# thangvubk/SoftGroup

Measured on AMD Instinct MI355X. Metric: scans/sec ScanNet-v2-like inference (softgroup_scannet.yaml, full forward_test), higher is better.
Workload: dtype f32

## Files before the change

### include/softgroup_hip.h

```cpp
#ifndef SOFTGROUP_HIP_H
#define SOFTGROUP_HIP_H

#include <stddef.h>
#include <stdint.h>

#ifdef __cplusplus
extern "C" {
#endif

typedef void *sg_stream_t;

#define SG_OK 0
#define SG_ERR_ARG (-1)
#define SG_ERR_WORKSPACE (-2)
#define SG_ERR_LAUNCH (-3)
#define SG_ERR_UNSUPPORTED (-4)

#define SG_BALLQUERY_MAX_NEIGHBORS 1000
#define SG_OCTREE_NUM_NODES 585
#define SG_OCTREE_NUM_LEAVES 512
#define SG_LISTS_SORTED 1
#define SG_LISTS_RADIUS 2

int sg_version(void);
const char *sg_last_error(void);
int sg_device_info(char *name_host, int name_cap, int *num_cu_host, int *clock_khz_host);

int sg_stream_release(sg_stream_t stream);
int sg_stream_create(sg_stream_t *stream_out);
int sg_stream_destroy(sg_stream_t stream);
int sg_stream_create_priority(sg_stream_t *stream_out, int level);

int sg_voxelize_idx_host(const int64_t *coords_host, int n, int ncol, int mode,
                         int32_t *input_map_host, int32_t *num_voxels_host,
                         int32_t *max_active_host);
int sg_voxelize_idx_fill_host(const int64_t *coords_host, int n, int ncol, int mode,
                              const int32_t *input_map_host, int num_voxels, int max_active,
                              int64_t *out_coords_host, int32_t *out_map_host);
size_t sg_voxelize_idx_workspace_bytes(int n);
int sg_voxelize_idx_build(const int64_t *coords, int n, int ncol, int mode, int32_t *input_map,
                          int32_t *meta, void *ws, size_t ws_bytes, sg_stream_t stream);
int sg_voxelize_idx_fill(const int64_t *coords, int n, int ncol, int mode,
                         const int32_t *input_map, int num_voxels, int max_active,
                         int64_t *out_coords, int32_t *out_map, void *ws, size_t ws_bytes,
                         sg_stream_t stream);

int sg_voxelize_fp(const float *feats, const int32_t *rules, int num_voxels, int max_active,
                   int channels, int average, float *out, sg_stream_t stream);
int sg_voxelize_bp(const float *d_out, const int32_t *rules, int num_voxels, int max_active,
                   int channels, int average, float *d_feats, sg_stream_t stream);

size_t sg_ballquery_workspace_bytes(int n);
int sg_ballquery_build_grid(const float *xyz, const int32_t *batch_idxs, int n, float radius,
                            void *ws, size_t ws_bytes, sg_stream_t stream);
int sg_ballquery_count(const float *xyz, const int32_t *batch_idxs, int n, float radius,
                       int32_t *start_len, int32_t *meta, void *ws, size_t ws_bytes,
                       sg_stream_t stream);
int sg_ballquery_fill(const float *xyz, const int32_t *batch_idxs, int n, float radius,
                      const int32_t *start_len, int32_t *idx, void *ws, size_t ws_bytes,
                      sg_stream_t stream);
size_t sg_scan_workspace_bytes(int n);
int sg_exclusive_scan_startlen(int32_t *start_len, int n, int32_t *meta, void *ws,
                               size_t ws_bytes, sg_stream_t stream);

int sg_octree_build_host(const float *points_host, const float *xyzwhl_host, int num_points,
                         int num_levels, float *boxes_host, int32_t *pt_inds_host,
                         int32_t *pt_start_len_host);
size_t sg_octree_build_workspace_bytes(int n);
int sg_octree_build(const float *points, int n, float *boxes, int32_t *pt_inds, int32_t *pt_start_len,
                    void *ws, size_t ws_bytes, sg_stream_t stream);
size_t sg_pyramid_inverse_map_workspace_bytes(int n_points, int n_voxels, int n_prop);
int sg_pyramid_inverse_map(const int32_t *proposals_idx, int64_t num_pairs, int n_prop,
                           const int32_t *l2p_map, int n_points, int n_voxels, int32_t *out_idx,
                           int32_t *out_offsets, int32_t *n_out_dev, void *ws, size_t ws_bytes,
                           sg_stream_t stream);
int sg_octree_ballquery_count(const float *points, const float *boxes, const int32_t *pt_inds,
                              const int32_t *pt_start_len, int n, float radius,
                              int32_t *start_len, sg_stream_t stream);
int sg_octree_ballquery_fill(const float *points, const float *boxes, const int32_t *pt_inds,
                             const int32_t *pt_start_len, int n, float radius,
                             const int32_t *start_len, int32_t *idx, sg_stream_t stream);

size_t sg_bfs_workspace_bytes(int n, int64_t n_edges);
int sg_bfs_cluster_label(const int32_t *bq_idxs, const int32_t *start_len, int n,
                         int64_t n_edges, int list_flags, const int32_t *seg_of_point,
                         const float *seg_thr, int n_seg, int32_t *n_cluster_host,
                         int32_t *sum_npoint_host, void *ws, size_t ws_bytes, sg_stream_t stream);
int sg_bfs_cluster_emit(const int32_t *bq_idxs, const int32_t *start_len, int n, int64_t n_edges,
                        const int32_t *seg_of_point, const float *seg_thr, int n_cluster,
                        int sum_npoint, int32_t *cluster_idxs, int32_t *cluster_offsets, void *ws,
                        size_t ws_bytes, sg_stream_t stream);

int sg_sec_mean(const float *inp, const int32_t *offsets, int n_seg, int channels, float *out,
                sg_stream_t stream);
int sg_sec_min(const float *inp, const int32_t *offsets, int n_seg, int channels, float *out,
               sg_stream_t stream);
int sg_sec_max(const float *inp, const int32_t *offsets, int n_seg, int channels, float *out,
               sg_stream_t stream);
int sg_global_avg_pool_fp(const float *feats, const int32_t *offsets, int n_seg, int channels,
                          float *out, sg_stream_t stream);
int sg_global_avg_pool_bp(float *d_feats, const int32_t *offsets, const float *d_out, int n_seg,
                          int channels, sg_stream_t stream);

int sg_get_mask_iou_on_cluster(const int32_t *proposals_idx, const int32_t *proposals_offset,
                               const int64_t *instance_labels, const int32_t *instance_pointnum,
                               int n_instance, int n_proposal, float *proposals_iou,
                               sg_stream_t stream);
int sg_get_mask_iou_on_pred(const int32_t *proposals_idx, const int32_t *proposals_offset,
                            const int64_t *instance_labels, const int32_t *instance_pointnum,
                            const float *mask_scores_sigmoid, int n_instance, int n_proposal,
                            float *proposals_iou, sg_stream_t stream);
int sg_get_mask_label(const int32_t *proposals_idx, const int32_t *proposals_offset,
                      const int64_t *instance_labels, const int64_t *instance_cls,
                      const float *proposals_iou, int n_instance, int n_proposal, float iou_thr,
                      float *mask_label, sg_stream_t stream);

size_t sg_spconv_hash_workspace_bytes(int num_rows);
int sg_spconv_subm_rulebook(const int32_t *indices, int num_rows, const int32_t *spatial_shape_host,
                            int32_t *nbr, void *ws, size_t ws_bytes, sg_stream_t stream);
int sg_spconv_down_build(const int32_t *indices, int num_rows, const int32_t *spatial_shape_host,
                         int32_t *in2out, int32_t *meta, void *ws, size_t ws_bytes,
                         sg_stream_t stream);
int sg_spconv_down_fill(const int32_t *indices, int num_rows, const int32_t *in2out,
                        int num_out_rows, int32_t *out_indices, int32_t *child, void *ws,
                        size_t ws_bytes, sg_stream_t stream);
int sg_spconv_inverse_rulebook(const int32_t *indices_fine, const int32_t *in2out, int num_rows,
                               int32_t *inv_nbr, sg_stream_t stream);

#define SG_PLAN_HIST_WORDS 40
size_t sg_spconv_plan_workspace_bytes(int num_out_rows);
int sg_spconv_plan(const int32_t *nbr, int num_out_rows, int kvol, int32_t *order,
                   uint32_t *tile_mask, int32_t *nbr_tiles, void *ws, size_t ws_bytes,
                   sg_stream_t stream);

#define SG_PYRAMID_MAX_LEVELS 10
typedef struct sg_plan_ptrs {
  int32_t *order;
  uint32_t *tile_mask;
  int32_t *nbr_tiles;
} sg_plan_ptrs;
typedef struct sg_pyramid_level {
  int rows;
  int32_t *indices;
  int32_t *nbr;
  sg_plan_ptrs subm;
  int32_t *in2out;
  int32_t *child;
  sg_plan_ptrs down;
  int32_t *inv;
  sg_plan_ptrs up;
} sg_pyramid_level;
size_t sg_spconv_pyramid_workspace_bytes(int num_rows, int n_levels);
int sg_spconv_pyramid_rows(const int32_t *indices, int num_rows, const int32_t *spatial_shape_host,
                           int n_levels, int32_t *rows_dev, void *ws, size_t ws_bytes,
                           sg_stream_t stream);
size_t sg_spconv_pyramid_build_workspace_bytes(const sg_pyramid_level *levels_host, int n_levels);
int sg_spconv_pyramid_build(const int32_t *indices, int num_rows, const int32_t *spatial_shape_host,
                            int n_levels, const sg_pyramid_level *levels_host, void *ws,
                            size_t ws_bytes, void *ws2, size_t ws2_bytes, sg_stream_t stream);

size_t sg_spconv_packed_weight_elems(int kvol, int cin, int cout);
int sg_spconv_pack_weight(const float *w, int cout, int kvol, int cin, int src_is_kio, float *w_k8,
                          sg_stream_t stream);

size_t sg_spconv_conv_workspace_bytes(int num_out_rows, int cout);
int sg_spconv_gather_conv_f32(const float *in, int num_in_rows, const int32_t *nbr,
                              int num_out_rows, int kvol, int cin, int cout, const float *w_k8,
                              const float *post_scale, const float *post_shift,
                              const float *residual, const float *act_scale,
                              const float *act_shift, float *out_act, const int32_t *order,
                              const uint32_t *tile_mask, const int32_t *nbr_tiles, float *out,
                              void *ws, size_t ws_bytes, sg_stream_t stream);

int sg_spconv_set_arithmetic(int mode);

int sg_spconv_set_combine(int mode);

int sg_grouping_set_lanes(int lanes);

int sg_spconv_set_chain(int mode);
int sg_spconv_chain_stats(int64_t *launches, int64_t *steps);

int sg_spconv_profile(int enable);
int sg_spconv_profile_read(double *total_ms, int *launches);
int sg_spconv_profile_detail(float *ms, int32_t *dims, int cap, int *calls);

typedef struct sg_mlp2 {
  const float *w1, *b1, *bn_scale, *bn_shift, *w2, *b2;
  int out;
} sg_mlp2;
int sg_pointwise_heads(const float *voxel_feats, const void *v2p_map, int v2p_is_int64, int n_points,
                       int channels, const sg_mlp2 *semantic, const sg_mlp2 *offset, float *output_feats,
                       float *semantic_scores, float *pt_offsets, int64_t *semantic_preds,
                       sg_stream_t stream);

size_t sg_spconv_packed_weight_elems_bf16(int kvol, int cin, int cout);
int sg_spconv_pack_weight_bf16(const float *w, int cout, int kvol, int cin, int src_is_kio,
                               uint16_t *w_k8_bf16, sg_stream_t stream);
size_t sg_spconv_conv_bf16_workspace_bytes(int num_out_rows, int cout);
int sg_spconv_gather_conv_bf16(const uint16_t *in, int num_in_rows, const int32_t *nbr, int num_out_rows,
                               int kvol, int cin, int cout, const uint16_t *w_k8_bf16,
                               const int32_t *order, const uint32_t *tile_mask, const int32_t *nbr_tiles,
                               uint16_t *out, void *ws, size_t ws_bytes, sg_stream_t stream);

int sg_spconv_transpose_table(const int32_t *nbr, int num_out_rows, int kvol, int32_t *nbr_t,
                              sg_stream_t stream);
size_t sg_spconv_wgrad_workspace_bytes(int num_out_rows, int kvol, int cin, int cout);
int sg_spconv_wgrad(const void *in, int in_is_bf16, const void *g_out, int g_is_bf16, const int32_t *nbr_t,
                    int num_out_rows, int kvol, int cin, int cout, float *dw_kio, void *ws,
                    size_t ws_bytes, sg_stream_t stream);

typedef struct sg_unet_block {
  int cin, cout;
  const float *bn1_scale, *bn1_shift;
  const float *w1;
  const float *bn2_scale, *bn2_shift;
  const float *w2;
  const float *w_i;
} sg_unet_block;
typedef struct sg_unet_level {
  int planes, n_blocks;
  const sg_unet_block *blocks;
  const sg_unet_block *tail;
  const float *down_bn_scale, *down_bn_shift, *down_w;
  const float *up_bn_scale, *up_bn_shift, *up_w;
} sg_unet_level;
typedef struct sg_unet_desc {
  int n_levels;
  const sg_unet_level *levels;
  int input_cin;
  const float *input_w;
  const float *out_bn_scale, *out_bn_shift;
  int input_cin_packed;
  int arithmetic;
} sg_unet_desc;
size_t sg_unet_arena_bytes(const sg_unet_desc *desc, int num_rows);
int sg_unet_forward(const sg_unet_desc *desc, const float *feats, const int32_t *indices,
                    int num_rows, const int32_t *spatial_shape_host, float *out, void *arena,
                    size_t arena_bytes, sg_stream_t stream);

typedef struct sg_train_bn {
  const float *weight, *bias;
  float *running_mean, *running_var;
  float momentum, eps;
  float *g_weight, *g_bias;
} sg_train_bn;
typedef struct sg_train_conv {
  const float *w;
  float *g_w;
} sg_train_conv;
typedef struct sg_unet_train_block {
  int cin, cout;
  sg_train_bn bn1, bn2;
  sg_train_conv c1, c2, ci;
} sg_unet_train_block;
typedef struct sg_unet_train_level {
  int planes, n_blocks;
  const sg_unet_train_block *blocks, *tail;
  sg_train_bn down_bn, up_bn;
  sg_train_conv down, up;
} sg_unet_train_level;
typedef struct sg_unet_train_desc {
  int n_levels;
  const sg_unet_train_level *levels;
  int input_cin;
  sg_train_conv input;
  sg_train_bn out_bn;
  int arithmetic;
} sg_unet_train_desc;
size_t sg_unet_train_arena_hint(const sg_unet_train_desc *desc, int num_rows);
int sg_unet_train_forward(const sg_unet_train_desc *desc, const float *feats, const int32_t *indices,
                          int num_rows, const int32_t *spatial_shape_host, float *out, void *arena,
                          size_t arena_bytes, size_t *arena_needed, void **tape, sg_stream_t stream);
int sg_unet_train_backward(void *tape, const float *g_out, float *g_feats, sg_stream_t stream);
void sg_unet_train_release(void *tape);

int sg_bn_relu_f32(const float *x, const float *scale, const float *shift, int64_t num_rows,
                   int channels, int relu, float *out, sg_stream_t stream);

int sg_gather_rows_f32(const float *in, const int32_t *index, int64_t num_out_rows, int channels,
                       float *out, sg_stream_t stream);
int sg_gather_rows_i64idx_f32(const float *in, const int64_t *index, int64_t num_out_rows,
                              int channels, float *out, sg_stream_t stream);

int sg_instance_npoint(const int32_t *proposals_idx, const float *mask_scores, int64_t num_pairs,
                       int stride, int n_classes, float mask_thr, int n_prop, int32_t *npoint,
                       sg_stream_t stream);
size_t sg_instance_runs_workspace_bytes(int n_kept, int n_points);
int sg_instance_runs(const int32_t *proposals_idx, const float *mask_scores, int64_t num_pairs,
                     int stride, int n_classes, float mask_thr, const int32_t *inst_of, int n_prop,
                     int n_kept, int n_points, int32_t *starts, int32_t *ends, int64_t *bounds,
                     int64_t runs_capacity, void *ws, size_t ws_bytes, sg_stream_t stream);

int64_t sg_rle_format_bound(int64_t total_runs, int digits);
int sg_rle_format_host(const int64_t *starts_host, const int64_t *lens_host,
                       const int64_t *bounds_host, int n_groups, char *out_host,
                       int64_t out_capacity, int64_t *out_offsets_host);
size_t sg_rle_format_device_workspace_bytes(int64_t run_capacity);
int64_t sg_rle_format_device_text_bytes(int64_t run_capacity, int64_t length);
int sg_rle_format_device(const int32_t *starts, const int32_t *ends, const int64_t *bounds, int n_inst,
                         int64_t run_capacity, int64_t length, uint8_t *text, int64_t text_capacity,
                         int64_t *text_off, void *ws, size_t ws_bytes, sg_stream_t stream);
int sg_rle_format_runs_host(const int32_t *starts_host, const int32_t *ends_host,
                            const int64_t *bounds_host, int n_groups, char *out_host,
                            int64_t out_capacity, int64_t *out_offsets_host);

size_t sg_panoptic_fusion_workspace_bytes(int n_inst, int n_points);
int sg_panoptic_fusion(const uint32_t *bits, int n_inst, int n_points, const int32_t *order,
                       const int32_t *label_id, const int64_t *semantic_preds, int cls_offset,
                       double skip_iou, int semantic_classes, int thing_class_min, uint32_t *out,
                       void *ws, size_t ws_bytes, sg_stream_t stream);

#define SG_NMS_IOU 0
#define SG_NMS_MIN 1
size_t sg_mask_nms_workspace_bytes(int n_inst, int64_t n_points);
int sg_mask_nms(const uint32_t *bits, int n_inst, int64_t n_points, const float *scores, const int32_t *labels,
                double thr, int measure, int class_agnostic, uint8_t *keep, int32_t *n_keep, int32_t *inter_out,
                void *ws, size_t ws_bytes, sg_stream_t stream);
int sg_mask_bits_from_runs(const int32_t *starts, const int32_t *ends, const int64_t *bounds, int64_t n_runs,
                           int n_inst, int64_t n_points, uint32_t *bits, sg_stream_t stream);

#define SG_SPLIT_ALL 0
#define SG_SPLIT_LARGEST 1
#define SG_SPLIT_FLAG_NOT_FINITE 1
#define SG_SPLIT_FLAG_CELL_RANGE 2
#define SG_SPLIT_FLAG_INTERNAL 4
#define SG_SPLIT_FLAG_TOO_MANY 8
size_t sg_mask_split_workspace_bytes(int n_inst, int64_t n_points, int64_t n_pairs);
int sg_mask_split_count(const float *xyz, const uint32_t *bits, int n_inst, int64_t n_points, double radius,
                        int min_npoint, int mode, int32_t *meta, void *ws, size_t ws_bytes, sg_stream_t stream);
int sg_mask_split_fill(int n_inst, int64_t n_points, int64_t n_pairs, const void *ws, size_t ws_bytes,
                       int64_t capacity, uint32_t *out_bits, int32_t *source, int32_t *npoint, sg_stream_t stream);

#define SG_SNAP_SNAP 0
#define SG_SNAP_GROW 1
#define SG_SNAP_TRIM 2
#define SG_SUPERPOINT_FLAG_ID 1
#define SG_SUPERPOINT_WALK 2048
size_t sg_superpoint_index_workspace_bytes(int64_t n_points);
int sg_superpoint_index(const int32_t *sp, int64_t n_points, int32_t *order, int32_t *seg_of, int32_t *seg_start,
                        int32_t *meta, void *ws, size_t ws_bytes, sg_stream_t stream);
size_t sg_mask_snap_workspace_bytes(int n_inst, int64_t n_points, int64_t n_seg);
int sg_mask_snap(const uint32_t *bits, int n_inst, int64_t n_points, const int32_t *order, const int32_t *seg_of,
                 const int32_t *seg_start, int64_t n_seg, int64_t n_valid, double thr, int mode, uint32_t *out_bits,
                 int32_t *npoint, void *ws, size_t ws_bytes, sg_stream_t stream);
size_t sg_superpoint_vote_workspace_bytes(int64_t n_points, int64_t n_seg, int n_classes);
int sg_superpoint_vote(const int32_t *labels, int64_t n_points, const int32_t *order, const int32_t *seg_of,
                       const int32_t *seg_start, int64_t n_seg, int n_classes, int ignore_label, int32_t *out_labels,
                       int32_t *seg_label, void *ws, size_t ws_bytes, sg_stream_t stream);

typedef struct sg_grouping_cfg {
  int n_points;
  int n_sem_classes;
  int n_seg;
  const int32_t *seg_class;
  const float *seg_thr;
  float score_thr;
  int min_npoint;
  float radius;
  int batch_size;
  float voxel_scale;
  int voxel_shape;
  int feat_channels;
} sg_grouping_cfg;
typedef struct sg_grouping_result {
  int n_selected, n_neighbours, n_proposals, sum_npoint, n_voxels, max_active;
  size_t proposals_idx;
  size_t proposals_offset;
  size_t voxel_coords;
  size_t voxel_offsets;
  size_t voxel_feats;
  size_t point_to_voxel;
  size_t arena_used, arena_needed;
  int deferred_classes;
  int reserved_;
} sg_grouping_result;
int sg_scan_grouping(const sg_grouping_cfg *cfg, const float *scores, const float *pt_offsets,
                     const float *coords_float, const int32_t *batch_idxs, const float *point_feats,
                     void *arena, size_t arena_bytes, sg_grouping_result *result_host,
                     sg_stream_t stream);

typedef struct sg_grouping_pp_cfg {
  sg_grouping_cfg base;
  int with_pyramid, with_octree, lvl_fusion;
  double radius;
  double base_size;
} sg_grouping_pp_cfg;
int sg_scan_grouping_pp(const sg_grouping_pp_cfg *cfg, const float *scores, const float *pt_offsets,
                        const float *coords_float, const int32_t *batch_idxs, const float *point_feats,
                        void *arena, size_t arena_bytes, sg_grouping_result *result_host,
                        sg_stream_t stream);

int sg_host_copy_2d(void *dst, int64_t dst_pitch_bytes, const void *src, int64_t src_pitch_bytes, int64_t rows,
                    int64_t row_bytes);
int sg_host_cast_f64_f32(float *dst, const double *src, int64_t n);
int sg_host_fill_i64_strided(int64_t *dst, int64_t pitch_elems, int64_t rows, int64_t value);
int sg_host_colmax_i64(const int64_t *src, int64_t rows, int64_t cols, int64_t *out_max);

typedef struct sg_instances_cfg {
  int n_proposals, n_classes;
  int score_stride;
  int64_t sum_npoint;
  int n_points;
  float cls_score_thr, mask_score_thr;
  int min_npoint;
} sg_instances_cfg;
typedef struct sg_instances_result {
  int n_kept;
  size_t off_class, off_score, off_text, text_bytes;
  size_t host_needed, arena_used, arena_needed;
  size_t bits;
  size_t label_id;
} sg_instances_result;
int sg_scan_instances(const sg_instances_cfg *cfg, const int32_t *proposals_idx, const float *mask_scores,
                      const float *cls_prob, const float *iou_scores, void *arena, size_t arena_bytes,
                      void *host_out, size_t host_bytes, sg_instances_result *result_host,
                      sg_stream_t stream);

typedef struct sg_linear {
  const float *w, *b;
  int out, in;
} sg_linear;
int sg_softmax_rows(const float *x, int64_t rows, int cols, float *out, sg_stream_t stream);
int sg_mlp_rows(const float *feats, const int32_t *idx, int64_t rows, int channels, const sg_mlp2 *mlp,
                float *out, sg_stream_t stream);
int sg_linear_rows(const float *x, int64_t rows, const sg_linear *lin, float *out, sg_stream_t stream);

#define SG_SCAN_DENSE_MAX 16
typedef struct sg_scan_dense_item {
  int kind;
  const void *ptr;
  size_t bytes;
} sg_scan_dense_item;
typedef struct sg_scan_desc {
  const sg_unet_desc *backbone;
  const sg_unet_desc *tiny;
  sg_mlp2 semantic, offset, mask;
  sg_linear cls, iou;
  int channels;
  int with_coords;
  int semantic_classes, instance_classes;
  sg_grouping_cfg grouping;
  float cls_score_thr, mask_score_thr;
  int min_npoint;
  int want_instances;
  int with_pyramid, with_octree;
  double pp_radius, pp_base_size;
} sg_scan_desc;
typedef struct sg_scan_input {
  int n_points, n_voxels, max_active;
  int batch_size;
  int spatial_shape[3];
  const float *feats;
  int feat_dim;
  const float *coords_float;
  const int32_t *p2v_map;
  const void *v2p_map;
  int v2p_is_int64;
  const void *voxel_coords;
  int voxel_coords_is_int64;
  const int32_t *batch_idxs;
  const int64_t *semantic_labels, *instance_labels;
  int n_dense;
  sg_scan_dense_item dense[SG_SCAN_DENSE_MAX];
} sg_scan_input;
typedef struct sg_scan_result {
  sg_grouping_result grouping;
  sg_instances_result instances;
  size_t grouping_base, instances_base;
  size_t dense_offset[SG_SCAN_DENSE_MAX];
  size_t dense_bytes;
  size_t voxel_feats_in, backbone_out, output_feats, semantic_scores, semantic_prob, pt_offsets,
      semantic_preds, tiny_out, mask_scores, cls_scores, cls_prob, iou_scores;
  size_t arena_used, arena_needed, host_dense_needed, host_inst_needed;
  int stage;
} sg_scan_result;
size_t sg_scan_arena_bytes(const sg_scan_desc *desc, int n_points, int n_voxels);
int sg_scan_forward(const sg_scan_desc *desc, const sg_scan_input *in, void *arena, size_t arena_bytes,
                    void *host_dense, size_t host_dense_bytes, void *host_inst, size_t host_inst_bytes,
                    sg_scan_result *result_host, sg_stream_t stream);

int sg_eval_intersections(const int32_t *run_start, const int64_t *run_off, const int32_t *run_pred,
                          int n_runs, int64_t total_points, const int32_t *gt_slot, int n_pred,
                          int n_slots, int32_t *counts, sg_stream_t stream);

#define SG_EVAL_I32 0
#define SG_EVAL_I64 1
#define SG_EVAL_U32 2
#define SG_EVAL_MAX_CLASSES 1024
#define SG_EVAL_BAD_GT 1
#define SG_EVAL_BAD_PRED 2
#define SG_EVAL_BAD_INST 4

size_t sg_eval_tally_workspace_bytes(int64_t n_points);
int sg_eval_class_tally(const void *pred, int pred_kind, const void *gt, int gt_kind, int64_t n_points,
                        int64_t ignore_label, int panoptic, int n_classes, uint64_t *tallies,
                        const void *inst, int inst_kind, const float *offset_pred, const float *offset_gt,
                        double *offset_sum, uint64_t *offset_count, int32_t *flags, void *ws, size_t ws_bytes,
                        sg_stream_t stream);

size_t sg_eval_panoptic_workspace_bytes(int64_t n_points);
int sg_eval_panoptic_segments(const void *pred, int pred_kind, const void *sem, int sem_kind,
                              const void *inst, int inst_kind, const int64_t *scan_off, int n_scans,
                              int64_t n_points, int64_t ignore_label, int n_classes, int64_t min_points,
                              uint64_t *fp_fn, int64_t *tp_rows, uint64_t *tp_count, int32_t *flags,
                              void *ws, size_t ws_bytes, sg_stream_t stream);

#define SG_INST_BAD_TEXT 1
#define SG_INST_ODD_TOKENS 2
#define SG_INST_RUN_RANGE 4
#define SG_INST_BAD_GT 8
#define SG_INST_OVERFLOW_GT 16
#define SG_INST_OVERFLOW_EX 32
#define SG_INST_NO_EXAMPLES 64
#define SG_INST_MAX_THRESHOLDS 16
#define SG_INST_SECTIONS 16

int64_t sg_inst_rle_run_slots(int64_t text_bytes, int n_masks);
int sg_inst_rle_parse(const uint8_t *text, const int64_t *text_off, const int32_t *mask_pred, int n_masks,
                      int64_t text_bytes, int64_t length, int32_t *run_start, int32_t *run_len, int32_t *run_pred,
                      int64_t run_slots, int32_t *vert_count, int32_t *flags, sg_stream_t stream);

size_t sg_inst_scan_workspace_bytes(int64_t n_points, int n_pred, int64_t run_slots, int n_classes, int gt_cap,
                                    int n_thr, int n_labels, int64_t *section_off);
int sg_inst_scan_update(const int64_t *gts, int64_t n_points, const int32_t *run_start, const int32_t *run_len,
                        const int32_t *run_pred, int64_t run_slots, const int32_t *pred_label,
                        const int32_t *pred_vert, const double *pred_conf, int n_pred, int n_labels, int n_classes,
                        int64_t min_region, const double *thresholds, int n_thr, int gt_cap, uint64_t *ex_key,
                        uint32_t *ex_meta, int64_t ex_cap, int32_t *seg_stats, int64_t *totals, int32_t *flags,
                        void *ws, size_t ws_bytes, sg_stream_t stream);

int sg_inst_scan_coverage(int64_t n_points, int n_pred, int64_t run_slots, int n_classes, int gt_cap, int n_thr,
                          int n_labels, const int32_t *pred_label, const int32_t *pred_vert,
                          const double *pred_conf, int64_t min_region, double iou_thr, double score_thr,
                          double *cov_sums, int64_t *tallies, const int32_t *flags, void *ws, size_t ws_bytes,
                          sg_stream_t stream);

size_t sg_inst_curves_workspace_bytes(int64_t n_examples, int n_seg);
int sg_inst_curves(const uint64_t *ex_key, const uint32_t *ex_meta, int64_t n_examples, const int32_t *seg_stats,
                   int n_seg, double *ap, double *rc, int32_t *flags, void *ws, size_t ws_bytes,
                   sg_stream_t stream);

#define SG_DET_BAD_COORD 1
#define SG_DET_MAX_THRESHOLDS 16

int sg_det_boxes_runs(const void *coords, int coords_f64, const int64_t *run_start, const int64_t *run_off,
                      const int32_t *run_owner, int64_t n_runs, int64_t total_points, int64_t n_owner,
                      double *boxes, int32_t *flags, sg_stream_t stream);

int sg_det_boxes_labels(const void *coords, int coords_f64, const int64_t *labels, const int64_t *scan_off,
                        const int64_t *owner_off, int n_scans, int64_t n_points, int64_t n_owner, double *boxes,
                        int64_t *count, int64_t *first, int32_t *flags, sg_stream_t stream);

size_t sg_det_match_workspace_bytes(int64_t n_gt, int n_thresholds);
int sg_det_match(const double *det_box, const int32_t *det_group, const int32_t *det_rank, int64_t n_det,
                 const double *gt_box, const int64_t *group_off, int64_t n_gt, const double *thresholds,
                 int n_thresholds, double *ovmax, int64_t *jmax, uint8_t *tp, void *ws, size_t ws_bytes,
                 sg_stream_t stream);

int sg_train_augment(const float *xyz, int64_t n, int has_scale, float scale_factor, const double *m_host,
                     double work_scale, double down, double *xyz_middle, double *work, uint64_t *stats,
                     sg_stream_t stream);
int sg_train_blur(float *grids, float *tmp, int b0, int b1, int b2, int n_grids, sg_stream_t stream);
int sg_train_elastic(double *work, int64_t n, const float *grids, int b0, int b1, int b2, double gran, double mag,
                     uint64_t *stats, sg_stream_t stream);
int sg_train_crop_count(const double *work, int64_t n, double down, const double *min_host,
                        const double *cand_host, int k, uint64_t *counts, sg_stream_t stream);
size_t sg_train_compact_workspace_bytes(int64_t n);
int sg_train_compact(const double *work, const double *xyz_middle, const float *feat, int c, const float *noise,
                     const int64_t *sem, const int64_t *inst, int64_t n, double down, const double *min_host,
                     const double *crop_host, int64_t out_cap, int64_t *coord, double *xyz_middle_out,
                     float *feat_out, int64_t *sem_out, int64_t *inst_out, int32_t *kept, void *ws,
                     size_t ws_bytes, sg_stream_t stream);
int sg_train_gather(const int64_t *idx, int64_t m, const float *xyz, const float *feat, int c, const int64_t *sem,
                    const int64_t *inst, float *xyz_out, float *feat_out, int64_t *sem_out, int64_t *inst_out,
                    sg_stream_t stream);
size_t sg_train_id_set_workspace_bytes(void);
int sg_train_id_set(const int64_t *labels, int64_t n, int64_t ignore, int64_t *out, int cap, void *ws,
                    size_t ws_bytes, sg_stream_t stream);
int sg_train_remap(int64_t *labels, int64_t n, const int64_t *sorted_ids, const int64_t *mapped, int k,
                   sg_stream_t stream);
size_t sg_train_instance_workspace_bytes(int64_t n, int k);
int sg_train_instance_info(const double *xyz_middle, const int64_t *inst, const int64_t *sem, int64_t n, int k,
                           int64_t cls_shift, int32_t *pointnum, int64_t *cls, double *pt_offset, void *ws,
                           size_t ws_bytes, sg_stream_t stream);

int sg_test_x4_minima(const float *xyz, int64_t n, const double *m_host, double scale, uint64_t *stats,
                      sg_stream_t stream);
int sg_test_x4_split(const float *xyz, const float *feat, int c, const int64_t *sem, const int64_t *inst, int64_t n,
                     const double *m_host, double scale, const double *min_host, int64_t *coord,
                     double *xyz_middle, float *feat_out, int64_t *sem_out, int64_t *inst_out, sg_stream_t stream);
int sg_kitti_decode_labels(const int32_t *words, int64_t n, const int32_t *lut, int64_t *sem, int64_t *inst,
                           uint64_t *missing, sg_stream_t stream);

int sg_mask_text_runs(const int32_t *starts, const int32_t *ends, const int64_t *bounds, int64_t n_runs, int n_inst,
                      int64_t length, int first, int count, uint8_t *text, int64_t text_capacity, sg_stream_t stream);
int sg_mask_text_bits(const uint32_t *bits, int n_inst, int64_t length, int first, int count, uint8_t *text,
                      int64_t text_capacity, sg_stream_t stream);
size_t sg_decimal_lines_workspace_bytes(int64_t n);
int sg_decimal_lines(const int64_t *values, int64_t n, const int32_t *nyu_table, int nyu_len, uint8_t *text,
                     int64_t text_capacity, int64_t *meta, void *ws, size_t ws_bytes, sg_stream_t stream);
int sg_panoptic_kitti_words(const uint32_t *words, int64_t n, const int32_t *lut, int lut_len, uint32_t *out,
                            uint64_t *missing, uint64_t *missing_host, sg_stream_t stream);
size_t sg_parse_decimal_lines_workspace_bytes(int64_t nbytes);
int sg_parse_decimal_lines(const uint8_t *text, int64_t nbytes, int64_t *values, int64_t capacity, int64_t *meta,
                           void *ws, size_t ws_bytes, sg_stream_t stream);
int sg_parse_mask_text(const uint8_t *text, int64_t nbytes, uint8_t *flags, uint32_t *bits, int64_t *meta,
                       sg_stream_t stream);

int sg_viz_paint_bits(const uint32_t *bits, int n_inst, int64_t n, const int32_t *priority, const uint8_t *skip,
                      int32_t *label, int32_t *pointnum, sg_stream_t stream);
size_t sg_viz_paint_runs_workspace_bytes(int n_inst, int64_t n);
int sg_viz_paint_runs(const int32_t *starts, const int32_t *ends, const int64_t *bounds, int64_t n_runs, int n_inst,
                      int64_t n, const int32_t *priority, const uint8_t *skip, int32_t *label, int32_t *pointnum,
                      void *ws, size_t ws_bytes, sg_stream_t stream);
int sg_viz_gt_labels(const int64_t *ids, int64_t n, int32_t *label, int32_t *pointnum, sg_stream_t stream);
size_t sg_viz_instance_rank_workspace_bytes(int n_inst);
int sg_viz_instance_rank(const int32_t *pointnum, int n_inst, int32_t *rank, void *ws, size_t ws_bytes,
                         sg_stream_t stream);
#define SG_VIZ_INPUT 0
#define SG_VIZ_CLASS 1
#define SG_VIZ_CLASS_WRAP 2
#define SG_VIZ_INSTANCE 3
int sg_viz_colors(int mode, const float *colors, const int64_t *cls, const int32_t *inst, const int32_t *rank,
                  int n_rank, const uint8_t *table, int k, int64_t n, uint8_t *rgb, int64_t *meta,
                  sg_stream_t stream);
size_t sg_viz_ply_vertices_workspace_bytes(int64_t n);
int sg_viz_ply_vertices(const float *xyz, const float *offset, const uint8_t *rgb, const uint8_t *keep, int64_t n,
                        uint8_t *text, int64_t text_capacity, int64_t *meta, void *ws, size_t ws_bytes,
                        sg_stream_t stream);

size_t sg_loss_reduce_workspace_bytes(void);
int sg_pointwise_loss_fwd(const float *semantic_scores, const int64_t *semantic_labels, const float *weight,
                          int64_t ignore_label, const float *pt_offsets, const float *pt_offset_labels,
                          const int64_t *instance_labels, int64_t n, int c, float *out, void *ws, size_t ws_bytes,
                          sg_stream_t stream);
int sg_pointwise_loss_bwd(const float *semantic_scores, const int64_t *semantic_labels, const float *weight,
                          int64_t ignore_label, const float *pt_offsets, const float *pt_offset_labels,
                          const int64_t *instance_labels, int64_t n, int c, const float *sums,
                          const float *g_semantic, const float *g_offset, float *d_scores, float *d_offsets,
                          sg_stream_t stream);
size_t sg_assign_proposals_workspace_bytes(int n_proposal);
int sg_assign_proposals(const float *ious_on_cluster, const int64_t *instance_cls, int64_t ignore_label,
                        float pos_iou_thr, int match_low_quality, float min_pos_thr, int64_t background_label,
                        int n_proposal, int n_gt, int64_t *labels, void *ws, size_t ws_bytes, sg_stream_t stream);
int sg_proposal_loss_fwd(const float *cls_scores, const float *iou_scores, const int64_t *labels,
                         const float *ious_on_pred, const int64_t *instance_cls, int64_t ignore_label,
                         int n_proposal, int n_gt, int k1, float *gt_iou, float *out, void *ws, size_t ws_bytes,
                         sg_stream_t stream);
int sg_proposal_loss_bwd(const float *cls_scores, const float *iou_scores, const int64_t *labels,
                         const float *gt_iou, const float *sums, const float *g_cls, const float *g_iou,
                         int n_proposal, int k1, float *d_cls_scores, float *d_iou_scores, sg_stream_t stream);
int sg_mask_loss_fwd(const float *mask_scores, const int32_t *instance_batch_idxs, const int64_t *labels,
                     const float *mask_label, int64_t m, int n_proposal, int k1, float *mask_sig, float *out,
                     void *ws, size_t ws_bytes, sg_stream_t stream);
int sg_mask_loss_bwd(const float *mask_scores, const int32_t *instance_batch_idxs, const int64_t *labels,
                     const float *mask_label, const float *sums, const float *g_mask, int64_t m, int n_proposal,
                     int k1, float *d_mask_scores, sg_stream_t stream);

#define SG_OPTIM_ROW_PARAM 0
#define SG_OPTIM_ROW_GRAD 1
#define SG_OPTIM_ROW_STATE0 2
#define SG_OPTIM_ROW_STATE1 3
#define SG_OPTIM_ROW_STEP 4
#define SG_OPTIM_ROW_COUNT 5
#define SG_OPTIM_TABLE_ROWS 6
int sg_optim_chunk_elems(void);
int64_t sg_optim_plan(const int64_t *counts, int n_tensors, int64_t *chunks, int64_t chunk_capacity);
size_t sg_optim_workspace_bytes(void);
int sg_optim_grad_norm(const int64_t *table, int n_tensors, const int64_t *chunks, int64_t n_chunks,
                       const float *grad_scale, float max_norm, float *out, void *ws, size_t ws_bytes,
                       sg_stream_t stream);
int sg_optim_adam_step(const int64_t *table, int n_tensors, const int64_t *chunks, int64_t n_chunks, double lr,
                       double beta1, double beta2, double eps, double weight_decay, int adamw,
                       const float *grad_scale, const float *found_inf, const float *clip_coef, int zero_grad,
                       int32_t *arrive, sg_stream_t stream);
int sg_optim_sgd_step(const int64_t *table, int n_tensors, const int64_t *chunks, int64_t n_chunks, double lr,
                      double momentum, double dampening, double weight_decay, int nesterov, const float *grad_scale,
                      const float *found_inf, const float *clip_coef, int zero_grad, int32_t *arrive,
                      sg_stream_t stream);
int sg_optim_scale_grads(const int64_t *table, int n_tensors, const int64_t *chunks, int64_t n_chunks,
                         const float *coef, sg_stream_t stream);

#define SG_PICK_FIRST 0
#define SG_PICK_CENTER 1
size_t sg_grid_downsample_workspace_bytes(int n);
int sg_grid_downsample(const float *xyz, int n, double voxel, int pick, int32_t *sample_ids, int32_t *inverse,
                       int32_t *meta, void *ws, size_t ws_bytes, sg_stream_t stream);
double sg_nearest_default_cell(const double *lo, const double *hi, int64_t n_src);
size_t sg_nearest_grid_bytes(int n_src);
int sg_nearest_build(const float *src, int n_src, double cell, void *grid, size_t grid_bytes, int32_t *meta,
                     sg_stream_t stream);
size_t sg_nearest_query_workspace_bytes(int n_query);
int sg_nearest_query(const float *src, int n_src, double cell, const void *grid, size_t grid_bytes, const float *query,
                     int n_query, double max_dist, int32_t *index, double *dist2, int32_t *meta, void *ws,
                     size_t ws_bytes, sg_stream_t stream);
int sg_mask_bits_gather(const uint32_t *bits, int n_inst, int64_t n_src, const int32_t *index, int64_t n_out,
                        uint32_t *out, int32_t *meta, sg_stream_t stream);
size_t sg_mask_runs_workspace_bytes(int n_inst, int64_t n_points);
int sg_mask_runs_count(const uint32_t *bits, int n_inst, int64_t n_points, int64_t *bounds, void *ws, size_t ws_bytes,
                       sg_stream_t stream);
int sg_mask_runs_fill(const uint32_t *bits, int n_inst, int64_t n_points, const void *ws, size_t ws_bytes,
                      int32_t *starts, int32_t *ends, int64_t capacity, sg_stream_t stream);

size_t sg_tile_assign_workspace_bytes(int n);
size_t sg_tile_assign_fill_workspace_bytes(int64_t total);
int sg_tile_assign_count(const float *xyz, int n, double size, double margin, double ox, double oy, int32_t *meta,
                         void *ws, size_t ws_bytes, sg_stream_t stream);
int sg_tile_assign_fill(const float *xyz, int n, double size, double margin, double ox, double oy, int n_tiles,
                        int64_t total, int32_t *tile_cells, int64_t *tile_off, int32_t *tile_points,
                        int32_t *core_tile, int32_t *core_pos, const void *ws, size_t ws_bytes, void *ws2,
                        size_t ws2_bytes, sg_stream_t stream);
size_t sg_tile_shared_workspace_bytes(int n_a);
int sg_tile_shared(const int32_t *a, int n_a, const int32_t *b, int n_b, int32_t *pos_a, int32_t *pos_b,
                   int32_t *count, void *ws, size_t ws_bytes, sg_stream_t stream);
int sg_mask_cross_links(const uint32_t *bits_a, int n_a, const uint32_t *bits_b, int n_b, int64_t n_bits,
                        const int32_t *labels_a, const int32_t *labels_b, int base_a, int base_b, int n_total,
                        double thr, int measure, int min_shared, uint32_t *adj, int32_t *inter_out,
                        int32_t *cnt_a_out, int32_t *cnt_b_out, sg_stream_t stream);
int sg_stitch_components(const uint32_t *adj, int n_total, int32_t *comp, sg_stream_t stream);
int sg_mask_bits_ids_count(const uint32_t *bits, int n_inst, int64_t n_bits, const uint8_t *core, int32_t *cnt,
                           int32_t *core_cnt, sg_stream_t stream);
int sg_mask_bits_ids_fill(const uint32_t *bits, int n_inst, int64_t n_bits, const int32_t *map, int64_t n_points,
                          const int64_t *row_off, const int32_t *row_key, int32_t *ids, uint32_t *keys,
                          int64_t capacity, int32_t *meta, sg_stream_t stream);
size_t sg_stitch_union_workspace_bytes(int64_t total, int n_obj, int64_t n_points);
int sg_stitch_union_count(const int32_t *ids, const uint32_t *keys, int64_t total, int n_obj, int64_t n_points,
                          int64_t *bounds, void *ws, size_t ws_bytes, sg_stream_t stream);
int sg_stitch_union_fill(int64_t total, int n_obj, int64_t n_points, const void *ws, size_t ws_bytes, int32_t *starts,
                         int32_t *ends, int64_t capacity, sg_stream_t stream);

#define SG_KNN_MAX_K 32
#define SG_KNN_MAX_SHELL 3
#define SG_KNN_FLAG_NOT_FINITE 1
#define SG_KNN_FLAG_CELL_RANGE 4
double sg_knn_default_cell(const double *lo, const double *hi, int64_t n, int k);
size_t sg_knn_workspace_bytes(int64_t n, int k);
int sg_knn(const float *xyz, int64_t n, int k, double cell, double max_dist, int32_t *idx, double *d2, int32_t *meta,
           void *ws, size_t ws_bytes, sg_stream_t stream);
#define SG_GEOMETRY_FLAG_INDEX 1
#define SG_GEOMETRY_FLAG_INTERNAL 2
int sg_point_normals(const float *xyz, int64_t n, const int32_t *nbr, int k, int min_neighbours, float *normals,
                     float *curvature, int32_t *meta, sg_stream_t stream);
size_t sg_grow_segments_workspace_bytes(int64_t n);
int sg_grow_segments(const int32_t *nbr, const double *nbr_d2, int64_t n, int k, const float *normals,
                     const float *curvature, double cos_thr, float max_curvature, double max_dist, int min_size,
                     int absorb, int32_t *sp, int32_t *meta, void *ws, size_t ws_bytes, sg_stream_t stream);

#ifdef __cplusplus
}
#endif
#endif
```

### softgroup_amd/_lib.py

```python
import ctypes as C
import os

_HERE = os.path.dirname(os.path.abspath(__file__))
LIB_PATH = os.path.join(_HERE, 'lib', os.environ.get('SG_LIB_NAME', 'libsoftgroup_hip.so'))

_lib = None

_vp, _i, _f, _i64, _sz, _d = C.c_void_p, C.c_int, C.c_float, C.c_int64, C.c_size_t, C.c_double
_pi32 = C.POINTER(C.c_int32)

SIGNATURES = {
    'sg_version': (_i, []),
    'sg_last_error': (C.c_char_p, []),
    'sg_device_info': (_i, [C.c_char_p, _i, C.POINTER(_i), C.POINTER(_i)]),
    'sg_stream_release': (_i, [_vp]),
    'sg_host_copy_2d': (_i, [_vp, _i64, _vp, _i64, _i64, _i64]),
    'sg_host_cast_f64_f32': (_i, [_vp, _vp, _i64]),
    'sg_host_fill_i64_strided': (_i, [_vp, _i64, _i64, _i64]),
    'sg_host_colmax_i64': (_i, [_vp, _i64, _i64, _vp]),
    'sg_stream_create': (_i, [_vp]),
    'sg_stream_create_priority': (_i, [_vp, _i]),
    'sg_stream_destroy': (_i, [_vp]),
    'sg_voxelize_idx_host': (_i, [_vp, _i, _i, _i, _vp, _pi32, _pi32]),
    'sg_voxelize_idx_fill_host': (_i, [_vp, _i, _i, _i, _vp, _i, _i, _vp, _vp]),
    'sg_voxelize_idx_workspace_bytes': (_sz, [_i]),
    'sg_voxelize_idx_build': (_i, [_vp, _i, _i, _i, _vp, _vp, _vp, _sz, _vp]),
    'sg_voxelize_idx_fill': (_i, [_vp, _i, _i, _i, _vp, _i, _i, _vp, _vp, _vp, _sz, _vp]),
    'sg_voxelize_fp': (_i, [_vp, _vp, _i, _i, _i, _i, _vp, _vp]),
    'sg_voxelize_bp': (_i, [_vp, _vp, _i, _i, _i, _i, _vp, _vp]),
    'sg_ballquery_workspace_bytes': (_sz, [_i]),
    'sg_ballquery_build_grid': (_i, [_vp, _vp, _i, _f, _vp, _sz, _vp]),
    'sg_ballquery_count': (_i, [_vp, _vp, _i, _f, _vp, _vp, _vp, _sz, _vp]),
    'sg_ballquery_fill': (_i, [_vp, _vp, _i, _f, _vp, _vp, _vp, _sz, _vp]),
    'sg_scan_workspace_bytes': (_sz, [_i]),
    'sg_exclusive_scan_startlen': (_i, [_vp, _i, _vp, _vp, _sz, _vp]),
    'sg_octree_build_host': (_i, [_vp, _vp, _i, _i, _vp, _vp, _vp]),
    'sg_octree_build_workspace_bytes': (_sz, [_i]),
    'sg_octree_build': (_i, [_vp, _i, _vp, _vp, _vp, _vp, _sz, _vp]),
    'sg_pyramid_inverse_map_workspace_bytes': (_sz, [_i, _i, _i]),
    'sg_pyramid_inverse_map': (_i, [_vp, _i64, _i, _vp, _i, _i, _vp, _vp, _vp, _vp, _sz, _vp]),
    'sg_octree_ballquery_count': (_i, [_vp, _vp, _vp, _vp, _i, _f, _vp, _vp]),
    'sg_octree_ballquery_fill': (_i, [_vp, _vp, _vp, _vp, _i, _f, _vp, _vp, _vp]),
    'sg_bfs_workspace_bytes': (_sz, [_i, _i64]),
    'sg_bfs_cluster_label': (_i, [_vp, _vp, _i, _i64, _i, _vp, _vp, _i, _pi32, _pi32, _vp, _sz, _vp]),
    'sg_bfs_cluster_emit': (_i, [_vp, _vp, _i, _i64, _vp, _vp, _i, _i, _vp, _vp, _vp, _sz, _vp]),
    'sg_sec_mean': (_i, [_vp, _vp, _i, _i, _vp, _vp]),
    'sg_sec_min': (_i, [_vp, _vp, _i, _i, _vp, _vp]),
    'sg_sec_max': (_i, [_vp, _vp, _i, _i, _vp, _vp]),
    'sg_global_avg_pool_fp': (_i, [_vp, _vp, _i, _i, _vp, _vp]),
    'sg_global_avg_pool_bp': (_i, [_vp, _vp, _vp, _i, _i, _vp]),
    'sg_get_mask_iou_on_cluster': (_i, [_vp, _vp, _vp, _vp, _i, _i, _vp, _vp]),
    'sg_get_mask_iou_on_pred': (_i, [_vp, _vp, _vp, _vp, _vp, _i, _i, _vp, _vp]),
    'sg_get_mask_label': (_i, [_vp, _vp, _vp, _vp, _vp, _i, _i, _f, _vp, _vp]),
    'sg_spconv_hash_workspace_bytes': (_sz, [_i]),
    'sg_spconv_subm_rulebook': (_i, [_vp, _i, _pi32, _vp, _vp, _sz, _vp]),
    'sg_spconv_pyramid_workspace_bytes': (_sz, [_i, _i]),
    'sg_spconv_pyramid_rows': (_i, [_vp, _i, _pi32, _i, _vp, _vp, _sz, _vp]),
    'sg_spconv_pyramid_build_workspace_bytes': (_sz, [_vp, _i]),
    'sg_spconv_pyramid_build': (_i, [_vp, _i, _pi32, _i, _vp, _vp, _sz, _vp, _sz, _vp]),
    'sg_spconv_down_build': (_i, [_vp, _i, _pi32, _vp, _vp, _vp, _sz, _vp]),
    'sg_spconv_down_fill': (_i, [_vp, _i, _vp, _i, _vp, _vp, _vp, _sz, _vp]),
    'sg_spconv_inverse_rulebook': (_i, [_vp, _vp, _i, _vp, _vp]),
    'sg_spconv_plan_workspace_bytes': (_sz, [_i]),
    'sg_spconv_plan': (_i, [_vp, _i, _i, _vp, _vp, _vp, _vp, _sz, _vp]),
    'sg_spconv_set_arithmetic': (_i, [_i]),
    'sg_spconv_set_combine': (_i, [_i]),
    'sg_spconv_set_chain': (_i, [_i]),
    'sg_grouping_set_lanes': (_i, [_i]),
    'sg_spconv_chain_stats': (_i, [_vp, _vp]),
    'sg_spconv_profile': (_i, [_i]),
    'sg_spconv_profile_read': (_i, [_vp, _vp]),
    'sg_spconv_profile_detail': (_i, [_vp, _vp, _i, _vp]),
    'sg_unet_arena_bytes': (_sz, [_vp, _i]),
    'sg_unet_forward': (_i, [_vp, _vp, _vp, _i, _vp, _vp, _vp, _sz, _vp]),
    'sg_unet_train_arena_hint': (_sz, [_vp, _i]),
    'sg_unet_train_forward': (_i, [_vp, _vp, _vp, _i, _vp, _vp, _vp, _sz, _vp, _vp, _vp]),
    'sg_unet_train_backward': (_i, [_vp, _vp, _vp, _vp]),
    'sg_unet_train_release': (None, [_vp]),
    'sg_pointwise_heads': (_i, [_vp, _vp, _i, _i, _i, _vp, _vp, _vp, _vp, _vp, _vp, _vp]),
    'sg_spconv_packed_weight_elems': (_sz, [_i, _i, _i]),
    'sg_spconv_pack_weight': (_i, [_vp, _i, _i, _i, _i, _vp, _vp]),
    'sg_spconv_conv_workspace_bytes': (_sz, [_i, _i]),
    'sg_spconv_gather_conv_f32': (_i, [_vp, _i, _vp, _i, _i, _i, _i, _vp, _vp, _vp, _vp, _vp, _vp,
                                       _vp, _vp, _vp, _vp, _vp, _vp, _sz, _vp]),
    'sg_spconv_packed_weight_elems_bf16': (_sz, [_i, _i, _i]),
    'sg_spconv_pack_weight_bf16': (_i, [_vp, _i, _i, _i, _i, _vp, _vp]),
    'sg_spconv_conv_bf16_workspace_bytes': (_sz, [_i, _i]),
    'sg_spconv_gather_conv_bf16': (_i, [_vp, _i, _vp, _i, _i, _i, _i, _vp, _vp, _vp, _vp, _vp, _vp, _sz,
                                        _vp]),
    'sg_spconv_transpose_table': (_i, [_vp, _i, _i, _vp, _vp]),
    'sg_spconv_wgrad_workspace_bytes': (_sz, [_i, _i, _i, _i]),
    'sg_spconv_wgrad': (_i, [_vp, _i, _vp, _i, _vp, _i, _i, _i, _i, _vp, _vp, _sz, _vp]),
    'sg_instance_npoint': (_i, [_vp, _vp, _i64, _i, _i, _f, _i, _vp, _vp]),
    'sg_instance_runs_workspace_bytes': (_sz, [_i, _i]),
    'sg_instance_runs': (_i, [_vp, _vp, _i64, _i, _i, _f, _vp, _i, _i, _i, _vp, _vp, _vp, _i64, _vp, _sz, _vp]),
    'sg_rle_format_bound': (_i64, [_i64, _i]),
    'sg_rle_format_host': (_i, [_vp, _vp, _vp, _i, _vp, _i64, _vp]),
    'sg_rle_format_device_workspace_bytes': (_sz, [_i64]),
    'sg_rle_format_device_text_bytes': (_i64, [_i64, _i64]),
    'sg_rle_format_device': (_i, [_vp, _vp, _vp, _i, _i64, _i64, _vp, _i64, _vp, _vp, _sz, _vp]),
    'sg_rle_format_runs_host': (_i, [_vp, _vp, _vp, _i, _vp, _i64, _vp]),
    'sg_panoptic_fusion_workspace_bytes': (_sz, [_i, _i]),
    'sg_panoptic_fusion': (_i, [_vp, _i, _i, _vp, _vp, _vp, _i, C.c_double, _i, _i, _vp, _vp, _sz, _vp]),
    'sg_mask_nms_workspace_bytes': (_sz, [_i, _i64]),
    'sg_mask_nms': (_i, [_vp, _i, _i64, _vp, _vp, _d, _i, _i, _vp, _vp, _vp, _vp, _sz, _vp]),
    'sg_mask_bits_from_runs': (_i, [_vp, _vp, _vp, _i64, _i, _i64, _vp, _vp]),
    'sg_mask_split_workspace_bytes': (_sz, [_i, _i64, _i64]),
    'sg_mask_split_count': (_i, [_vp, _vp, _i, _i64, _d, _i, _i, _vp, _vp, _sz, _vp]),
    'sg_mask_split_fill': (_i, [_i, _i64, _i64, _vp, _sz, _i64, _vp, _vp, _vp, _vp]),
    'sg_superpoint_index_workspace_bytes': (_sz, [_i64]),
    'sg_superpoint_index': (_i, [_vp, _i64, _vp, _vp, _vp, _vp, _vp, _sz, _vp]),
    'sg_mask_snap_workspace_bytes': (_sz, [_i, _i64, _i64]),
    'sg_mask_snap': (_i, [_vp, _i, _i64, _vp, _vp, _vp, _i64, _i64, _d, _i, _vp, _vp, _vp, _sz, _vp]),
    'sg_superpoint_vote_workspace_bytes': (_sz, [_i64, _i64, _i]),
    'sg_superpoint_vote': (_i, [_vp, _i64, _vp, _vp, _vp, _i64, _i, _i, _vp, _vp, _vp, _sz, _vp]),
    'sg_scan_grouping': (_i, [_vp, _vp, _vp, _vp, _vp, _vp, _vp, _sz, _vp, _vp]),
    'sg_scan_grouping_pp': (_i, [_vp, _vp, _vp, _vp, _vp, _vp, _vp, _sz, _vp, _vp]),
    'sg_scan_instances': (_i, [_vp, _vp, _vp, _vp, _vp, _vp, _sz, _vp, _sz, _vp, _vp]),
    'sg_softmax_rows': (_i, [_vp, _i64, _i, _vp, _vp]),
    'sg_mlp_rows': (_i, [_vp, _vp, _i64, _i, _vp, _vp, _vp]),
    'sg_linear_rows': (_i, [_vp, _i64, _vp, _vp, _vp]),
    'sg_scan_arena_bytes': (_sz, [_vp, _i, _i]),
    'sg_scan_forward': (_i, [_vp, _vp, _vp, _sz, _vp, _sz, _vp, _sz, _vp, _vp]),
    'sg_eval_intersections': (_i, [_vp, _vp, _vp, _i, _i64, _vp, _i, _i, _vp, _vp]),
    'sg_eval_tally_workspace_bytes': (_sz, [_i64]),
    'sg_eval_class_tally': (_i, [_vp, _i, _vp, _i, _i64, _i64, _i, _i, _vp, _vp, _i, _vp, _vp, _vp, _vp, _vp,
                                 _vp, _sz, _vp]),
    'sg_eval_panoptic_workspace_bytes': (_sz, [_i64]),
    'sg_eval_panoptic_segments': (_i, [_vp, _i, _vp, _i, _vp, _i, _vp, _i, _i64, _i64, _i, _i64, _vp, _vp, _vp,
                                       _vp, _vp, _sz, _vp]),
    'sg_inst_rle_run_slots': (_i64, [_i64, _i]),
    'sg_inst_rle_parse': (_i, [_vp, _vp, _vp, _i, _i64, _i64, _vp, _vp, _vp, _i64, _vp, _vp, _vp]),
    'sg_inst_scan_workspace_bytes': (_sz, [_i64, _i, _i64, _i, _i, _i, _i, _vp]),
    'sg_inst_scan_update': (_i, [_vp, _i64, _vp, _vp, _vp, _i64, _vp, _vp, _vp, _i, _i, _i, _i64, _vp, _i, _i,
                                 _vp, _vp, _i64, _vp, _vp, _vp, _vp, _sz, _vp]),
    'sg_inst_scan_coverage': (_i, [_i64, _i, _i64, _i, _i, _i, _i, _vp, _vp, _vp, _i64, _d, _d, _vp, _vp, _vp, _vp,
                                   _sz, _vp]),
    'sg_inst_curves_workspace_bytes': (_sz, [_i64, _i]),
    'sg_inst_curves': (_i, [_vp, _vp, _i64, _vp, _i, _vp, _vp, _vp, _vp, _sz, _vp]),
    'sg_det_boxes_runs': (_i, [_vp, _i, _vp, _vp, _vp, _i64, _i64, _i64, _vp, _vp, _vp]),
    'sg_det_boxes_labels': (_i, [_vp, _i, _vp, _vp, _vp, _i, _i64, _i64, _vp, _vp, _vp, _vp, _vp]),
    'sg_det_match_workspace_bytes': (_sz, [_i64, _i]),
    'sg_det_match': (_i, [_vp, _vp, _vp, _i64, _vp, _vp, _i64, _vp, _i, _vp, _vp, _vp, _vp, _sz, _vp]),
    'sg_bn_relu_f32': (_i, [_vp, _vp, _vp, _i64, _i, _i, _vp, _vp]),
    'sg_gather_rows_f32': (_i, [_vp, _vp, _i64, _i, _vp, _vp]),
    'sg_gather_rows_i64idx_f32': (_i, [_vp, _vp, _i64, _i, _vp, _vp]),
    'sg_train_augment': (_i, [_vp, _i64, _i, _f, _vp, C.c_double, C.c_double, _vp, _vp, _vp, _vp]),
    'sg_train_blur': (_i, [_vp, _vp, _i, _i, _i, _i, _vp]),
    'sg_train_elastic': (_i, [_vp, _i64, _vp, _i, _i, _i, C.c_double, C.c_double, _vp, _vp]),
    'sg_train_crop_count': (_i, [_vp, _i64, C.c_double, _vp, _vp, _i, _vp, _vp]),
    'sg_train_compact_workspace_bytes': (_sz, [_i64]),
    'sg_train_compact': (_i, [_vp, _vp, _vp, _i, _vp, _vp, _vp, _i64, C.c_double, _vp, _vp, _i64, _vp, _vp, _vp, _vp,
                              _vp, _vp, _vp, _sz, _vp]),
    'sg_train_gather': (_i, [_vp, _i64, _vp, _vp, _i, _vp, _vp, _vp, _vp, _vp, _vp, _vp]),
    'sg_train_id_set_workspace_bytes': (_sz, []),
    'sg_train_id_set': (_i, [_vp, _i64, _i64, _vp, _i, _vp, _sz, _vp]),
    'sg_train_remap': (_i, [_vp, _i64, _vp, _vp, _i, _vp]),
    'sg_train_instance_workspace_bytes': (_sz, [_i64, _i]),
    'sg_train_instance_info': (_i, [_vp, _vp, _vp, _i64, _i, _i64, _vp, _vp, _vp, _vp, _sz, _vp]),
    'sg_test_x4_minima': (_i, [_vp, _i64, _vp, C.c_double, _vp, _vp]),
    'sg_test_x4_split': (_i, [_vp, _vp, _i, _vp, _vp, _i64, _vp, C.c_double, _vp, _vp, _vp, _vp, _vp, _vp, _vp]),
    'sg_kitti_decode_labels': (_i, [_vp, _i64, _vp, _vp, _vp, _vp, _vp]),
    'sg_mask_text_runs': (_i, [_vp, _vp, _vp, _i64, _i, _i64, _i, _i, _vp, _i64, _vp]),
    'sg_mask_text_bits': (_i, [_vp, _i, _i64, _i, _i, _vp, _i64, _vp]),
    'sg_decimal_lines_workspace_bytes': (_sz, [_i64]),
    'sg_decimal_lines': (_i, [_vp, _i64, _vp, _i, _vp, _i64, _vp, _vp, _sz, _vp]),
    'sg_panoptic_kitti_words': (_i, [_vp, _i64, _vp, _i, _vp, _vp, _vp, _vp]),
    'sg_parse_decimal_lines_workspace_bytes': (_sz, [_i64]),
    'sg_parse_decimal_lines': (_i, [_vp, _i64, _vp, _i64, _vp, _vp, _sz, _vp]),
    'sg_parse_mask_text': (_i, [_vp, _i64, _vp, _vp, _vp, _vp]),
    'sg_viz_paint_bits': (_i, [_vp, _i, _i64, _vp, _vp, _vp, _vp, _vp]),
    'sg_viz_paint_runs_workspace_bytes': (_sz, [_i, _i64]),
    'sg_viz_paint_runs': (_i, [_vp, _vp, _vp, _i64, _i, _i64, _vp, _vp, _vp, _vp, _vp, _sz, _vp]),
    'sg_viz_gt_labels': (_i, [_vp, _i64, _vp, _vp, _vp]),
    'sg_viz_instance_rank_workspace_bytes': (_sz, [_i]),
    'sg_viz_instance_rank': (_i, [_vp, _i, _vp, _vp, _sz, _vp]),
    'sg_viz_colors': (_i, [_i, _vp, _vp, _vp, _vp, _i, _vp, _i, _i64, _vp, _vp, _vp]),
    'sg_viz_ply_vertices_workspace_bytes': (_sz, [_i64]),
    'sg_viz_ply_vertices': (_i, [_vp, _vp, _vp, _vp, _i64, _vp, _i64, _vp, _vp, _sz, _vp]),
    'sg_loss_reduce_workspace_bytes': (_sz, []),
    'sg_pointwise_loss_fwd': (_i, [_vp, _vp, _vp, _i64, _vp, _vp, _vp, _i64, _i, _vp, _vp, _sz, _vp]),
    'sg_pointwise_loss_bwd': (_i, [_vp, _vp, _vp, _i64, _vp, _vp, _vp, _i64, _i, _vp, _vp, _vp, _vp, _vp, _vp]),
    'sg_assign_proposals_workspace_bytes': (_sz, [_i]),
    'sg_assign_proposals': (_i, [_vp, _vp, _i64, _f, _i, _f, _i64, _i, _i, _vp, _vp, _sz, _vp]),
    'sg_proposal_loss_fwd': (_i, [_vp, _vp, _vp, _vp, _vp, _i64, _i, _i, _i, _vp, _vp, _vp, _sz, _vp]),
    'sg_proposal_loss_bwd': (_i, [_vp, _vp, _vp, _vp, _vp, _vp, _vp, _i, _i, _vp, _vp, _vp]),
    'sg_mask_loss_fwd': (_i, [_vp, _vp, _vp, _vp, _i64, _i, _i, _vp, _vp, _vp, _sz, _vp]),
    'sg_mask_loss_bwd': (_i, [_vp, _vp, _vp, _vp, _vp, _vp, _i64, _i, _i, _vp, _vp]),
    'sg_optim_chunk_elems': (_i, []),
    'sg_optim_plan': (_i64, [_vp, _i, _vp, _i64]),
    'sg_optim_workspace_bytes': (_sz, []),
    'sg_optim_grad_norm': (_i, [_vp, _i, _vp, _i64, _vp, _f, _vp, _vp, _sz, _vp]),
    'sg_optim_adam_step': (_i, [_vp, _i, _vp, _i64, _d, _d, _d, _d, _d, _i, _vp, _vp, _vp, _i, _vp, _vp]),
    'sg_optim_sgd_step': (_i, [_vp, _i, _vp, _i64, _d, _d, _d, _d, _i, _vp, _vp, _vp, _i, _vp, _vp]),
    'sg_optim_scale_grads': (_i, [_vp, _i, _vp, _i64, _vp, _vp]),
    'sg_grid_downsample_workspace_bytes': (_sz, [_i]),
    'sg_grid_downsample': (_i, [_vp, _i, _d, _i, _vp, _vp, _vp, _vp, _sz, _vp]),
    'sg_nearest_default_cell': (_d, [_vp, _vp, _i64]),
    'sg_nearest_grid_bytes': (_sz, [_i]),
    'sg_nearest_build': (_i, [_vp, _i, _d, _vp, _sz, _vp, _vp]),
    'sg_nearest_query_workspace_bytes': (_sz, [_i]),
    'sg_nearest_query': (_i, [_vp, _i, _d, _vp, _sz, _vp, _i, _d, _vp, _vp, _vp, _vp, _sz, _vp]),
    'sg_mask_bits_gather': (_i, [_vp, _i, _i64, _vp, _i64, _vp, _vp, _vp]),
    'sg_mask_runs_workspace_bytes': (_sz, [_i, _i64]),
    'sg_mask_runs_count': (_i, [_vp, _i, _i64, _vp, _vp, _sz, _vp]),
    'sg_mask_runs_fill': (_i, [_vp, _i, _i64, _vp, _sz, _vp, _vp, _i64, _vp]),
    'sg_tile_assign_workspace_bytes': (_sz, [_i]),
    'sg_tile_assign_fill_workspace_bytes': (_sz, [_i64]),
    'sg_tile_assign_count': (_i, [_vp, _i, _d, _d, _d, _d, _vp, _vp, _sz, _vp]),
    'sg_tile_assign_fill': (_i, [_vp, _i, _d, _d, _d, _d, _i, _i64, _vp, _vp, _vp, _vp, _vp, _vp, _sz, _vp, _sz, _vp]),
    'sg_tile_shared_workspace_bytes': (_sz, [_i]),
    'sg_tile_shared': (_i, [_vp, _i, _vp, _i, _vp, _vp, _vp, _vp, _sz, _vp]),
    'sg_mask_cross_links': (_i, [_vp, _i, _vp, _i, _i64, _vp, _vp, _i, _i, _i, _d, _i, _i, _vp, _vp, _vp, _vp, _vp]),
    'sg_stitch_components': (_i, [_vp, _i, _vp, _vp]),
    'sg_mask_bits_ids_count': (_i, [_vp, _i, _i64, _vp, _vp, _vp, _vp]),
    'sg_mask_bits_ids_fill': (_i, [_vp, _i, _i64, _vp, _i64, _vp, _vp, _vp, _vp, _i64, _vp, _vp]),
    'sg_stitch_union_workspace_bytes': (_sz, [_i64, _i, _i64]),
    'sg_stitch_union_count': (_i, [_vp, _vp, _i64, _i, _i64, _vp, _vp, _sz, _vp]),
    'sg_stitch_union_fill': (_i, [_i64, _i, _i64, _vp, _sz, _vp, _vp, _i64, _vp]),
    'sg_knn_default_cell': (_d, [_vp, _vp, _i64, _i]),
    'sg_knn_workspace_bytes': (_sz, [_i64, _i]),
    'sg_knn': (_i, [_vp, _i64, _i, _d, _d, _vp, _vp, _vp, _vp, _sz, _vp]),
    'sg_point_normals': (_i, [_vp, _i64, _vp, _i, _i, _vp, _vp, _vp, _vp]),
    'sg_grow_segments_workspace_bytes': (_sz, [_i64]),
    'sg_grow_segments': (_i, [_vp, _vp, _i64, _i, _vp, _vp, _d, _f, _d, _i, _i, _vp, _vp, _vp, _sz, _vp]),
}


class SoftGroupHipError(RuntimeError):
    pass


def lib():
    global _lib
    if _lib is None:
        import torch
        if not os.path.exists(LIB_PATH):
            raise SoftGroupHipError(
                f'{LIB_PATH} not found: the HIP extension is required (no CPU fallback). '
                'Build it with `python -c "import __graft_entry__ as g; g.build()"`.')
        L = C.CDLL(LIB_PATH)
        for name, (res, args) in SIGNATURES.items():
            fn = getattr(L, name)
            fn.restype = res
            fn.argtypes = args
        _lib = L
    return _lib


def check(rc, what=''):
    if rc != 0:
        msg = lib().sg_last_error()
        raise SoftGroupHipError(f'{what} failed ({rc}): {msg.decode() if msg else ""}')


def ptr(t):
    return None if t is None else t.data_ptr()


_raw_stream = None


def stream():
    global _raw_stream
    import torch
    if _raw_stream is None:
        _raw_stream = getattr(torch._C, '_cuda_getCurrentRawStream', None) or (
            lambda dev: torch.cuda.current_stream(dev).cuda_stream)
    return _raw_stream(torch.cuda.current_device())


def workspace(nbytes, device):
    import torch
    return torch.empty(max(int(nbytes), 256), dtype=torch.uint8, device=device)
```

### softgroup_amd/csrc/heads.h

```cpp
#pragma once
#include "common.h"

namespace sg {

struct Mlp2 {
  const float *w1, *b1, *scale, *shift, *w2, *b2;
  int out;
};

template <int C, int OUT_MAX>
__device__ __forceinline__ void mlp2(const float (&x)[C], const Mlp2 &m, float (&y)[OUT_MAX]) {
  float h[C];
#pragma unroll
  for (int o = 0; o < C; ++o) {
    float a = m.b1[o];
#pragma unroll
    for (int c = 0; c < C; ++c) a = fmaf(x[c], m.w1[o * C + c], a);
    h[o] = fmaxf(fmaf(a, m.scale[o], m.shift[o]), 0.f);
  }
#pragma unroll
  for (int o = 0; o < OUT_MAX; ++o) {
    if (o < m.out) {
      float a = m.b2[o];
#pragma unroll
      for (int c = 0; c < C; ++c) a = fmaf(h[c], m.w2[o * C + c], a);
      y[o] = a;
    }
  }
}

}
```

### softgroup_amd/csrc/heads.hip

```cpp
#include "common.h"
#include "heads.h"

namespace sg {

template <int C, int SEM_MAX, typename IdxT>
__global__ void __launch_bounds__(256) pointwise_heads_kernel(const float *__restrict__ vox, const IdxT *__restrict__ v2p,
                                                             int n, Mlp2 sem, Mlp2 off, float *__restrict__ out_feats,
                                                             float *__restrict__ sem_scores, float *__restrict__ pt_offsets,
                                                             int64_t *__restrict__ sem_preds) {
  const int p = blockIdx.x * 256 + threadIdx.x;
  if (p >= n) return;
  const int64_t row = v2p ? static_cast<int64_t>(v2p[p]) : p;
  float x[C];
  const float4 *src = reinterpret_cast<const float4 *>(vox + row * C);
#pragma unroll
  for (int q = 0; q < C / 4; ++q) {
    const float4 v = src[q];
    x[4 * q] = v.x; x[4 * q + 1] = v.y; x[4 * q + 2] = v.z; x[4 * q + 3] = v.w;
  }
  if (out_feats) {
    float4 *dst = reinterpret_cast<float4 *>(out_feats + static_cast<int64_t>(p) * C);
#pragma unroll
    for (int q = 0; q < C / 4; ++q) dst[q] = make_float4(x[4 * q], x[4 * q + 1], x[4 * q + 2], x[4 * q + 3]);
  }
  {
    float y[SEM_MAX];
    mlp2<C, SEM_MAX>(x, sem, y);
    float best = y[0];
    int arg = 0;
#pragma unroll
    for (int o = 0; o < SEM_MAX; ++o) {
      if (o < sem.out) {
        sem_scores[static_cast<int64_t>(p) * sem.out + o] = y[o];
        if (o > 0 && (y[o] > best || (y[o] != y[o] && best == best))) {
          best = y[o];
          arg = o;
        }
      }
    }
    if (sem_preds) sem_preds[p] = arg;
  }
  {
    float y[4];
    mlp2<C, 4>(x, off, y);
#pragma unroll
    for (int o = 0; o < 4; ++o)
      if (o < off.out) pt_offsets[static_cast<int64_t>(p) * off.out + o] = y[o];
  }
}

template <int C, typename IdxT>
static void launch_heads(const float *vox, const void *v2p, int n, const Mlp2 &s, const Mlp2 &o, float *out_feats,
                         float *sem_scores, float *pt_offsets, int64_t *sem_preds, hipStream_t st) {
  pointwise_heads_kernel<C, 32, IdxT><<<(n + 255) / 256, 256, 0, st>>>(vox, static_cast<const IdxT *>(v2p), n, s, o,
                                                                       out_feats, sem_scores, pt_offsets, sem_preds);
}

}

using namespace sg;

extern "C" int sg_pointwise_heads(const float *voxel_feats, const void *v2p_map, int v2p_is_int64, int n_points,
                                  int channels, const sg_mlp2 *semantic, const sg_mlp2 *offset, float *output_feats,
                                  float *semantic_scores, float *pt_offsets, int64_t *semantic_preds,
                                  sg_stream_t stream) {
  SG_REQUIRE(n_points >= 0 && semantic && offset && semantic_scores && pt_offsets, "sg_pointwise_heads: bad arguments");
  SG_REQUIRE(channels == 16 || channels == 32, "sg_pointwise_heads: channels must be 16 or 32 (got %d)", channels);
  SG_REQUIRE(semantic->out >= 1 && semantic->out <= 32 && offset->out >= 1 && offset->out <= 4,
             "sg_pointwise_heads: head widths out of range (semantic %d, offset %d)", semantic->out, offset->out);
  if (n_points == 0) return SG_OK;
  const Mlp2 s{semantic->w1, semantic->b1, semantic->bn_scale, semantic->bn_shift, semantic->w2, semantic->b2, semantic->out};
  const Mlp2 o{offset->w1, offset->b1, offset->bn_scale, offset->bn_shift, offset->w2, offset->b2, offset->out};
  hipStream_t st = as_stream(stream);
  if (channels == 32) {
    if (v2p_is_int64) launch_heads<32, int64_t>(voxel_feats, v2p_map, n_points, s, o, output_feats, semantic_scores, pt_offsets, semantic_preds, st);
    else launch_heads<32, int32_t>(voxel_feats, v2p_map, n_points, s, o, output_feats, semantic_scores, pt_offsets, semantic_preds, st);
  } else {
    if (v2p_is_int64) launch_heads<16, int64_t>(voxel_feats, v2p_map, n_points, s, o, output_feats, semantic_scores, pt_offsets, semantic_preds, st);
    else launch_heads<16, int32_t>(voxel_feats, v2p_map, n_points, s, o, output_feats, semantic_scores, pt_offsets, semantic_preds, st);
  }
  return check_launch("sg_pointwise_heads");
}
```

### softgroup_amd/csrc/scan_exec.hip

```cpp
#include <stdlib.h>
#include <string.h>

#include "common.h"
#include "scan.h"

namespace sg {

constexpr int kSelBlock = 256;
constexpr int kMaxSeg = 32;

__global__ void __launch_bounds__(kSelBlock) select_count_kernel(const float *__restrict__ scores, int n,
                                                                int n_cls, const int32_t *__restrict__ seg_class,
                                                                int n_seg, float thr, int n_blocks,
                                                                int32_t *__restrict__ blk_cnt) {
  __shared__ int part[4][kMaxSeg];
  const int i = blockIdx.x * kSelBlock + threadIdx.x;
  const int wave = threadIdx.x >> 6, lane = threadIdx.x & 63;
  for (int s = 0; s < n_seg; ++s) {
    const bool on = i < n && scores[static_cast<int64_t>(i) * n_cls + seg_class[s]] > thr;
    const int c = __popcll(__ballot(on));
    if (lane == 0) part[wave][s] = c;
  }
  __syncthreads();
  if (threadIdx.x < n_seg)
    blk_cnt[threadIdx.x * n_blocks + blockIdx.x] =
        part[0][threadIdx.x] + part[1][threadIdx.x] + part[2][threadIdx.x] + part[3][threadIdx.x];
}

__global__ void __launch_bounds__(1024) select_scan_kernel(const int32_t *__restrict__ blk_cnt, int n_seg,
                                                          int n_blocks, int min_npoint,
                                                          int32_t *__restrict__ blk_off,
                                                          int32_t *__restrict__ meta) {
  constexpr int kG = 8;
  __shared__ int seg_tot[kMaxSeg], seg_base[kMaxSeg + 1], carry_s[kMaxSeg];
  __shared__ int wtot[kG][16];
  const int wave = threadIdx.x >> 6, lane = threadIdx.x & 63;
  for (int s0 = 0; s0 < n_seg; s0 += kG) {
    int sum[kG];
#pragma unroll
    for (int j = 0; j < kG; ++j) sum[j] = 0;
    for (int b0 = 0; b0 < n_blocks; b0 += 1024) {
      const int b = b0 + threadIdx.x;
      int v[kG];
#pragma unroll
      for (int j = 0; j < kG; ++j) v[j] = (s0 + j < n_seg && b < n_blocks) ? blk_cnt[(s0 + j) * n_blocks + b] : 0;
#pragma unroll
      for (int j = 0; j < kG; ++j) sum[j] += v[j];
    }
#pragma unroll
    for (int j = 0; j < kG; ++j) {
      const int t = wave_sum(sum[j]);
      if (lane == 0) wtot[j][wave] = t;
    }
    __syncthreads();
    if (threadIdx.x < kG && s0 + threadIdx.x < n_seg) {
      int t = 0;
      for (int w = 0; w < 16; ++w) t += wtot[threadIdx.x][w];
      seg_tot[s0 + threadIdx.x] = t >= min_npoint ? t : 0;
    }
    __syncthreads();
  }
  if (threadIdx.x == 0) {
    int acc = 0;
    for (int s = 0; s < n_seg; ++s) {
      seg_base[s] = acc;
      carry_s[s] = acc;
      acc += seg_tot[s];
      meta[1 + s] = seg_tot[s];
    }
    seg_base[n_seg] = acc;
    meta[0] = acc;
  }
  __syncthreads();
  for (int s0 = 0; s0 < n_seg; s0 += kG) {
    for (int b0 = 0; b0 < n_blocks; b0 += 1024) {
      const int b = b0 + threadIdx.x;
      int v[kG], incl[kG];
#pragma unroll
      for (int j = 0; j < kG; ++j)
        v[j] = (s0 + j < n_seg && b < n_blocks && seg_tot[s0 + j] > 0) ? blk_cnt[(s0 + j) * n_blocks + b] : 0;
#pragma unroll
      for (int j = 0; j < kG; ++j) {
        incl[j] = wave_incl_scan(v[j]);
        if (lane == 63) wtot[j][wave] = incl[j];
      }
      __syncthreads();
#pragma unroll
      for (int j = 0; j < kG; ++j) {
        if (s0 + j < n_seg) {
          int before = 0, all = 0;
          for (int w = 0; w < 16; ++w) {
            const int x = wtot[j][w];
            before += w < wave ? x : 0;
            all += x;
          }
          if (b < n_blocks)
            blk_off[(s0 + j) * n_blocks + b] = seg_tot[s0 + j] > 0 ? carry_s[s0 + j] + before + incl[j] - v[j] : -1;
        }
      }
      __syncthreads();
      if (threadIdx.x < kG && s0 + threadIdx.x < n_seg) {
        int all = 0;
        for (int w = 0; w < 16; ++w) all += wtot[threadIdx.x][w];
        carry_s[s0 + threadIdx.x] += all;
      }
      __syncthreads();
    }
  }
}

__global__ void __launch_bounds__(kSelBlock) select_emit_kernel(
    const float *__restrict__ scores, int n, int n_cls, const int32_t *__restrict__ seg_class, int n_seg,
    float thr, int n_blocks, const int32_t *__restrict__ blk_off, const float *__restrict__ coords,
    const float *__restrict__ offsets, const int32_t *__restrict__ batch_idxs, int batch_size,
    int32_t *__restrict__ obj, int32_t *__restrict__ seg_of, float *__restrict__ pts, int32_t *__restrict__ key) {
  __shared__ int wcnt[4];
  const int i = blockIdx.x * kSelBlock + threadIdx.x;
  const int wave = threadIdx.x >> 6;
  float c[3] = {0.f, 0.f, 0.f};
  int bi = 0;
  if (i < n) {
#pragma unroll
    for (int a = 0; a < 3; ++a) c[a] = __fadd_rn(coords[3LL * i + a], offsets[3LL * i + a]);
    bi = batch_idxs[i];
  }
  for (int s = 0; s < n_seg; ++s) {
    const int base = blk_off[s * n_blocks + blockIdx.x];
    if (base < 0) continue;
    const bool on = i < n && scores[static_cast<int64_t>(i) * n_cls + seg_class[s]] > thr;
    const uint64_t m = __ballot(on);
    if ((threadIdx.x & 63) == 0) wcnt[wave] = __popcll(m);
    __syncthreads();
    int before = 0;
    for (int w = 0; w < wave; ++w) before += wcnt[w];
    if (on) {
      const int pos = base + before + mask_prefix(m);
      obj[pos] = i;
      seg_of[pos] = s;
      pts[3LL * pos] = c[0];
      pts[3LL * pos + 1] = c[1];
      pts[3LL * pos + 2] = c[2];
      key[pos] = s * batch_size + bi;
    }
    __syncthreads();
  }
}

__global__ void __launch_bounds__(256) proposal_map_kernel(int32_t *__restrict__ pairs, int64_t S,
                                                          const int32_t *__restrict__ obj) {
  for (int64_t e = blockIdx.x * 256LL + threadIdx.x; e < S; e += gridDim.x * 256LL)
    pairs[2 * e + 1] = obj[pairs[2 * e + 1]];
}

__global__ void __launch_bounds__(256) proposal_box_kernel(const int32_t *__restrict__ pairs,
                                                          const int32_t *__restrict__ offsets, int n_prop,
                                                          const float *__restrict__ coords, float inv_ss,
                                                          float scale_max, float *__restrict__ cscale,
                                                          float *__restrict__ lo_s) {
  __shared__ float rmin[3][256], rmax[3][256];
  for (int p = blockIdx.x; p < n_prop; p += gridDim.x) {
    const int s = offsets[p], e = offsets[p + 1];
    float mn[3] = {INFINITY, INFINITY, INFINITY}, mx[3] = {-INFINITY, -INFINITY, -INFINITY};
#pragma unroll 4
    for (int i = s + threadIdx.x; i < e; i += 256) {
      const int pt = pairs[2LL * i + 1];
#pragma unroll
      for (int a = 0; a < 3; ++a) {
        const float x = coords[3LL * pt + a];
        if (x < mn[a]) mn[a] = x;
        if (x > mx[a]) mx[a] = x;
      }
    }
#pragma unroll
    for (int a = 0; a < 3; ++a) {
      rmin[a][threadIdx.x] = mn[a];
      rmax[a][threadIdx.x] = mx[a];
    }
    __syncthreads();
    for (int w = 128; w > 0; w >>= 1) {
      if (threadIdx.x < w) {
#pragma unroll
        for (int a = 0; a < 3; ++a) {
          const float x = rmin[a][threadIdx.x + w], y = rmax[a][threadIdx.x + w];
          if (x < rmin[a][threadIdx.x]) rmin[a][threadIdx.x] = x;
          if (y > rmax[a][threadIdx.x]) rmax[a][threadIdx.x] = y;
        }
      }
      __syncthreads();
    }
    if (threadIdx.x == 0) {
      float ext = -INFINITY;
      bool nan = false;
#pragma unroll
      for (int a = 0; a < 3; ++a) {
        const float d = __fmul_rn(__fsub_rn(rmax[a][0], rmin[a][0]), inv_ss);
        nan |= d != d;
        if (d > ext) ext = d;
      }
      if (nan) ext = NAN;
      float cs = __fadd_rn(__fmul_rn(__fdiv_rn(1.0f, ext), 1.0f), -0.01f);
      cs = (cs != cs) ? cs : fminf(cs, scale_max);
      cscale[p] = cs;
#pragma unroll
      for (int a = 0; a < 3; ++a) lo_s[3 * p + a] = __fmul_rn(rmin[a][0], cs);
    }
    __syncthreads();
  }
}

__global__ void __launch_bounds__(256) proposal_voxel_coords_kernel(
    const int32_t *__restrict__ pairs, int64_t S, const float *__restrict__ coords,
    const float *__restrict__ cscale, const float *__restrict__ lo_s, int ss, int64_t *__restrict__ vox,
    int32_t *__restrict__ bad) {
  for (int64_t e = blockIdx.x * 256LL + threadIdx.x; e < S; e += gridDim.x * 256LL) {
    const int p = pairs[2 * e], pt = pairs[2 * e + 1];
    const float cs = cscale[p];
    int64_t *o = vox + 4 * e;
    o[0] = p;
    bool ok = true;
#pragma unroll
    for (int a = 0; a < 3; ++a) {
      const float v = __fsub_rn(__fmul_rn(coords[3LL * pt + a], cs), lo_s[3 * p + a]);
      ok &= v >= 0.f && v < static_cast<float>(ss);
      o[1 + a] = static_cast<int64_t>(v);
    }
    if (!ok) atomicOr(bad, 1);
  }
}

__global__ void __launch_bounds__(256) proposal_voxel_feats_kernel(const float *__restrict__ feats,
                                                                  const int32_t *__restrict__ pairs,
                                                                  const int32_t *__restrict__ rules, int M,
                                                                  int max_active, int C,
                                                                  float *__restrict__ out) {
  const int64_t total = static_cast<int64_t>(M) * C;
  for (int64_t t = blockIdx.x * 256LL + threadIdx.x; t < total; t += gridDim.x * 256LL) {
    const int row = static_cast<int>(t / C), c = static_cast<int>(t - static_cast<int64_t>(row) * C);
    const int32_t *r = rules + static_cast<int64_t>(row) * (max_active + 1);
    const int cnt = r[0];
    const float m = cnt > 0 ? __fdiv_rn(1.0f, static_cast<float>(cnt)) : 1.0f;
    float acc = 0.0f;
    int i = 1;
    for (; i + 15 <= cnt; i += 16) {
      int a[16], q[16];
      float f[16];
#pragma unroll
      for (int j = 0; j < 16; ++j) a[j] = r[i + j];
#pragma unroll
      for (int j = 0; j < 16; ++j) q[j] = pairs[2LL * a[j] + 1];
#pragma unroll
      for (int j = 0; j < 16; ++j) f[j] = feats[static_cast<int64_t>(q[j]) * C + c];
#pragma unroll
      for (int j = 0; j < 16; ++j) acc = __fadd_rn(acc, __fmul_rn(m, f[j]));
    }
    for (; i + 3 <= cnt; i += 4) {
      const int a0 = r[i], a1 = r[i + 1], a2 = r[i + 2], a3 = r[i + 3];
      const int p0 = pairs[2LL * a0 + 1], p1 = pairs[2LL * a1 + 1], p2 = pairs[2LL * a2 + 1],
                p3 = pairs[2LL * a3 + 1];
      const float f0 = feats[static_cast<int64_t>(p0) * C + c], f1 = feats[static_cast<int64_t>(p1) * C + c],
                  f2 = feats[static_cast<int64_t>(p2) * C + c], f3 = feats[static_cast<int64_t>(p3) * C + c];
      acc = __fadd_rn(acc, __fmul_rn(m, f0));
      acc = __fadd_rn(acc, __fmul_rn(m, f1));
      acc = __fadd_rn(acc, __fmul_rn(m, f2));
      acc = __fadd_rn(acc, __fmul_rn(m, f3));
    }
    for (; i <= cnt; ++i)
      acc = __fadd_rn(acc, __fmul_rn(m, feats[static_cast<int64_t>(pairs[2LL * r[i] + 1]) * C + c]));
    out[t] = acc;
  }
}

__global__ void __launch_bounds__(256) proposal_voxel_pack_kernel(const int64_t *__restrict__ vc, int M,
                                                                 int n_prop, int32_t *__restrict__ out,
                                                                 int32_t *__restrict__ vox_off) {
  for (int m = blockIdx.x * 256 + threadIdx.x; m < M; m += gridDim.x * 256) {
    const int p = static_cast<int>(vc[4LL * m]);
#pragma unroll
    for (int a = 0; a < 4; ++a) out[4LL * m + a] = static_cast<int32_t>(vc[4LL * m + a]);
    if (m == 0 || static_cast<int>(vc[4LL * (m - 1)]) != p) vox_off[p] = m;
    if (m == M - 1) vox_off[n_prop] = M;
  }
}

__global__ void __launch_bounds__(1024) instance_keep_kernel(const float *__restrict__ cls_prob,
                                                           const float *__restrict__ iou, int stride,
                                                           const int32_t *__restrict__ npoint, int n_prop,
                                                           int nc, float cls_thr, int min_npoint,
                                                           int32_t *__restrict__ inst_of,
                                                           int32_t *__restrict__ kept_cls,
                                                           float *__restrict__ kept_score,
                                                           int32_t *__restrict__ head) {
  __shared__ int wsum[16];
  __shared__ int cap_s;
  if (threadIdx.x == 0) cap_s = 0;
  __syncthreads();
  const int total = nc * n_prop;
  const int wave = threadIdx.x >> 6, lane = threadIdx.x & 63;
  int carry = 0, cap = 0;
  for (int base = 0; base < total; base += 1024) {
    const int t = base + threadIdx.x;
    int keep = 0, np = 0, i = 0, p = 0;
    if (t < total) {
      i = t / n_prop;
      p = t - i * n_prop;
      np = npoint[p * nc + i];
      keep = (cls_prob[p * stride + i] > cls_thr && np >= min_npoint) ? 1 : 0;
    }
    int incl = wave_incl_scan(keep);
    if (lane == 63) wsum[wave] = incl;
    __syncthreads();
    int tot = 0;
#pragma unroll
    for (int w = 0; w < 16; ++w) {
      const int x = wsum[w];
      incl += w < wave ? x : 0;
      tot += x;
    }
    __syncthreads();
    if (t < total) {
      const int k = carry + incl - keep;
      inst_of[t] = keep ? k : -1;
      if (keep) {
        kept_cls[k] = i + 1;
        const float q = iou[p * stride + i];
        const float qc = (q != q) ? q : fminf(fmaxf(q, 0.f), 1.f);
        kept_score[k] = __fmul_rn(cls_prob[p * stride + i], qc);
        cap += np;
      }
    }
    carry += tot;
  }
  cap = wave_sum(cap);
  if ((threadIdx.x & 63) == 0) atomicAdd(&cap_s, cap);
  __syncthreads();
  if (threadIdx.x == 0) {
    head[0] = carry;
    head[1] = cap_s;
  }
}

__global__ void __launch_bounds__(256) pp_level_inputs_kernel(const int32_t *__restrict__ obj, int n,
                                                             const float *__restrict__ coords,
                                                             const float *__restrict__ offsets,
                                                             const int32_t *__restrict__ batch_idxs, float inv,
                                                             int64_t *__restrict__ vox, float *__restrict__ c3,
                                                             float *__restrict__ o3) {
  const int i = blockIdx.x * 256 + threadIdx.x;
  if (i >= n) return;
  const int p = obj[i];
  vox[4LL * i] = batch_idxs[p];
#pragma unroll
  for (int a = 0; a < 3; ++a) {
    const float c = coords[3LL * p + a];
    c3[3LL * i + a] = c;
    o3[3LL * i + a] = offsets[3LL * p + a];
    vox[4LL * i + 1 + a] = static_cast<int64_t>(__fmul_rn(c, inv));
  }
}
__global__ void __launch_bounds__(256) pp_level_points_kernel(const float *__restrict__ cl, const float *__restrict__ ol,
                                                             const int64_t *__restrict__ vc, int m,
                                                             float *__restrict__ q, int32_t *__restrict__ qb) {
  const int i = blockIdx.x * 256 + threadIdx.x;
  if (i >= m) return;
#pragma unroll
  for (int a = 0; a < 3; ++a) q[3LL * i + a] = __fadd_rn(cl[3LL * i + a], ol[3LL * i + a]);
  qb[i] = static_cast<int32_t>(vc[4LL * i]);
}
__global__ void __launch_bounds__(256) pp_append_kernel(const int32_t *__restrict__ pairs, int rows,
                                                       const int32_t *__restrict__ offs, int n_prop,
                                                       const int32_t *__restrict__ obj, int prop_base, int row_base,
                                                       int32_t *__restrict__ out_pairs, int32_t *__restrict__ out_offs) {
  const int i = blockIdx.x * 256 + threadIdx.x;
  if (i < rows) {
    out_pairs[2LL * (row_base + i)] = pairs[2LL * i] + prop_base;
    out_pairs[2LL * (row_base + i) + 1] = obj[pairs[2LL * i + 1]];
  }
  if (i < n_prop) out_offs[prop_base + 1 + i] = offs[i + 1] + row_base;
  if (i == 0 && prop_base == 0) out_offs[0] = 0;
}

struct ScanArena {
  char *base;
  size_t cap, off;
  bool ok = true;
  ScanArena(void *p, size_t n) : base(static_cast<char *>(p)), cap(n), off(0) {}
  template <typename T>
  T *take(size_t count) {
    const size_t bytes = align_up((count ? count : 1) * sizeof(T));
    const size_t at = off;
    off += bytes;
    if (off > cap) {
      ok = false;
      return nullptr;
    }
    return reinterpret_cast<T *>(base + at);
  }
  size_t at(const void *p) const { return static_cast<size_t>(static_cast<const char *>(p) - base); }
};

__global__ void __launch_bounds__(64) read_back_kernel(const int32_t *__restrict__ dev, int words, int32_t *host) {
  if (static_cast<int>(threadIdx.x) < words)
    __hip_atomic_store(host + threadIdx.x, dev[threadIdx.x], __ATOMIC_RELAXED, __HIP_MEMORY_SCOPE_SYSTEM);
}
static int read_back(int32_t *host, const int32_t *dev, int words, hipStream_t stream, const char *what) {
  static const bool by_kernel = getenv("SG_READBACK_KERNEL") && atoi(getenv("SG_READBACK_KERNEL")) != 0;
  if (by_kernel && words <= 64) {
    read_back_kernel<<<1, 64, 0, stream>>>(dev, words, host);
    if (hipStreamSynchronize(stream) != hipSuccess) {
      set_error("%s: device -> host read-back failed", what);
      return SG_ERR_LAUNCH;
    }
    return SG_OK;
  }
  if (hipMemcpyAsync(host, dev, sizeof(int32_t) * words, hipMemcpyDeviceToHost, stream) != hipSuccess ||
      hipStreamSynchronize(stream) != hipSuccess) {
    set_error("%s: device -> host read-back failed", what);
    return SG_ERR_LAUNCH;
  }
  return SG_OK;
}

#define SG_TRY(expr)              \
  do {                            \
    const int rc_ = (expr);       \
    if (rc_ != SG_OK) return rc_; \
  } while (0)
#define SG_TAKE(var, T, count)                                                                    \
  T *var = ar.take<T>(count);                                                                     \
  if (var == nullptr) {                                                                           \
    res->arena_needed = ar.off + ar.off / 2 + (8 << 20);                                          \
    set_error("%s: arena too small (%zu bytes, need about %zu)", kWhat, ar.cap, res->arena_needed); \
    return SG_ERR_WORKSPACE;                                                                      \
  }

thread_local void (*t_scan_emit_hook)(void *) = nullptr;
thread_local void *t_scan_emit_ctx = nullptr;

}

using namespace sg;

static int voxelise_proposals(const sg_grouping_cfg *cfg, const int32_t *pairs, const int32_t *poff, int n_prop, int S,
                              const float *coords_float, const float *point_feats, ScanArena &ar, int32_t *meta,
                              int32_t *host, sg_grouping_result *res, sg_stream_t stream_, const char *kWhat) {
  hipStream_t stream = as_stream(stream_);
  const int C = cfg->feat_channels;
  SG_TAKE(cscale, float, n_prop);
  SG_TAKE(lo_s, float, 3 * static_cast<size_t>(n_prop));
  SG_TAKE(vox, int64_t, 4 * static_cast<size_t>(S));
  SG_TAKE(bad, int32_t, 64);
  hipMemsetAsync(bad, 0, sizeof(int32_t), stream);
  const float inv_ss = 1.0f / static_cast<float>(cfg->voxel_shape);
  proposal_box_kernel<<<n_prop < 1024 ? n_prop : 1024, 256, 0, stream>>>(pairs, poff, n_prop, coords_float, inv_ss,
                                                                        cfg->voxel_scale, cscale, lo_s);
  proposal_voxel_coords_kernel<<<grid_for(S, 256), 256, 0, stream>>>(pairs, S, coords_float, cscale, lo_s,
                                                                    cfg->voxel_shape, vox, bad);
  const size_t vx_bytes = sg_voxelize_idx_workspace_bytes(S);
  SG_TAKE(vx_ws, char, vx_bytes);
  SG_TAKE(inp_map, int32_t, S);
  SG_TRY(sg_voxelize_idx_build(vox, S, 4, 4, inp_map, meta + 40, vx_ws, vx_bytes, stream_));
  hipMemcpyAsync(meta + 42, bad, sizeof(int32_t), hipMemcpyDeviceToDevice, stream);
  SG_TRY(read_back(host, meta + 40, 3, stream, kWhat));
  const int M = host[0], mA = host[1];
  SG_REQUIRE(host[2] == 0, "%s: a proposal voxel coordinate fell outside [0, %d) "
             "(the reference asserts here, softgroup.py:698)", kWhat, cfg->voxel_shape);
  res->n_voxels = M;
  res->max_active = mA;
  SG_TAKE(vc64, int64_t, 4 * static_cast<size_t>(M));
  SG_TAKE(rules, int32_t, static_cast<size_t>(M) * (mA + 1));
  SG_TRY(sg_voxelize_idx_fill(vox, S, 4, 4, inp_map, M, mA, vc64, rules, vx_ws, vx_bytes, stream_));
  SG_TAKE(vc32, int32_t, 4 * static_cast<size_t>(M));
  SG_TAKE(vox_off, int32_t, static_cast<size_t>(n_prop) + 1);
  SG_TAKE(vfeat, float, static_cast<size_t>(M) * C);
  proposal_voxel_pack_kernel<<<grid_for(M, 256), 256, 0, stream>>>(vc64, M, n_prop, vc32, vox_off);
  proposal_voxel_feats_kernel<<<grid_for(static_cast<int64_t>(M) * C, 256), 256, 0, stream>>>(
      point_feats, pairs, rules, M, mA, C, vfeat);
  res->voxel_coords = ar.at(vc32);
  res->voxel_offsets = ar.at(vox_off);
  res->voxel_feats = ar.at(vfeat);
  res->point_to_voxel = ar.at(inp_map);
  res->arena_used = ar.off;
  return check_launch(kWhat);
}

extern "C" {

int sg_scan_grouping(const sg_grouping_cfg *cfg, const float *scores, const float *pt_offsets,
                     const float *coords_float, const int32_t *batch_idxs, const float *point_feats,
                     void *arena, size_t arena_bytes, sg_grouping_result *res, sg_stream_t stream_) {
  static const char *kWhat = "sg_scan_grouping";
  SG_REQUIRE(cfg != nullptr && res != nullptr, "sg_scan_grouping: null descriptor");
  SG_REQUIRE(cfg->n_points >= 0 && cfg->n_sem_classes >= 1 && cfg->n_seg >= 0 && cfg->n_seg <= kMaxSeg &&
                 cfg->batch_size >= 1 && cfg->feat_channels >= 1 && cfg->voxel_shape >= 0,
             "sg_scan_grouping: bad configuration (n_seg must be <= %d)", kMaxSeg);
  memset(res, 0, sizeof(*res));
  hipStream_t stream = as_stream(stream_);
  int32_t *host = pinned_words();
  SG_REQUIRE(host != nullptr, "sg_scan_grouping: no pinned host words");
  ScanArena ar(arena, arena_bytes);
  const int n = cfg->n_points, n_seg = cfg->n_seg;
  if (n == 0 || n_seg == 0) return SG_OK;

  const int n_blocks = (n + kSelBlock - 1) / kSelBlock;
  SG_TAKE(meta, int32_t, 64);
  SG_TAKE(blk_cnt, int32_t, static_cast<size_t>(n_seg) * n_blocks);
  SG_TAKE(blk_off, int32_t, static_cast<size_t>(n_seg) * n_blocks);
  select_count_kernel<<<n_blocks, kSelBlock, 0, stream>>>(scores, n, cfg->n_sem_classes, cfg->seg_class, n_seg,
                                                         cfg->score_thr, n_blocks, blk_cnt);
  select_scan_kernel<<<1, 1024, 0, stream>>>(blk_cnt, n_seg, n_blocks, cfg->min_npoint, blk_off, meta);
  SG_TRY(check_launch(kWhat));
  SG_TRY(read_back(host, meta, 1, stream, kWhat));
  const int n_sel = host[0];
  res->n_selected = n_sel;
  if (n_sel == 0) return SG_OK;
  SG_TAKE(obj, int32_t, n_sel);
  SG_TAKE(seg_of, int32_t, n_sel);
  SG_TAKE(pts, float, 3 * static_cast<size_t>(n_sel));
  SG_TAKE(key, int32_t, n_sel);
  select_emit_kernel<<<n_blocks, kSelBlock, 0, stream>>>(scores, n, cfg->n_sem_classes, cfg->seg_class, n_seg,
                                                        cfg->score_thr, n_blocks, blk_off, coords_float,
                                                        pt_offsets, batch_idxs, cfg->batch_size, obj, seg_of,
                                                        pts, key);

  const size_t bq_bytes = sg_ballquery_workspace_bytes(n_sel);
  SG_TAKE(bq_ws, char, bq_bytes);
  SG_TAKE(start_len, int32_t, 2 * static_cast<size_t>(n_sel));
  const size_t sc_bytes = sg_scan_workspace_bytes(n_sel);
  SG_TAKE(sc_ws, char, sc_bytes);
  hipMemsetAsync(start_len, 0, sizeof(int32_t) * 2 * n_sel, stream);
  SG_TRY(sg_ballquery_build_grid(pts, key, n_sel, cfg->radius, bq_ws, bq_bytes, stream_));
  SG_TRY(sg_ballquery_count(pts, key, n_sel, cfg->radius, start_len, nullptr, bq_ws, bq_bytes, stream_));
  SG_TRY(sg_exclusive_scan_startlen(start_len, n_sel, meta + 32, sc_ws, sc_bytes, stream_));
  SG_TRY(read_back(host, meta + 32, 1, stream, kWhat));
  const int n_active = host[0];
  res->n_neighbours = n_active;
  SG_TAKE(bq_idx, int32_t, n_active);
  SG_TRY(sg_ballquery_fill(pts, key, n_sel, cfg->radius, start_len, bq_idx, bq_ws, bq_bytes, stream_));

  const size_t bfs_bytes = sg_bfs_workspace_bytes(n_sel, n_active);
  SG_TAKE(bfs_ws, char, bfs_bytes);
  int32_t n_prop = 0, S = 0;
  SG_TRY(sg_bfs_cluster_label(bq_idx, start_len, n_sel, n_active, SG_LISTS_SORTED | SG_LISTS_RADIUS, seg_of,
                              cfg->seg_thr, n_seg, &n_prop, &S, bfs_ws, bfs_bytes, stream_));
  res->n_proposals = n_prop;
  res->sum_npoint = S;
  if (S == 0) return SG_OK;
  SG_TAKE(pairs, int32_t, 2 * static_cast<size_t>(S));
  SG_TAKE(poff, int32_t, static_cast<size_t>(n_prop) + 1);
  hipMemsetAsync(poff, 0, sizeof(int32_t) * (n_prop + 1), stream);
  if (t_scan_emit_hook != nullptr) t_scan_emit_hook(t_scan_emit_ctx);
  SG_TRY(sg_bfs_cluster_emit(bq_idx, start_len, n_sel, n_active, seg_of, cfg->seg_thr, n_prop, S, pairs, poff,
                             bfs_ws, bfs_bytes, stream_));
  proposal_map_kernel<<<grid_for(S, 256), 256, 0, stream>>>(pairs, S, obj);
  res->proposals_idx = ar.at(pairs);
  res->proposals_offset = ar.at(poff);
  if (cfg->voxel_shape == 0) {
    res->arena_used = ar.off;
    return check_launch(kWhat);
  }

  return voxelise_proposals(cfg, pairs, poff, n_prop, S, coords_float, point_feats, ar, meta, host, res, stream_, kWhat);
}

int sg_scan_grouping_pp(const sg_grouping_pp_cfg *pcfg, const float *scores, const float *pt_offsets,
                        const float *coords_float, const int32_t *batch_idxs, const float *point_feats,
                        void *arena, size_t arena_bytes, sg_grouping_result *res, sg_stream_t stream_) {
  static const char *kWhat = "sg_scan_grouping_pp";
  SG_REQUIRE(pcfg != nullptr && res != nullptr, "sg_scan_grouping_pp: null descriptor");
  const sg_grouping_cfg *cfg = &pcfg->base;
  SG_REQUIRE(cfg->n_points >= 0 && cfg->n_sem_classes >= 1 && cfg->n_seg >= 0 && cfg->n_seg <= kMaxSeg &&
                 cfg->batch_size >= 1 && cfg->feat_channels >= 1 && cfg->voxel_shape >= 0,
             "sg_scan_grouping_pp: bad configuration (n_seg must be <= %d)", kMaxSeg);
  SG_REQUIRE(pcfg->radius > 0 && (!pcfg->with_pyramid || pcfg->base_size > 0),
             "sg_scan_grouping_pp: radius and pyramid_base_size must be positive");
  memset(res, 0, sizeof(*res));
  hipStream_t stream = as_stream(stream_);
  int32_t *host = pinned_words();
  SG_REQUIRE(host != nullptr, "sg_scan_grouping_pp: no pinned host words");
  ScanArena ar(arena, arena_bytes);
  const int n = cfg->n_points, n_seg = cfg->n_seg;
  if (n == 0 || n_seg == 0) return SG_OK;

  const int n_blocks = (n + kSelBlock - 1) / kSelBlock;
  SG_TAKE(meta, int32_t, 128);
  SG_TAKE(blk_cnt, int32_t, static_cast<size_t>(n_seg) * n_blocks);
  SG_TAKE(blk_off, int32_t, static_cast<size_t>(n_seg) * n_blocks);
  select_count_kernel<<<n_blocks, kSelBlock, 0, stream>>>(scores, n, cfg->n_sem_classes, cfg->seg_class, n_seg,
                                                         cfg->score_thr, n_blocks, blk_cnt);
  select_scan_kernel<<<1, 1024, 0, stream>>>(blk_cnt, n_seg, n_blocks, cfg->min_npoint, blk_off, meta);
  SG_TRY(check_launch(kWhat));
  SG_TRY(read_back(host, meta, 1 + n_seg, stream, kWhat));
  const int n_sel = host[0];
  int count[kMaxSeg];
  for (int s = 0; s < n_seg; ++s) count[s] = host[1 + s];
  res->n_selected = n_sel;
  if (n_sel == 0) return SG_OK;
  SG_TAKE(obj, int32_t, n_sel);
  SG_TAKE(seg_of, int32_t, n_sel);
  SG_TAKE(pts, float, 3 * static_cast<size_t>(n_sel));
  SG_TAKE(key, int32_t, n_sel);
  select_emit_kernel<<<n_blocks, kSelBlock, 0, stream>>>(scores, n, cfg->n_sem_classes, cfg->seg_class, n_seg,
                                                        cfg->score_thr, n_blocks, blk_off, coords_float,
                                                        pt_offsets, batch_idxs, cfg->batch_size, obj, seg_of,
                                                        pts, key);
  SG_TAKE(pairs, int32_t, 2 * static_cast<size_t>(n_sel));
  SG_TAKE(poff, int32_t, static_cast<size_t>(n_sel) + 2);
  int n_prop = 0, S = 0;
  int64_t n_nbr = 0;
  const size_t loop_mark0 = ar.off;
  size_t loop_mark = loop_mark0;
  bool hook_pending = t_scan_emit_hook != nullptr;
  const bool defer_on = !(getenv("SG_PP_DEFER") && atoi(getenv("SG_PP_DEFER")) == 0);
  BfsDefer def;
  int def_rows = -1;
  bool def_mapped = false;
  struct DeferGuard {
    BfsDefer &d;
    ~DeferGuard() {
      if (d.deferred && d.side != nullptr) hipStreamSynchronize(d.side);
    }
  } defer_guard{def};
  int s0 = 0;
  for (int s = 0; s < n_seg; s0 += count[s], ++s) {
    const int nc_pts = count[s];
    if (nc_pts == 0) continue;
    ar.off = loop_mark;
    int level = 1;
    if (pcfg->with_pyramid) level = nc_pts > 1000000 ? 3 : nc_pts > 100000 ? 2 : 1;
    const float radius = static_cast<float>(pcfg->with_pyramid ? pcfg->radius * level : pcfg->radius);
    const bool mapped = pcfg->with_pyramid && (level > 1 || !pcfg->lvl_fusion);
    const float *q = pts + 3 * static_cast<size_t>(s0);
    const int32_t *qb = key + s0;
    int n_q = nc_pts, n_lvl = 0;
    const int32_t *l2p = nullptr;
    if (mapped) {
      const float inv = 1.0f / static_cast<float>(pcfg->base_size * level);
      SG_TAKE(vox, int64_t, 4 * static_cast<size_t>(nc_pts));
      SG_TAKE(c3, float, 3 * static_cast<size_t>(nc_pts));
      SG_TAKE(o3, float, 3 * static_cast<size_t>(nc_pts));
      pp_level_inputs_kernel<<<grid_for(nc_pts, 256, 1 << 22), 256, 0, stream>>>(obj + s0, nc_pts, coords_float, pt_offsets,
                                                                            batch_idxs, inv, vox, c3, o3);
      const size_t vx_bytes = sg_voxelize_idx_workspace_bytes(nc_pts);
      SG_TAKE(vx_ws, char, vx_bytes);
      SG_TAKE(l2p_, int32_t, nc_pts);
      SG_TRY(sg_voxelize_idx_build(vox, nc_pts, 4, 4, l2p_, meta + 40, vx_ws, vx_bytes, stream_));
      SG_TRY(read_back(host, meta + 40, 2, stream, kWhat));
      const int M = host[0], mA = host[1];
      SG_TAKE(vc64, int64_t, 4 * static_cast<size_t>(M));
      SG_TAKE(rules, int32_t, static_cast<size_t>(M) * (mA + 1));
      SG_TRY(sg_voxelize_idx_fill(vox, nc_pts, 4, 4, l2p_, M, mA, vc64, rules, vx_ws, vx_bytes, stream_));
      SG_TAKE(cl, float, 3 * static_cast<size_t>(M));
      SG_TAKE(ol, float, 3 * static_cast<size_t>(M));
      SG_TAKE(ql, float, 3 * static_cast<size_t>(M));
      SG_TAKE(qbl, int32_t, M);
      SG_TRY(sg_voxelize_fp(c3, rules, M, mA, 3, 1, cl, stream_));
      SG_TRY(sg_voxelize_fp(o3, rules, M, mA, 3, 1, ol, stream_));
      pp_level_points_kernel<<<grid_for(M, 256, 1 << 22), 256, 0, stream>>>(cl, ol, vc64, M, ql, qbl);
      q = ql;
      qb = qbl;
      n_q = n_lvl = M;
      l2p = l2p_;
    }
    SG_TAKE(start_len, int32_t, 2 * static_cast<size_t>(n_q));
    const size_t sc_bytes = sg_scan_workspace_bytes(n_q);
    SG_TAKE(sc_ws, char, sc_bytes);
    hipMemsetAsync(start_len, 0, sizeof(int32_t) * 2 * n_q, stream);
    int32_t *bq_idx = nullptr;
    int n_active = 0, flags = 0;
    if (pcfg->with_octree) {
      SG_TAKE(boxes, float, (1 + 8 + 64 + 512) * 6);
      SG_TAKE(pt_inds, int32_t, n_q);
      SG_TAKE(pt_sl, int32_t, 512 * 2);
      const size_t ob = sg_octree_build_workspace_bytes(n_q);
      SG_TAKE(o_ws, char, ob);
      SG_TAKE(stash, int32_t, octree_stash_bytes(n_q) / sizeof(int32_t));
      SG_TRY(sg_octree_build(q, n_q, boxes, pt_inds, pt_sl, o_ws, ob, stream_));
      SG_TRY(octree_ballquery_count_stash(q, boxes, pt_inds, pt_sl, n_q, radius, start_len, stash, stream));
      SG_TRY(sg_exclusive_scan_startlen(start_len, n_q, meta + 56, sc_ws, sc_bytes, stream_));
      SG_TRY(read_back(host, meta + 56, 1, stream, kWhat));
      n_active = host[0];
      SG_TAKE(idx_, int32_t, n_active);
      SG_TRY(octree_ballquery_fill_stash(q, boxes, pt_inds, pt_sl, n_q, radius, start_len, stash, idx_, stream));
      bq_idx = idx_;
      flags = SG_LISTS_RADIUS;
    } else {
      const size_t bq_bytes = sg_ballquery_workspace_bytes(n_q);
      SG_TAKE(bq_ws, char, bq_bytes);
      SG_TRY(sg_ballquery_build_grid(q, qb, n_q, radius, bq_ws, bq_bytes, stream_));
      SG_TRY(sg_ballquery_count(q, qb, n_q, radius, start_len, nullptr, bq_ws, bq_bytes, stream_));
      SG_TRY(sg_exclusive_scan_startlen(start_len, n_q, meta + 56, sc_ws, sc_bytes, stream_));
      SG_TRY(read_back(host, meta + 56, 1, stream, kWhat));
      n_active = host[0];
      SG_TAKE(idx_, int32_t, n_active);
      SG_TRY(sg_ballquery_fill(q, qb, n_q, radius, start_len, idx_, bq_ws, bq_bytes, stream_));
      bq_idx = idx_;
      flags = SG_LISTS_SORTED | SG_LISTS_RADIUS;
    }
    n_nbr += n_active;
    const size_t bfs_bytes = sg_bfs_workspace_bytes(n_q, n_active);
    SG_TAKE(bfs_ws, char, bfs_bytes);
    int32_t nc = 0, sp = 0;
    SG_TRY(sg_bfs_cluster_label(bq_idx, start_len, n_q, n_active, flags, nullptr, cfg->seg_thr + s, 1, &nc, &sp, bfs_ws,
                                bfs_bytes, stream_));
    if (sp == 0) continue;
    bool later = false;
    for (int t = s + 1; t < n_seg; ++t) later = later || count[t] > 0;
    const bool want_defer = defer_on && def_rows < 0 && later && bfs_label_max_kept(bfs_ws) > kBfsGiantMin;
    int rows = sp;
    if (want_defer && mapped) {
      SG_TRY(bfs_count_kept_members(bfs_ws, bfs_bytes, n_q, n_active, l2p, nc_pts, cfg->seg_thr + s, meta + 72, stream));
      SG_TRY(read_back(host, meta + 72, 1, stream, kWhat));
      rows = host[0];
    }
    SG_TAKE(cidx, int32_t, 2 * static_cast<size_t>(sp));
    SG_TAKE(coff, int32_t, static_cast<size_t>(nc) + 1);
    hipMemsetAsync(coff, 0, sizeof(int32_t) * (nc + 1), stream);
    if (hook_pending) {
      t_scan_emit_hook(t_scan_emit_ctx);
      hook_pending = false;
    }
    if (want_defer) bfs_emit_defer(&def);
    SG_TRY(sg_bfs_cluster_emit(bq_idx, start_len, n_q, n_active, nullptr, cfg->seg_thr + s, nc, sp, cidx, coff, bfs_ws,
                               bfs_bytes, stream_));
    const bool deferred = want_defer && def.deferred;
    hipStream_t tail = deferred ? def.side : stream;
    const int32_t *src_idx = cidx, *src_off = coff;
    if (mapped) {
      SG_TAKE(oidx, int32_t, 2 * static_cast<size_t>(nc_pts));
      SG_TAKE(ooff, int32_t, static_cast<size_t>(nc) + 1);
      const size_t ib = sg_pyramid_inverse_map_workspace_bytes(nc_pts, n_lvl, nc);
      SG_TAKE(i_ws, char, ib);
      SG_TRY(sg_pyramid_inverse_map(cidx, sp, nc, l2p, nc_pts, n_lvl, oidx, ooff, deferred ? meta + 80 : meta + 48, i_ws,
                                    ib, reinterpret_cast<sg_stream_t>(tail)));
      if (!deferred) {
        SG_TRY(read_back(host, meta + 48, 1, stream, kWhat));
        rows = host[0];
      }
      src_idx = oidx;
      src_off = ooff;
    }
    if (deferred) {
      def_rows = rows;
      def_mapped = mapped;
      loop_mark = ar.off;
    }
    if (rows == 0) continue;
    SG_REQUIRE(S + rows <= n_sel, "sg_scan_grouping_pp: more proposal rows than selected points");
    pp_append_kernel<<<grid_for(rows > nc ? rows : nc, 256, 1 << 22), 256, 0, tail>>>(src_idx, rows, src_off, nc, obj + s0,
                                                                                  n_prop, S, pairs, poff);
    n_prop += nc;
    S += rows;
  }
  res->deferred_classes = def_rows >= 0 ? 1 : 0;
  if (def.deferred) {
    SG_TRY(bfs_emit_join(def, stream));
    def.deferred = false;
    if (def_mapped) {
      SG_TRY(read_back(host, meta + 80, 1, stream, kWhat));
      SG_REQUIRE(host[0] == def_rows, "sg_scan_grouping_pp: the deferred class's rows were predicted as %d, the inverse map made %d",
                 def_rows, host[0]);
    }
  }
  ar.off = loop_mark0;
  res->n_neighbours = static_cast<int>(n_nbr < 0x7fffffff ? n_nbr : 0x7fffffff);
  res->n_proposals = n_prop;
  res->sum_npoint = S;
  if (S == 0) return check_launch(kWhat);
  res->proposals_idx = ar.at(pairs);
  res->proposals_offset = ar.at(poff);
  if (cfg->voxel_shape == 0) {
    res->arena_used = ar.off;
    return check_launch(kWhat);
  }
  return voxelise_proposals(cfg, pairs, poff, n_prop, S, coords_float, point_feats, ar, meta, host, res, stream_, kWhat);
}

int sg_scan_instances(const sg_instances_cfg *cfg, const int32_t *proposals_idx, const float *mask_scores,
                      const float *cls_prob, const float *iou_scores, void *arena, size_t arena_bytes,
                      void *host_out, size_t host_bytes, sg_instances_result *res, sg_stream_t stream_) {
  static const char *kWhat = "sg_scan_instances";
  SG_REQUIRE(cfg != nullptr && res != nullptr, "sg_scan_instances: null descriptor");
  SG_REQUIRE(cfg->n_classes >= 1 && cfg->score_stride >= cfg->n_classes && cfg->n_proposals >= 0 &&
                 cfg->sum_npoint >= 0 && cfg->n_points >= 0,
             "sg_scan_instances: bad configuration");
  memset(res, 0, sizeof(*res));
  hipStream_t stream = as_stream(stream_);
  int32_t *host = pinned_words();
  SG_REQUIRE(host != nullptr, "sg_scan_instances: no pinned host words");
  ScanArena ar(arena, arena_bytes);
  const int nP = cfg->n_proposals, nc = cfg->n_classes, stride = cfg->score_stride;
  const int64_t S = cfg->sum_npoint;
  if (nP == 0 || S == 0) return SG_OK;
  SG_TAKE(npoint, int32_t, static_cast<size_t>(nP) * nc);
  SG_TAKE(inst_of, int32_t, static_cast<size_t>(nP) * nc);
  SG_TAKE(kept_cls, int32_t, static_cast<size_t>(nP) * nc);
  SG_TAKE(kept_score, float, static_cast<size_t>(nP) * nc);
  SG_TAKE(head, int32_t, 64);
  SG_TRY(sg_instance_npoint(proposals_idx, mask_scores, S, stride, nc, cfg->mask_score_thr, nP, npoint, stream_));
  instance_keep_kernel<<<1, 1024, 0, stream>>>(cls_prob, iou_scores, stride, npoint, nP, nc, cfg->cls_score_thr,
                                             cfg->min_npoint, inst_of, kept_cls, kept_score, head);
  SG_TRY(check_launch(kWhat));
  SG_TRY(read_back(host, head, 2, stream, kWhat));
  const int n_kept = host[0];
  const int64_t cap = host[1] > 0 ? host[1] : 1;
  res->n_kept = n_kept;
  if (n_kept == 0) return SG_OK;
  SG_TAKE(starts, int32_t, cap);
  SG_TAKE(ends, int32_t, cap);
  SG_TAKE(bounds, int64_t, static_cast<size_t>(n_kept) + 1);
  const size_t rws_bytes = sg_instance_runs_workspace_bytes(n_kept, cfg->n_points);
  SG_TAKE(rws, char, rws_bytes);
  SG_TRY(sg_instance_runs(proposals_idx, mask_scores, S, stride, nc, cfg->mask_score_thr, inst_of, nP, n_kept,
                          cfg->n_points, starts, ends, bounds, cap, rws, rws_bytes, stream_));
  const int64_t tcap = sg_rle_format_device_text_bytes(cap, cfg->n_points);
  SG_TAKE(text, uint8_t, static_cast<size_t>(tcap));
  SG_TAKE(text_off, int64_t, static_cast<size_t>(n_kept) + 1);
  const size_t fws_bytes = sg_rle_format_device_workspace_bytes(cap);
  SG_TAKE(fws, char, fws_bytes);
  SG_TRY(sg_rle_format_device(starts, ends, bounds, n_kept, cap, cfg->n_points, text, tcap, text_off, fws,
                              fws_bytes, stream_));
  const size_t off_cls = sizeof(int64_t) * (static_cast<size_t>(n_kept) + 1);
  const size_t off_score = off_cls + sizeof(int32_t) * static_cast<size_t>(n_kept);
  const size_t off_text = align_up(off_score + sizeof(float) * static_cast<size_t>(n_kept), 8);
  res->host_needed = off_text + static_cast<size_t>(tcap);
  if (host_out == nullptr || host_bytes < off_text + 16) {
    set_error("sg_scan_instances: host buffer too small (%zu bytes, need up to %zu)", host_bytes, res->host_needed);
    return SG_ERR_WORKSPACE;
  }
  char *h = static_cast<char *>(host_out);
  if (hipMemcpyAsync(h, text_off, off_cls, hipMemcpyDeviceToHost, stream) != hipSuccess ||
      hipMemcpyAsync(h + off_cls, kept_cls, sizeof(int32_t) * n_kept, hipMemcpyDeviceToHost, stream) != hipSuccess ||
      hipMemcpyAsync(h + off_score, kept_score, sizeof(float) * n_kept, hipMemcpyDeviceToHost, stream) != hipSuccess ||
      hipStreamSynchronize(stream) != hipSuccess) {
    set_error("sg_scan_instances: result copy failed");
    return SG_ERR_LAUNCH;
  }
  const int64_t text_bytes = reinterpret_cast<const int64_t *>(h)[n_kept];
  res->host_needed = off_text + static_cast<size_t>(text_bytes);
  if (host_bytes < res->host_needed) {
    set_error("sg_scan_instances: host buffer too small (%zu bytes, need %zu)", host_bytes, res->host_needed);
    return SG_ERR_WORKSPACE;
  }
  if (text_bytes > 0 &&
      (hipMemcpyAsync(h + off_text, text, static_cast<size_t>(text_bytes), hipMemcpyDeviceToHost, stream) != hipSuccess ||
       hipStreamSynchronize(stream) != hipSuccess)) {
    set_error("sg_scan_instances: text copy failed");
    return SG_ERR_LAUNCH;
  }
  res->bits = ar.at(rws);
  res->label_id = ar.at(kept_cls);
  res->off_class = off_cls;
  res->off_score = off_score;
  res->off_text = off_text;
  res->text_bytes = static_cast<size_t>(text_bytes);
  res->arena_used = ar.off;
  return SG_OK;
}

}
```

### softgroup_amd/csrc/scan_forward.hip

```cpp
#include <stdlib.h>
#include <string.h>
#include <condition_variable>

#include <map>
#include <mutex>
#include <utility>

#include "common.h"
#include "heads.h"

#define SG_TRY_(expr)             \
  do {                            \
    const int rc_ = (expr);       \
    if (rc_ != SG_OK) return rc_; \
  } while (0)

namespace sg {

extern thread_local void (*t_scan_emit_hook)(void *);
extern thread_local void (*t_unet_conv_hook)(void *);
extern thread_local void *t_unet_conv_ctx;
extern thread_local void *t_scan_emit_ctx;

__global__ void __launch_bounds__(256) voxelize_cat_kernel(const float *__restrict__ a, int ca,
                                                          const float *__restrict__ b, int cb,
                                                          const int32_t *__restrict__ rules, int M, int max_active,
                                                          float *__restrict__ out) {
  const int C = ca + cb;
  const int64_t total = static_cast<int64_t>(M) * C;
  for (int64_t t = blockIdx.x * 256LL + threadIdx.x; t < total; t += gridDim.x * 256LL) {
    const int row = static_cast<int>(t / C), p = static_cast<int>(t - static_cast<int64_t>(row) * C);
    const float *src = p < ca ? a + p : b + (p - ca);
    const int pitch = p < ca ? ca : cb;
    const int32_t *r = rules + static_cast<int64_t>(row) * (max_active + 1);
    const int cnt = r[0];
    const float m = cnt > 0 ? __fdiv_rn(1.0f, static_cast<float>(cnt)) : 1.0f;
    float acc = 0.0f;
    int i = 1;
    for (; i + 3 <= cnt; i += 4) {
      const int a0 = r[i], a1 = r[i + 1], a2 = r[i + 2], a3 = r[i + 3];
      const float f0 = src[static_cast<int64_t>(a0) * pitch], f1 = src[static_cast<int64_t>(a1) * pitch],
                  f2 = src[static_cast<int64_t>(a2) * pitch], f3 = src[static_cast<int64_t>(a3) * pitch];
      acc = __fadd_rn(acc, __fmul_rn(m, f0));
      acc = __fadd_rn(acc, __fmul_rn(m, f1));
      acc = __fadd_rn(acc, __fmul_rn(m, f2));
      acc = __fadd_rn(acc, __fmul_rn(m, f3));
    }
    for (; i <= cnt; ++i) acc = __fadd_rn(acc, __fmul_rn(m, src[static_cast<int64_t>(r[i]) * pitch]));
    out[t] = acc;
  }
}

__global__ void __launch_bounds__(256) narrow_i64_kernel(const int64_t *__restrict__ in, int64_t n,
                                                        int32_t *__restrict__ out) {
  for (int64_t i = blockIdx.x * 256LL + threadIdx.x; i < n; i += gridDim.x * 256LL) out[i] = static_cast<int32_t>(in[i]);
}

template <int COLS_MAX>
__global__ void __launch_bounds__(256) softmax_rows_kernel(const float *__restrict__ x, int64_t rows, int cols,
                                                          float *__restrict__ out) {
  const int64_t r = blockIdx.x * 256LL + threadIdx.x;
  if (r >= rows) return;
  float e[32];
  float mx = -INFINITY;
#pragma unroll
  for (int j = 0; j < COLS_MAX; ++j) {
    e[j] = j < cols ? x[r * cols + j] : -INFINITY;
    mx = fmaxf(mx, e[j]);
  }
#pragma unroll
  for (int j = 0; j < 32; ++j) e[j] = j < COLS_MAX ? expf(e[j] - mx) : 0.f;
  float s[32];
#pragma unroll
  for (int j = 0; j < 32; ++j) s[j] = e[j];
#pragma unroll
  for (int off = 16; off > 0; off >>= 1) {
    float t[32];
#pragma unroll
    for (int j = 0; j < 32; ++j) t[j] = __fadd_rn(s[j], s[j ^ off]);
#pragma unroll
    for (int j = 0; j < 32; ++j) s[j] = t[j];
  }
  const float sum = s[0];
#pragma unroll
  for (int j = 0; j < COLS_MAX; ++j)
    if (j < cols) out[r * cols + j] = __fdiv_rn(e[j], sum);
}

template <int C>
__global__ void __launch_bounds__(256) mlp_rows_kernel(const float *__restrict__ feats, const int32_t *__restrict__ idx,
                                                      int64_t rows, Mlp2 m, float *__restrict__ out) {
  const int64_t r = blockIdx.x * 256LL + threadIdx.x;
  if (r >= rows) return;
  const int64_t row = idx ? static_cast<int64_t>(idx[r]) : r;
  float x[C];
  const float4 *src = reinterpret_cast<const float4 *>(feats + row * C);
#pragma unroll
  for (int q = 0; q < C / 4; ++q) {
    const float4 v = src[q];
    x[4 * q] = v.x; x[4 * q + 1] = v.y; x[4 * q + 2] = v.z; x[4 * q + 3] = v.w;
  }
  float y[32];
  mlp2<C, 32>(x, m, y);
#pragma unroll
  for (int o = 0; o < 32; ++o)
    if (o < m.out) out[r * m.out + o] = y[o];
}

__global__ void __launch_bounds__(256) linear_rows_kernel(const float *__restrict__ x, int64_t rows,
                                                         const float *__restrict__ w, const float *__restrict__ b,
                                                         int n_out, int n_in, float *__restrict__ out) {
  const int64_t total = rows * n_out;
  for (int64_t t = blockIdx.x * 256LL + threadIdx.x; t < total; t += gridDim.x * 256LL) {
    const int64_t r = t / n_out;
    const int j = static_cast<int>(t - r * n_out);
    float a = b ? b[j] : 0.f;
    for (int c = 0; c < n_in; ++c) a = fmaf(x[r * n_in + c], w[static_cast<int64_t>(j) * n_in + c], a);
    out[t] = a;
  }
}

__global__ void __launch_bounds__(256) gt_instances_kernel(const int64_t *__restrict__ sem, const int64_t *__restrict__ inst,
                                                          int n, int64_t shift, int64_t *__restrict__ out) {
  for (int i = blockIdx.x * 256 + threadIdx.x; i < n; i += gridDim.x * 256) {
    int64_t s = sem[i] - shift + 1;
    if (s < 0) s = 0;
    const int64_t k = inst[i] + 1;
    out[i] = k < 0 ? 0 : s * 1000 + k;
  }
}

struct PackList {
  const char *src[SG_SCAN_DENSE_MAX];
  size_t dst[SG_SCAN_DENSE_MAX], bytes[SG_SCAN_DENSE_MAX];
  int n;
};
__global__ void __launch_bounds__(256) pack_segments_kernel(PackList p, char *__restrict__ out) {
  const int s = blockIdx.y;
  const char *src = p.src[s];
  char *dst = out + p.dst[s];
  const size_t nb = p.bytes[s];
  if ((reinterpret_cast<uintptr_t>(src) & 15) == 0) {
    const size_t q = nb / 16;
    const uint4 *s4 = reinterpret_cast<const uint4 *>(src);
    uint4 *d4 = reinterpret_cast<uint4 *>(dst);
    for (size_t i = blockIdx.x * 256ull + threadIdx.x; i < q; i += gridDim.x * 256ull) d4[i] = s4[i];
    if (blockIdx.x == 0)
      for (size_t i = q * 16 + threadIdx.x; i < nb; i += 256) dst[i] = src[i];
  } else {
    for (size_t i = blockIdx.x * 256ull + threadIdx.x; i < nb; i += gridDim.x * 256ull) dst[i] = src[i];
  }
}

typedef unsigned u32x4 __attribute__((ext_vector_type(4)));
__global__ void __launch_bounds__(256) d2h_copy_kernel(const u32x4 *__restrict__ src, u32x4 *__restrict__ dst, size_t n16) {
  for (size_t i = blockIdx.x * 256ull + threadIdx.x; i < n16; i += gridDim.x * 256ull)
    __builtin_nontemporal_store(src[i], dst + i);
}

struct ScanStream {
  hipStream_t copy = nullptr;
  hipEvent_t packed = nullptr, copied = nullptr, backbone_done = nullptr;
};
static std::mutex g_backbone_mu[16];
static hipEvent_t g_backbone_last[16];
struct BackboneSem {
  std::mutex m;
  std::condition_variable cv;
  int in_use = 0;
};
static BackboneSem g_backbone_sem[16];
static int backbone_permits() {
  static const int p = getenv("SG_SCAN_TOKEN_PERMITS") ? atoi(getenv("SG_SCAN_TOKEN_PERMITS")) : 2;
  return p < 1 ? 1 : p;
}
struct BackboneToken {
  int dev;
  hipStream_t stream;
  std::unique_lock<std::mutex> lock;
  bool taken = false;
  bool sem = false;
};
static void backbone_token_take(void *ctx) {
  BackboneToken *t = static_cast<BackboneToken *>(ctx);
  if (t->sem) {
    BackboneSem &s = g_backbone_sem[t->dev];
    std::unique_lock<std::mutex> g(s.m);
    s.cv.wait(g, [&] { return s.in_use < backbone_permits(); });
    ++s.in_use;
    t->taken = true;
    return;
  }
  t->lock = std::unique_lock<std::mutex>(g_backbone_mu[t->dev]);
  t->taken = true;
  if (g_backbone_last[t->dev] != nullptr) hipStreamWaitEvent(t->stream, g_backbone_last[t->dev], 0);
}
static void backbone_token_give(BackboneToken *t) {
  if (!t->taken) return;
  if (t->sem) {
    BackboneSem &s = g_backbone_sem[t->dev];
    {
      std::lock_guard<std::mutex> g(s.m);
      --s.in_use;
    }
    s.cv.notify_one();
  } else {
    t->lock.unlock();
  }
  t->taken = false;
}
static std::mutex g_scan_mu;
static std::map<std::pair<int, hipStream_t>, ScanStream> g_scan_streams;

static ScanStream *scan_stream(hipStream_t stream) {
  int dev = 0;
  if (hipGetDevice(&dev) != hipSuccess) return nullptr;
  std::lock_guard<std::mutex> g(g_scan_mu);
  ScanStream &s = g_scan_streams[{dev, stream}];
  if (s.copy == nullptr) {
    if (hipStreamCreateWithFlags(&s.copy, hipStreamNonBlocking) != hipSuccess ||
        hipEventCreateWithFlags(&s.packed, hipEventDisableTiming) != hipSuccess ||
        hipEventCreateWithFlags(&s.copied, hipEventDisableTiming) != hipSuccess ||
        hipEventCreateWithFlags(&s.backbone_done, hipEventDisableTiming) != hipSuccess) {
      s = ScanStream();
      return nullptr;
    }
  }
  return &s;
}

void scan_release_stream(int dev, hipStream_t stream) {
  std::lock_guard<std::mutex> g(g_scan_mu);
  auto it = g_scan_streams.find({dev, stream});
  if (it == g_scan_streams.end()) return;
  if (it->second.copy) {
    hipStreamSynchronize(it->second.copy);
    hipStreamDestroy(it->second.copy);
    hipEventDestroy(it->second.packed);
    hipEventDestroy(it->second.copied);
    if (dev >= 0 && dev < 16) {
      std::lock_guard<std::mutex> b(g_backbone_mu[dev]);
      if (g_backbone_last[dev] == it->second.backbone_done) g_backbone_last[dev] = nullptr;
    }
    hipEventDestroy(it->second.backbone_done);
  }
  g_scan_streams.erase(it);
}

struct DenseCopy {
  ScanStream *ss;
  hipStream_t main;
  const void *dev_block;
  void *host_block;
  size_t bytes;
  bool issued, failed;
};
static void start_dense_copy(void *ctx) {
  DenseCopy *d = static_cast<DenseCopy *>(ctx);
  if (d->issued || d->bytes == 0) return;
  d->issued = true;
  static const int d2h_wgs = getenv("SG_SCAN_D2H_WGS") ? atoi(getenv("SG_SCAN_D2H_WGS")) : 0;
  static const bool side = !(getenv("SG_SCAN_COPY_STREAM") && atoi(getenv("SG_SCAN_COPY_STREAM")) == 0);
  hipStream_t cs = side ? d->ss->copy : d->main;
  if (side && (hipEventRecord(d->ss->packed, d->main) != hipSuccess ||
               hipStreamWaitEvent(d->ss->copy, d->ss->packed, 0) != hipSuccess)) {
    d->failed = true;
    return;
  }
  if (d2h_wgs > 0 && d->bytes % 16 == 0) {
    d2h_copy_kernel<<<d2h_wgs, 256, 0, cs>>>(static_cast<const u32x4 *>(d->dev_block),
                                             static_cast<u32x4 *>(d->host_block), d->bytes / 16);
    if (hipGetLastError() != hipSuccess) d->failed = true;
  } else if (hipMemcpyAsync(d->host_block, d->dev_block, d->bytes, hipMemcpyDeviceToHost, cs) != hipSuccess) {
    d->failed = true;
  }
  if (hipEventRecord(d->ss->copied, cs) != hipSuccess) d->failed = true;
}

static Mlp2 as_mlp(const sg_mlp2 &m) { return Mlp2{m.w1, m.b1, m.bn_scale, m.bn_shift, m.w2, m.b2, m.out}; }

struct Carve {
  char *base;
  size_t cap, off;
  Carve(void *p, size_t n) : base(static_cast<char *>(p)), cap(n), off(0) {}
  template <typename T>
  T *take(size_t count) {
    const size_t bytes = align_up((count ? count : 1) * sizeof(T));
    const size_t at = off;
    off += bytes;
    return off > cap ? nullptr : reinterpret_cast<T *>(base + at);
  }
  size_t at(const void *p) const { return static_cast<size_t>(static_cast<const char *>(p) - base); }
};

}

using namespace sg;

extern "C" {

int sg_softmax_rows(const float *x, int64_t rows, int cols, float *out, sg_stream_t stream) {
  SG_REQUIRE(rows >= 0 && cols >= 1 && cols <= 32 && x && out, "sg_softmax_rows: rows of 1..32 columns (got %d)", cols);
  if (rows == 0) return SG_OK;
  const int grid = static_cast<int>((rows + 255) / 256);
  if (cols <= 4) softmax_rows_kernel<4><<<grid, 256, 0, as_stream(stream)>>>(x, rows, cols, out);
  else if (cols <= 8) softmax_rows_kernel<8><<<grid, 256, 0, as_stream(stream)>>>(x, rows, cols, out);
  else if (cols <= 16) softmax_rows_kernel<16><<<grid, 256, 0, as_stream(stream)>>>(x, rows, cols, out);
  else softmax_rows_kernel<32><<<grid, 256, 0, as_stream(stream)>>>(x, rows, cols, out);
  return check_launch("sg_softmax_rows");
}

int sg_mlp_rows(const float *feats, const int32_t *idx, int64_t rows, int channels, const sg_mlp2 *mlp, float *out,
                sg_stream_t stream) {
  SG_REQUIRE(rows >= 0 && mlp && feats && out, "sg_mlp_rows: bad arguments");
  SG_REQUIRE(channels == 16 || channels == 32, "sg_mlp_rows: channels must be 16 or 32 (got %d)", channels);
  SG_REQUIRE(mlp->out >= 1 && mlp->out <= 32, "sg_mlp_rows: head width %d out of range", mlp->out);
  if (rows == 0) return SG_OK;
  const int grid = static_cast<int>((rows + 255) / 256);
  if (channels == 32) mlp_rows_kernel<32><<<grid, 256, 0, as_stream(stream)>>>(feats, idx, rows, as_mlp(*mlp), out);
  else mlp_rows_kernel<16><<<grid, 256, 0, as_stream(stream)>>>(feats, idx, rows, as_mlp(*mlp), out);
  return check_launch("sg_mlp_rows");
}

int sg_linear_rows(const float *x, int64_t rows, const sg_linear *lin, float *out, sg_stream_t stream) {
  SG_REQUIRE(rows >= 0 && lin && lin->w && lin->out >= 1 && lin->in >= 1 && x && out, "sg_linear_rows: bad arguments");
  if (rows == 0) return SG_OK;
  linear_rows_kernel<<<grid_for(rows * lin->out, 256), 256, 0, as_stream(stream)>>>(x, rows, lin->w, lin->b, lin->out,
                                                                                  lin->in, out);
  return check_launch("sg_linear_rows");
}

size_t sg_scan_arena_bytes(const sg_scan_desc *d, int n_points, int n_voxels) {
  if (d == nullptr || d->backbone == nullptr) return 0;
  const size_t N = static_cast<size_t>(n_points > 0 ? n_points : 1), M = static_cast<size_t>(n_voxels > 0 ? n_voxels : 1);
  const size_t C = static_cast<size_t>(d->channels), ns = static_cast<size_t>(d->semantic_classes);
  size_t p = align_up(M * 16) + align_up(M * 8 * 4) + align_up(M * C * 4) + align_up(N * C * 4) + 2 * align_up(N * ns * 4) +
             align_up(N * 12) + 2 * align_up(N * 8) + align_up(N * 96) + (1 << 20);
  size_t bb = sg_unet_arena_bytes(d->backbone, n_voxels) / 4;
  if (bb < (64u << 20)) bb = 64u << 20;
  const size_t later = (160u << 20) + N * 256;
  return p + (bb > later ? bb : later) + (8 << 20);
}

int sg_scan_forward(const sg_scan_desc *d, const sg_scan_input *in, void *arena, size_t arena_bytes, void *host_dense,
                    size_t host_dense_bytes, void *host_inst, size_t host_inst_bytes, sg_scan_result *res,
                    sg_stream_t stream_) {
  static const char *kWhat = "sg_scan_forward";
  SG_REQUIRE(d && in && res && d->backbone, "sg_scan_forward: null descriptor");
  SG_REQUIRE(!d->want_instances || d->tiny, "sg_scan_forward: instances need the tiny U-Net's descriptor");
  SG_REQUIRE(d->channels == 16 || d->channels == 32, "sg_scan_forward: backbone channels must be 16 or 32");
  SG_REQUIRE(d->semantic.out == d->semantic_classes && d->semantic_classes >= 1 && d->semantic_classes <= 32,
             "sg_scan_forward: 1..32 semantic classes");
  SG_REQUIRE(in->n_points >= 0 && in->n_voxels >= 0 && in->max_active >= 0 && in->batch_size >= 1 && in->feat_dim >= 1,
             "sg_scan_forward: bad input sizes");
  SG_REQUIRE(in->n_dense >= 0 && in->n_dense <= SG_SCAN_DENSE_MAX, "sg_scan_forward: at most %d dense items",
             SG_SCAN_DENSE_MAX);
  memset(res, 0, sizeof(*res));
  hipStream_t stream = as_stream(stream_);
  const int N = in->n_points, M = in->n_voxels, C = d->channels, ns = d->semantic_classes;
  const int cin = in->feat_dim + (d->with_coords ? 3 : 0);
  SG_REQUIRE(d->backbone->input_w == nullptr ? cin == C : cin == d->backbone->input_cin,
             "sg_scan_forward: %d feature columns, the backbone takes %d", cin,
             d->backbone->input_w ? d->backbone->input_cin : C);
  if (N == 0 || M == 0) return SG_OK;
  ScanStream *ss = scan_stream(stream);
  SG_REQUIRE(ss != nullptr, "sg_scan_forward: side stream / event creation failed");
  Carve ar(arena, arena_bytes);
#define SG_CARVE(var, T, count)                                                                          \
  T *var = ar.take<T>(count);                                                                            \
  if (var == nullptr) {                                                                                  \
    res->arena_needed = ar.off + ar.off / 4 + (64u << 20);                                               \
    set_error("%s: arena too small (%zu bytes, need about %zu)", kWhat, ar.cap, res->arena_needed);      \
    return SG_ERR_WORKSPACE;                                                                             \
  }

  const int32_t *vc32 = static_cast<const int32_t *>(in->voxel_coords);
  if (in->voxel_coords_is_int64) {
    SG_CARVE(vc, int32_t, static_cast<size_t>(M) * 4);
    narrow_i64_kernel<<<grid_for(static_cast<int64_t>(M) * 4, 256), 256, 0, stream>>>(
        static_cast<const int64_t *>(in->voxel_coords), static_cast<int64_t>(M) * 4, vc);
    vc32 = vc;
  }
  SG_CARVE(vfeat, float, static_cast<size_t>(M) * cin);
  SG_CARVE(bb_out, float, static_cast<size_t>(M) * C);
  SG_CARVE(out_feats, float, static_cast<size_t>(N) * C);
  SG_CARVE(sem, float, static_cast<size_t>(N) * ns);
  SG_CARVE(prob, float, static_cast<size_t>(N) * ns);
  SG_CARVE(off, float, static_cast<size_t>(N) * 3);
  SG_CARVE(preds, int64_t, N);
  PackList pl;
  pl.n = 0;
  size_t dense_total = 0;
  bool want_gt = false;
  for (int i = 0; i < in->n_dense; ++i) {
    const sg_scan_dense_item &it = in->dense[i];
    size_t nb = 0;
    switch (it.kind) {
      case 0: nb = it.bytes; SG_REQUIRE(it.ptr != nullptr || nb == 0, "sg_scan_forward: dense item %d has no source", i); break;
      case 1: nb = static_cast<size_t>(N) * 8; break;
      case 2: nb = static_cast<size_t>(N) * 12; break;
      case 3:
        nb = static_cast<size_t>(N) * 8;
        want_gt = true;
        SG_REQUIRE(in->semantic_labels && in->instance_labels, "sg_scan_forward: gt_instances need the label arrays");
        break;
      case 4: nb = static_cast<size_t>(N) * ns * 4; break;
      default: SG_REQUIRE(false, "sg_scan_forward: dense item %d: unknown kind %d", i, it.kind);
    }
    res->dense_offset[i] = dense_total;
    pl.dst[i] = dense_total;
    pl.bytes[i] = nb;
    dense_total += align_up(nb);
  }
  pl.n = in->n_dense;
  res->dense_bytes = dense_total;
  res->host_dense_needed = dense_total;
  if (dense_total > 0 && (host_dense == nullptr || host_dense_bytes < dense_total)) {
    set_error("%s: host block for the dense results too small (%zu bytes, need %zu)", kWhat, host_dense_bytes, dense_total);
    return SG_ERR_WORKSPACE;
  }
  int64_t *gt = nullptr;
  if (want_gt) {
    SG_CARVE(gt_, int64_t, N);
    gt = gt_;
  }
  SG_CARVE(dense_dev, char, dense_total);
  for (int i = 0; i < in->n_dense; ++i) {
    switch (in->dense[i].kind) {
      case 0: pl.src[i] = static_cast<const char *>(in->dense[i].ptr); break;
      case 1: pl.src[i] = reinterpret_cast<const char *>(preds); break;
      case 2: pl.src[i] = reinterpret_cast<const char *>(off); break;
      case 3: pl.src[i] = reinterpret_cast<const char *>(gt); break;
      default: pl.src[i] = reinterpret_cast<const char *>(sem); break;
    }
  }
  res->voxel_feats_in = ar.at(vfeat);
  res->backbone_out = ar.at(bb_out);
  res->output_feats = ar.at(out_feats);
  res->semantic_scores = ar.at(sem);
  res->semantic_prob = ar.at(prob);
  res->pt_offsets = ar.at(off);
  res->semantic_preds = ar.at(preds);

  static const int token_env = getenv("SG_SCAN_TOKEN") ? atoi(getenv("SG_SCAN_TOKEN")) : 4;
  int token_mode = 0;
  int dev = 0;
  if (token_env != 0 && hipGetDevice(&dev) == hipSuccess && dev >= 0 && dev < 16) {
    std::lock_guard<std::mutex> g(g_scan_mu);
    int n = 0;
    for (const auto &kv : g_scan_streams) n += kv.first.first == dev;
    if (n > 1) token_mode = token_env;
  }
  const bool use_token = token_mode == 3;
  std::unique_lock<std::mutex> token;
  if (use_token) token = std::unique_lock<std::mutex>(g_backbone_mu[dev]);
  BackboneToken bt{dev, stream, {}, false, token_mode == 4};
  struct TokenHookScope {
    BackboneToken &t;
    ~TokenHookScope() {
      t_unet_conv_hook = nullptr;
      t_unet_conv_ctx = nullptr;
      if (t.sem) backbone_token_give(&t);
    }
  } token_hook_scope{bt};
  if (token_mode == 1 || token_mode == 2 || token_mode == 4) {
    t_unet_conv_hook = backbone_token_take;
    t_unet_conv_ctx = &bt;
  }
  voxelize_cat_kernel<<<grid_for(static_cast<int64_t>(M) * cin, 256), 256, 0, stream>>>(
      in->feats, in->feat_dim, d->with_coords ? in->coords_float : nullptr, d->with_coords ? 3 : 0, in->p2v_map, M,
      in->max_active, vfeat);
  SG_TRY_(check_launch(kWhat));
  {
    const size_t room = arena_bytes > ar.off ? arena_bytes - ar.off : 0;
    const int rc = sg_unet_forward(d->backbone, vfeat, vc32, M, in->spatial_shape, bb_out,
                                   static_cast<char *>(arena) + ar.off, room, stream_);
    if (rc == SG_ERR_WORKSPACE) res->arena_needed = ar.off + sg_unet_arena_bytes(d->backbone, M) + (64u << 20);
    SG_TRY_(rc);
  }
  SG_TRY_(sg_pointwise_heads(bb_out, in->v2p_map, in->v2p_is_int64, N, C, &d->semantic, &d->offset, out_feats, sem, off,
                             preds, stream_));
  if (want_gt)
    gt_instances_kernel<<<grid_for(N, 256, 1024), 256, 0, stream>>>(in->semantic_labels, in->instance_labels, N,
                                                                  static_cast<int64_t>(d->semantic_classes - d->instance_classes), gt);
  if (pl.n > 0) {
    size_t mx = 0;
    for (int i = 0; i < pl.n; ++i) mx = pl.bytes[i] > mx ? pl.bytes[i] : mx;
    pack_segments_kernel<<<dim3(grid_for(static_cast<int64_t>(mx / 16 + 1), 256, 512), pl.n), 256, 0, stream>>>(pl, dense_dev);
  }
  SG_TRY_(check_launch(kWhat));
  if (bt.taken) {
    if (hipEventRecord(ss->backbone_done, stream) == hipSuccess) {
      if (!bt.sem) g_backbone_last[dev] = ss->backbone_done;
      if (token_mode == 1 || token_mode == 4) hipEventSynchronize(ss->backbone_done);
    }
    backbone_token_give(&bt);
  }
  DenseCopy dc{ss, stream, dense_dev, host_dense, dense_total, false, false};
  struct DenseGuard {
    DenseCopy &d;
    ~DenseGuard() {
      if (d.issued && !d.failed && d.bytes > 0) hipEventSynchronize(d.ss->copied);
    }
  } dense_guard{dc};
  res->stage = 1;
  auto finish_dense = [&]() -> int {
    start_dense_copy(&dc);
    if (dc.failed || (dc.bytes > 0 && hipEventSynchronize(ss->copied) != hipSuccess)) {
      set_error("%s: copy of the dense results failed", kWhat);
      return SG_ERR_LAUNCH;
    }
    return SG_OK;
  };
  if (!d->want_instances) {
    res->arena_used = ar.off;
    SG_TRY_(finish_dense());
    if (hipStreamSynchronize(stream) != hipSuccess) return SG_ERR_LAUNCH;
    return SG_OK;
  }
  SG_TRY_(sg_softmax_rows(sem, N, ns, prob, stream_));
  if (use_token) {
    if (hipEventRecord(ss->backbone_done, stream) != hipSuccess || hipEventSynchronize(ss->backbone_done) != hipSuccess) {
      set_error("%s: waiting for the backbone failed", kWhat);
      return SG_ERR_LAUNCH;
    }
    token.unlock();
  }

  sg_grouping_cfg gc = d->grouping;
  gc.n_points = N;
  gc.n_sem_classes = ns;
  gc.batch_size = in->batch_size;
  gc.feat_channels = C;
  res->grouping_base = ar.off;
  {
    struct HookScope {
      HookScope(void (*f)(void *), void *c) { t_scan_emit_hook = f; t_scan_emit_ctx = c; }
      ~HookScope() { t_scan_emit_hook = nullptr; t_scan_emit_ctx = nullptr; }
    } hook(start_dense_copy, &dc);
    const size_t room = arena_bytes > ar.off ? arena_bytes - ar.off : 0;
    int rc;
    if (d->with_pyramid || d->with_octree) {
      sg_grouping_pp_cfg pc;
      memset(&pc, 0, sizeof(pc));
      pc.base = gc;
      pc.with_pyramid = d->with_pyramid;
      pc.with_octree = d->with_octree;
      pc.lvl_fusion = 0;
      pc.radius = d->pp_radius;
      pc.base_size = d->pp_base_size;
      rc = sg_scan_grouping_pp(&pc, prob, off, in->coords_float, in->batch_idxs, out_feats,
                               static_cast<char *>(arena) + ar.off, room, &res->grouping, stream_);
    } else {
      rc = sg_scan_grouping(&gc, prob, off, in->coords_float, in->batch_idxs, out_feats,
                            static_cast<char *>(arena) + ar.off, room, &res->grouping, stream_);
    }
    if (rc == SG_ERR_WORKSPACE) res->arena_needed = ar.off + res->grouping.arena_needed + (64u << 20);
    if (rc != SG_OK) return rc;
  }
  res->stage = 2;
  const sg_grouping_result &g = res->grouping;
  if (g.sum_npoint == 0) {
    res->arena_used = ar.off;
    SG_TRY_(finish_dense());
    if (hipStreamSynchronize(stream) != hipSuccess) return SG_ERR_LAUNCH;
    return SG_OK;
  }
  char *gbase = static_cast<char *>(arena) + res->grouping_base;
  ar.off += align_up(g.arena_used);
  const int nP = g.n_proposals, Mv = g.n_voxels;
  const int64_t S = g.sum_npoint;
  const int32_t *pairs = reinterpret_cast<const int32_t *>(gbase + g.proposals_idx);
  const int32_t *pvc = reinterpret_cast<const int32_t *>(gbase + g.voxel_coords);
  const int32_t *pvoff = reinterpret_cast<const int32_t *>(gbase + g.voxel_offsets);
  const float *pvfeat = reinterpret_cast<const float *>(gbase + g.voxel_feats);
  const int32_t *p2v = reinterpret_cast<const int32_t *>(gbase + g.point_to_voxel);

  const int ncol = d->instance_classes + 1;
  SG_REQUIRE(d->mask.out == ncol && d->cls.out == ncol && d->iou.out == ncol && d->cls.in == C && d->iou.in == C,
             "sg_scan_forward: refinement heads must have instance_classes + 1 = %d outputs", ncol);
  SG_CARVE(tiny_out, float, static_cast<size_t>(Mv) * C);
  SG_CARVE(mask_scores, float, static_cast<size_t>(S) * ncol);
  SG_CARVE(pooled, float, static_cast<size_t>(nP) * C);
  SG_CARVE(cls, float, static_cast<size_t>(nP) * ncol);
  SG_CARVE(cls_prob, float, static_cast<size_t>(nP) * ncol);
  SG_CARVE(iou, float, static_cast<size_t>(nP) * ncol);
  {
    const size_t room = arena_bytes > ar.off ? arena_bytes - ar.off : 0;
    const int32_t shape[3] = {d->grouping.voxel_shape, d->grouping.voxel_shape, d->grouping.voxel_shape};
    const int rc = sg_unet_forward(d->tiny, pvfeat, pvc, Mv, shape, tiny_out, static_cast<char *>(arena) + ar.off, room,
                                   stream_);
    if (rc == SG_ERR_WORKSPACE) res->arena_needed = ar.off + sg_unet_arena_bytes(d->tiny, Mv) + (64u << 20);
    if (rc != SG_OK) return rc;
  }
  int rc = sg_mlp_rows(tiny_out, p2v, S, C, &d->mask, mask_scores, stream_);
  if (rc == SG_OK) rc = sg_global_avg_pool_fp(tiny_out, pvoff, nP, C, pooled, stream_);
  if (rc == SG_OK) rc = sg_linear_rows(pooled, nP, &d->cls, cls, stream_);
  if (rc == SG_OK) rc = sg_linear_rows(pooled, nP, &d->iou, iou, stream_);
  if (rc == SG_OK) rc = sg_softmax_rows(cls, nP, ncol, cls_prob, stream_);
  if (rc != SG_OK) return rc;
  res->tiny_out = ar.at(tiny_out);
  res->mask_scores = ar.at(mask_scores);
  res->cls_scores = ar.at(cls);
  res->cls_prob = ar.at(cls_prob);
  res->iou_scores = ar.at(iou);
  res->stage = 3;

  sg_instances_cfg ic;
  ic.n_proposals = nP;
  ic.n_classes = d->instance_classes;
  ic.score_stride = ncol;
  ic.sum_npoint = S;
  ic.n_points = N;
  ic.cls_score_thr = d->cls_score_thr;
  ic.mask_score_thr = d->mask_score_thr;
  ic.min_npoint = d->min_npoint;
  res->instances_base = ar.off;
  {
    const size_t room = arena_bytes > ar.off ? arena_bytes - ar.off : 0;
    rc = sg_scan_instances(&ic, pairs, mask_scores, cls_prob, iou, static_cast<char *>(arena) + ar.off, room, host_inst,
                           host_inst_bytes, &res->instances, stream_);
    res->host_inst_needed = res->instances.host_needed;
    if (rc == SG_ERR_WORKSPACE && res->instances.arena_needed > room)
      res->arena_needed = ar.off + res->instances.arena_needed + (16u << 20);
    if (rc != SG_OK) return rc;
  }
  res->stage = 4;
  res->arena_used = ar.off + res->instances.arena_used;
  SG_TRY_(finish_dense());
  return SG_OK;
#undef SG_CARVE
}

}
```

Before: 430.2.

## Fuse pointwise heads, softmax and grouping selection into one front kernel

Adds a fused pointwise_front kernel that runs the semantic and offset MLP heads with LDS staging, computes softmax probabilities and argmax, and emits per-point selection bitmasks plus per-block counts for grouping. Outputs are written directly into the dense output block, which removes separate pack copies, the standalone softmax launch and the selection pass inside grouping. It is on by default via an env toggle and adds arena space plus a more complex kernel with higher LDS use.

New measurement: 435.5 (median of 6 runs). 1.01x the previous value.

```diff
diff --git a/include/softgroup_hip.h b/include/softgroup_hip.h
--- a/include/softgroup_hip.h
+++ b/include/softgroup_hip.h
@@ -193,6 +193,11 @@
                        int channels, const sg_mlp2 *semantic, const sg_mlp2 *offset, float *output_feats,
                        float *semantic_scores, float *pt_offsets, int64_t *semantic_preds,
                        sg_stream_t stream);
+int sg_pointwise_front(const float *voxel_feats, const void *v2p_map, int v2p_is_int64, int n_points,
+                       int channels, const sg_mlp2 *semantic, const sg_mlp2 *offset, const int32_t *seg_class,
+                       int n_seg, float score_thr, float *output_feats, float *semantic_scores,
+                       float *semantic_prob, float *pt_offsets, int64_t *semantic_preds, uint32_t *sel_words,
+                       int32_t *blk_cnt, sg_stream_t stream);
 
 size_t sg_spconv_packed_weight_elems_bf16(int kvol, int cin, int cout);
 int sg_spconv_pack_weight_bf16(const float *w, int cout, int kvol, int cin, int src_is_kio,
@@ -379,6 +384,9 @@
                      const float *coords_float, const int32_t *batch_idxs, const float *point_feats,
                      void *arena, size_t arena_bytes, sg_grouping_result *result_host,
                      sg_stream_t stream);
+int sg_scan_select(const sg_grouping_cfg *cfg, int source, const float *scores, const uint32_t *sel_words,
+                   const int32_t *blk_cnt, const float *pt_offsets, const float *coords_float,
+                   const int32_t *batch_idxs, void *arena, size_t arena_bytes, size_t *out, sg_stream_t stream);
 
 typedef struct sg_grouping_pp_cfg {
   sg_grouping_cfg base;
@@ -479,6 +487,7 @@
 int sg_scan_forward(const sg_scan_desc *desc, const sg_scan_input *in, void *arena, size_t arena_bytes,
                     void *host_dense, size_t host_dense_bytes, void *host_inst, size_t host_inst_bytes,
                     sg_scan_result *result_host, sg_stream_t stream);
+int sg_scan_set_pointwise_fused(int mode);
 
 int sg_eval_intersections(const int32_t *run_start, const int64_t *run_off, const int32_t *run_pred,
                           int n_runs, int64_t total_points, const int32_t *gt_slot, int n_pred,
diff --git a/softgroup_amd/_lib.py b/softgroup_amd/_lib.py
--- a/softgroup_amd/_lib.py
+++ b/softgroup_amd/_lib.py
@@ -78,6 +78,7 @@
     'sg_unet_train_backward': (_i, [_vp, _vp, _vp, _vp]),
     'sg_unet_train_release': (None, [_vp]),
     'sg_pointwise_heads': (_i, [_vp, _vp, _i, _i, _i, _vp, _vp, _vp, _vp, _vp, _vp, _vp]),
+    'sg_pointwise_front': (_i, [_vp, _vp, _i, _i, _i, _vp, _vp, _vp, _i, _f, _vp, _vp, _vp, _vp, _vp, _vp, _vp, _vp]),
     'sg_spconv_packed_weight_elems': (_sz, [_i, _i, _i]),
     'sg_spconv_pack_weight': (_i, [_vp, _i, _i, _i, _i, _vp, _vp]),
     'sg_spconv_conv_workspace_bytes': (_sz, [_i, _i]),
@@ -116,12 +117,14 @@
     'sg_superpoint_vote': (_i, [_vp, _i64, _vp, _vp, _vp, _i64, _i, _i, _vp, _vp, _vp, _sz, _vp]),
     'sg_scan_grouping': (_i, [_vp, _vp, _vp, _vp, _vp, _vp, _vp, _sz, _vp, _vp]),
     'sg_scan_grouping_pp': (_i, [_vp, _vp, _vp, _vp, _vp, _vp, _vp, _sz, _vp, _vp]),
+    'sg_scan_select': (_i, [_vp, _i, _vp, _vp, _vp, _vp, _vp, _vp, _vp, _sz, _vp, _vp]),
     'sg_scan_instances': (_i, [_vp, _vp, _vp, _vp, _vp, _vp, _sz, _vp, _sz, _vp, _vp]),
     'sg_softmax_rows': (_i, [_vp, _i64, _i, _vp, _vp]),
     'sg_mlp_rows': (_i, [_vp, _vp, _i64, _i, _vp, _vp, _vp]),
     'sg_linear_rows': (_i, [_vp, _i64, _vp, _vp, _vp]),
     'sg_scan_arena_bytes': (_sz, [_vp, _i, _i]),
     'sg_scan_forward': (_i, [_vp, _vp, _vp, _sz, _vp, _sz, _vp, _sz, _vp, _vp]),
+    'sg_scan_set_pointwise_fused': (_i, [_i]),
     'sg_eval_intersections': (_i, [_vp, _vp, _vp, _i, _i64, _vp, _i, _i, _vp, _vp]),
     'sg_eval_tally_workspace_bytes': (_sz, [_i64]),
     'sg_eval_class_tally': (_i, [_vp, _i, _vp, _i, _i64, _i64, _i, _i, _vp, _vp, _i, _vp, _vp, _vp, _vp, _vp,
diff --git a/softgroup_amd/csrc/heads.h b/softgroup_amd/csrc/heads.h
--- a/softgroup_amd/csrc/heads.h
+++ b/softgroup_amd/csrc/heads.h
@@ -8,25 +8,75 @@
   int out;
 };
 
+typedef const float __attribute__((address_space(4))) *cfloat_p;
+__device__ __forceinline__ cfloat_p as_const(const float *p) { return (cfloat_p)(uintptr_t)p; }
+
+template <int C, typename P>
+__device__ __forceinline__ float mlp2_hidden(const float (&x)[C], P w1, P b1, P scale, P shift, int o) {
+  float a = b1[o];
+#pragma unroll
+  for (int c = 0; c < C; ++c) a = fmaf(x[c], w1[o * C + c], a);
+  return fmaxf(fmaf(a, scale[o], shift[o]), 0.f);
+}
+template <int C, typename P>
+__device__ __forceinline__ float mlp2_out(const float (&h)[C], P w2, P b2, int o) {
+  float a = b2[o];
+#pragma unroll
+  for (int c = 0; c < C; ++c) a = fmaf(h[c], w2[o * C + c], a);
+  return a;
+}
+
 template <int C, int OUT_MAX>
 __device__ __forceinline__ void mlp2(const float (&x)[C], const Mlp2 &m, float (&y)[OUT_MAX]) {
   float h[C];
 #pragma unroll
-  for (int o = 0; o < C; ++o) {
-    float a = m.b1[o];
-#pragma unroll
-    for (int c = 0; c < C; ++c) a = fmaf(x[c], m.w1[o * C + c], a);
-    h[o] = fmaxf(fmaf(a, m.scale[o], m.shift[o]), 0.f);
-  }
+  for (int o = 0; o < C; ++o) h[o] = mlp2_hidden<C>(x, m.w1, m.b1, m.scale, m.shift, o);
 #pragma unroll
   for (int o = 0; o < OUT_MAX; ++o) {
-    if (o < m.out) {
-      float a = m.b2[o];
-#pragma unroll
-      for (int c = 0; c < C; ++c) a = fmaf(h[c], m.w2[o * C + c], a);
-      y[o] = a;
-    }
+    if (o < m.out) y[o] = mlp2_out<C>(h, m.w2, m.b2, o);
   }
 }
 
+template <int OUT_MAX>
+__device__ __forceinline__ int argmax_first(const float (&y)[OUT_MAX], int n) {
+  float best = y[0];
+  int arg = 0;
+#pragma unroll
+  for (int o = 1; o < OUT_MAX; ++o) {
+    if (o < n && (y[o] > best || (y[o] != y[o] && best == best))) {
+      best = y[o];
+      arg = o;
+    }
+  }
+  return arg;
 }
+
+template <int COLS_MAX>
+__device__ __forceinline__ void softmax_row(float (&e)[32]) {
+  float mx = -INFINITY;
+#pragma unroll
+  for (int j = 0; j < COLS_MAX; ++j) mx = fmaxf(mx, e[j]);
+#pragma unroll
+  for (int j = 0; j < 32; ++j) e[j] = j < COLS_MAX ? expf(e[j] - mx) : 0.f;
+  float s[32];
+#pragma unroll
+  for (int j = 0; j < 32; ++j) s[j] = e[j];
+#pragma unroll
+  for (int off = 16; off > 0; off >>= 1) {
+    float t[32];
+#pragma unroll
+    for (int j = 0; j < 32; ++j) t[j] = __fadd_rn(s[j], s[j ^ off]);
+#pragma unroll
+    for (int j = 0; j < 32; ++j) s[j] = t[j];
+  }
+  const float sum = s[0];
+#pragma unroll
+  for (int j = 0; j < COLS_MAX; ++j) e[j] = __fdiv_rn(e[j], sum);
+}
+
+int pointwise_front(const float *vox, const void *v2p, int v2p_is_int64, int n, int channels, const Mlp2 &sem,
+                    const Mlp2 &off, const int32_t *seg_class, int n_seg, float score_thr, float *out_feats,
+                    float *sem_scores, float *sem_prob, float *pt_offsets, int64_t *sem_preds, uint32_t *sel_words,
+                    int32_t *blk_cnt, bool blk_cnt_zeroed, hipStream_t stream);
+
+}
diff --git a/softgroup_amd/csrc/heads.hip b/softgroup_amd/csrc/heads.hip
--- a/softgroup_amd/csrc/heads.hip
+++ b/softgroup_amd/csrc/heads.hip
@@ -54,6 +54,179 @@
                          float *sem_scores, float *pt_offsets, int64_t *sem_preds, hipStream_t st) {
   pointwise_heads_kernel<C, 32, IdxT><<<(n + 255) / 256, 256, 0, st>>>(vox, static_cast<const IdxT *>(v2p), n, s, o,
                                                                        out_feats, sem_scores, pt_offsets, sem_preds);
+}
+
+constexpr int kFrontPts = 64;
+constexpr int kFrontSelBlock = 256;
+
+struct FrontArgs {
+  const float *vox;
+  const void *v2p;
+  int n, n_seg, n_blocks;
+  float thr;
+  Mlp2 sem, off;
+  const int32_t *seg_class;
+  float *out_feats, *sem_scores, *sem_prob, *pt_offsets;
+  int64_t *sem_preds;
+  uint32_t *sel_words;
+  int32_t *blk_cnt;
+};
+
+__device__ __forceinline__ void store_staged(const float *lds, float *__restrict__ dst, int count, int t, int nt) {
+  const int q = count >> 2;
+  for (int i = t; i < q; i += nt) reinterpret_cast<float4 *>(dst)[i] = reinterpret_cast<const float4 *>(lds)[i];
+  for (int i = 4 * q + t; i < count; i += nt) dst[i] = lds[i];
+}
+
+template <int COLS_MAX>
+__device__ __forceinline__ void front_softmax(const float *row_lds, int ns, float *prob_lds, int *arg) {
+  float e[32];
+#pragma unroll
+  for (int j = 0; j < COLS_MAX; ++j) e[j] = j < ns ? row_lds[j] : -INFINITY;
+  float y[COLS_MAX];
+#pragma unroll
+  for (int j = 0; j < COLS_MAX; ++j) y[j] = e[j];
+  *arg = argmax_first<COLS_MAX>(y, ns);
+  softmax_row<COLS_MAX>(e);
+#pragma unroll
+  for (int j = 0; j < COLS_MAX; ++j)
+    if (j < ns) prob_lds[j] = e[j];
+}
+
+template <int C, typename IdxT>
+__global__ void __launch_bounds__(256) pointwise_front_kernel(const FrontArgs a) {
+  constexpr int XP = kFrontPts + 1;
+  constexpr int PQ = C / 4;
+  constexpr int HU = C / 4;
+  __shared__ __attribute__((aligned(16))) float XL[C * XP > kFrontPts * 32 ? C * XP : kFrontPts * 32];
+  __shared__ __attribute__((aligned(16))) float HP[kFrontPts * 32];
+  __shared__ __attribute__((aligned(16))) float HO[C * kFrontPts];
+  __shared__ __attribute__((aligned(16))) float OF[kFrontPts * 4];
+  const int tid = threadIdx.x, lane = tid & 63;
+  const int w = __builtin_amdgcn_readfirstlane(tid >> 6);
+  const int p0 = blockIdx.x * kFrontPts;
+  const int rows = min(kFrontPts, a.n - p0);
+  const int ns = a.sem.out, no = a.off.out;
+  const IdxT *v2p = static_cast<const IdxT *>(a.v2p);
+
+#pragma unroll
+  for (int i = tid; i < kFrontPts * PQ; i += 256) {
+    const int r = i / PQ, q = i % PQ;
+    float4 v = make_float4(0.f, 0.f, 0.f, 0.f);
+    if (r < rows) {
+      const int64_t p = p0 + r;
+      const int64_t row = v2p ? static_cast<int64_t>(v2p[p]) : p;
+      v = reinterpret_cast<const float4 *>(a.vox + row * C)[q];
+      reinterpret_cast<float4 *>(a.out_feats + p * C)[q] = v;
+    }
+    XL[(4 * q) * XP + r] = v.x;
+    XL[(4 * q + 1) * XP + r] = v.y;
+    XL[(4 * q + 2) * XP + r] = v.z;
+    XL[(4 * q + 3) * XP + r] = v.w;
+  }
+  __syncthreads();
+
+  {
+    float x[C];
+#pragma unroll
+    for (int c = 0; c < C; ++c) x[c] = XL[c * XP + lane];
+    const cfloat_p sw1 = as_const(a.sem.w1), sb1 = as_const(a.sem.b1), ssc = as_const(a.sem.scale), ssh = as_const(a.sem.shift);
+    const cfloat_p ow1 = as_const(a.off.w1), ob1 = as_const(a.off.b1), osc = as_const(a.off.scale), osh = as_const(a.off.shift);
+#pragma unroll
+    for (int j = 0; j < HU; ++j) {
+      const int o = w * HU + j;
+      HP[o * kFrontPts + lane] = mlp2_hidden<C>(x, sw1, sb1, ssc, ssh, o);
+    }
+#pragma unroll
+    for (int j = 0; j < HU; ++j) {
+      const int o = w * HU + j;
+      HO[o * kFrontPts + lane] = mlp2_hidden<C>(x, ow1, ob1, osc, osh, o);
+    }
+  }
+  __syncthreads();
+
+  {
+    float h[C];
+#pragma unroll
+    for (int c = 0; c < C; ++c) h[c] = HP[c * kFrontPts + lane];
+    const cfloat_p w2 = as_const(a.sem.w2), b2 = as_const(a.sem.b2);
+#pragma unroll
+    for (int j = 0; j < 8; ++j) {
+      const int o = w + 4 * j;
+      if (o < ns) XL[lane * ns + o] = mlp2_out<C>(h, w2, b2, o);
+    }
+    if (w < no) {
+#pragma unroll
+      for (int c = 0; c < C; ++c) h[c] = HO[c * kFrontPts + lane];
+      OF[lane * no + w] = mlp2_out<C>(h, as_const(a.off.w2), as_const(a.off.b2), w);
+    }
+  }
+  __syncthreads();
+
+  if (w == 0) {
+    int arg = 0;
+    if (ns <= 16) front_softmax<16>(XL + lane * ns, ns, HP + lane * ns, &arg);
+    else if (ns <= 24) front_softmax<24>(XL + lane * ns, ns, HP + lane * ns, &arg);
+    else front_softmax<32>(XL + lane * ns, ns, HP + lane * ns, &arg);
+    if (lane < rows) a.sem_preds[p0 + lane] = arg;
+  } else {
+    store_staged(XL, a.sem_scores + static_cast<int64_t>(p0) * ns, rows * ns, tid - 64, 192);
+    store_staged(OF, a.pt_offsets + static_cast<int64_t>(p0) * no, rows * no, tid - 64, 192);
+  }
+  __syncthreads();
+
+  store_staged(HP, a.sem_prob + static_cast<int64_t>(p0) * ns, rows * ns, tid, 256);
+  if (w == 3 && a.n_seg > 0) {
+    uint32_t word = 0;
+    int mine = 0;
+    for (int s = 0; s < a.n_seg; ++s) {
+      const bool on = lane < rows && HP[lane * ns + a.seg_class[s]] > a.thr;
+      word |= static_cast<uint32_t>(on) << s;
+      const int c = __popcll(__ballot(on));
+      if (lane == s) mine = c;
+    }
+    if (lane < rows) a.sel_words[p0 + lane] = word;
+    if (lane < a.n_seg && mine > 0) atomicAdd(a.blk_cnt + static_cast<int64_t>(lane) * a.n_blocks + p0 / kFrontSelBlock, mine);
+  }
+}
+
+template <int C, typename IdxT>
+static void launch_front(const FrontArgs &a, hipStream_t st) {
+  pointwise_front_kernel<C, IdxT><<<(a.n + kFrontPts - 1) / kFrontPts, 256, 0, st>>>(a);
+}
+
+int pointwise_front(const float *vox, const void *v2p, int v2p_is_int64, int n, int channels, const Mlp2 &sem,
+                    const Mlp2 &off, const int32_t *seg_class, int n_seg, float score_thr, float *out_feats,
+                    float *sem_scores, float *sem_prob, float *pt_offsets, int64_t *sem_preds, uint32_t *sel_words,
+                    int32_t *blk_cnt, bool blk_cnt_zeroed, hipStream_t stream) {
+  SG_REQUIRE(n >= 0 && vox && out_feats && sem_scores && sem_prob && pt_offsets && sem_preds,
+             "sg_pointwise_front: bad arguments");
+  SG_REQUIRE(channels == 16 || channels == 32, "sg_pointwise_front: channels must be 16 or 32 (got %d)", channels);
+  SG_REQUIRE(sem.out >= 1 && sem.out <= 32 && off.out >= 1 && off.out <= 4,
+             "sg_pointwise_front: head widths out of range (semantic %d, offset %d)", sem.out, off.out);
+  SG_REQUIRE(n_seg >= 0 && n_seg <= 32 && (n_seg == 0 || (seg_class && sel_words && blk_cnt)),
+             "sg_pointwise_front: 0..32 segments with their class list, words and counts");
+  SG_REQUIRE(((reinterpret_cast<uintptr_t>(vox) | reinterpret_cast<uintptr_t>(out_feats) |
+               reinterpret_cast<uintptr_t>(sem_scores) | reinterpret_cast<uintptr_t>(sem_prob) |
+               reinterpret_cast<uintptr_t>(pt_offsets)) & 15) == 0,
+             "sg_pointwise_front: float arrays must be 16-byte aligned");
+  if (n == 0) return SG_OK;
+  const int n_blocks = (n + kFrontSelBlock - 1) / kFrontSelBlock;
+  if (n_seg > 0 && !blk_cnt_zeroed &&
+      hipMemsetAsync(blk_cnt, 0, sizeof(int32_t) * static_cast<size_t>(n_seg) * n_blocks, stream) != hipSuccess) {
+    set_error("sg_pointwise_front: clearing the block counts failed");
+    return SG_ERR_LAUNCH;
+  }
+  const FrontArgs a{vox, v2p, n, n_seg, n_blocks, score_thr, sem, off, seg_class, out_feats, sem_scores, sem_prob,
+                    pt_offsets, sem_preds, sel_words, blk_cnt};
+  if (channels == 32) {
+    if (v2p_is_int64) launch_front<32, int64_t>(a, stream);
+    else launch_front<32, int32_t>(a, stream);
+  } else {
+    if (v2p_is_int64) launch_front<16, int64_t>(a, stream);
+    else launch_front<16, int32_t>(a, stream);
+  }
+  return check_launch("sg_pointwise_front");
 }
 
 }
@@ -81,3 +254,16 @@
   }
   return check_launch("sg_pointwise_heads");
 }
+
+extern "C" int sg_pointwise_front(const float *voxel_feats, const void *v2p_map, int v2p_is_int64, int n_points,
+                                  int channels, const sg_mlp2 *semantic, const sg_mlp2 *offset,
+                                  const int32_t *seg_class, int n_seg, float score_thr, float *output_feats,
+                                  float *semantic_scores, float *semantic_prob, float *pt_offsets,
+                                  int64_t *semantic_preds, uint32_t *sel_words, int32_t *blk_cnt, sg_stream_t stream) {
+  SG_REQUIRE(semantic && offset, "sg_pointwise_front: bad arguments");
+  const Mlp2 s{semantic->w1, semantic->b1, semantic->bn_scale, semantic->bn_shift, semantic->w2, semantic->b2, semantic->out};
+  const Mlp2 o{offset->w1, offset->b1, offset->bn_scale, offset->bn_shift, offset->w2, offset->b2, offset->out};
+  return pointwise_front(voxel_feats, v2p_map, v2p_is_int64, n_points, channels, s, o, seg_class, n_seg, score_thr,
+                         output_feats, semantic_scores, semantic_prob, pt_offsets, semantic_preds, sel_words, blk_cnt,
+                         false, as_stream(stream));
+}
diff --git a/softgroup_amd/csrc/scan_exec.hip b/softgroup_amd/csrc/scan_exec.hip
--- a/softgroup_amd/csrc/scan_exec.hip
+++ b/softgroup_amd/csrc/scan_exec.hip
@@ -143,6 +143,68 @@
       key[pos] = s * batch_size + bi;
     }
     __syncthreads();
+  }
+}
+
+__global__ void __launch_bounds__(kSelBlock) select_words_kernel(const float *__restrict__ scores, int n, int n_cls,
+                                                                const int32_t *__restrict__ seg_class, int n_seg,
+                                                                float thr, int n_blocks,
+                                                                uint32_t *__restrict__ words,
+                                                                int32_t *__restrict__ blk_cnt) {
+  __shared__ int part[4][kMaxSeg];
+  const int i = blockIdx.x * kSelBlock + threadIdx.x;
+  const int wave = threadIdx.x >> 6, lane = threadIdx.x & 63;
+  uint32_t word = 0;
+  for (int s = 0; s < n_seg; ++s) {
+    const bool on = i < n && scores[static_cast<int64_t>(i) * n_cls + seg_class[s]] > thr;
+    word |= static_cast<uint32_t>(on) << s;
+    const int c = __popcll(__ballot(on));
+    if (lane == 0) part[wave][s] = c;
+  }
+  if (i < n) words[i] = word;
+  __syncthreads();
+  if (threadIdx.x < n_seg)
+    blk_cnt[threadIdx.x * n_blocks + blockIdx.x] =
+        part[0][threadIdx.x] + part[1][threadIdx.x] + part[2][threadIdx.x] + part[3][threadIdx.x];
+}
+
+__global__ void __launch_bounds__(kSelBlock) select_emit_words_kernel(
+    const uint32_t *__restrict__ words, int n, int n_seg, int n_blocks, const int32_t *__restrict__ blk_off,
+    const float *__restrict__ coords, const float *__restrict__ offsets, const int32_t *__restrict__ batch_idxs,
+    int batch_size, int32_t *__restrict__ obj, int32_t *__restrict__ seg_of, float *__restrict__ pts,
+    int32_t *__restrict__ key) {
+  __shared__ int wcnt[2][4];
+  const int i = blockIdx.x * kSelBlock + threadIdx.x;
+  const int wave = threadIdx.x >> 6;
+  float c[3] = {0.f, 0.f, 0.f};
+  int bi = 0;
+  uint32_t word = 0;
+  if (i < n) {
+#pragma unroll
+    for (int a = 0; a < 3; ++a) c[a] = __fadd_rn(coords[3LL * i + a], offsets[3LL * i + a]);
+    bi = batch_idxs[i];
+    word = words[i];
+  }
+  int flip = 0;
+  for (int s = 0; s < n_seg; ++s) {
+    const int base = blk_off[s * n_blocks + blockIdx.x];
+    if (base < 0) continue;
+    const bool on = (word >> s) & 1u;
+    const uint64_t m = __ballot(on);
+    if ((threadIdx.x & 63) == 0) wcnt[flip][wave] = __popcll(m);
+    __syncthreads();
+    int before = 0;
+    for (int w = 0; w < wave; ++w) before += wcnt[flip][w];
+    flip ^= 1;
+    if (on) {
+      const int pos = base + before + mask_prefix(m);
+      obj[pos] = i;
+      seg_of[pos] = s;
+      pts[3LL * pos] = c[0];
+      pts[3LL * pos + 1] = c[1];
+      pts[3LL * pos + 2] = c[2];
+      key[pos] = s * batch_size + bi;
+    }
   }
 }
 
@@ -483,11 +545,72 @@
   return check_launch(kWhat);
 }
 
-extern "C" {
-
-int sg_scan_grouping(const sg_grouping_cfg *cfg, const float *scores, const float *pt_offsets,
-                     const float *coords_float, const int32_t *batch_idxs, const float *point_feats,
-                     void *arena, size_t arena_bytes, sg_grouping_result *res, sg_stream_t stream_) {
+enum { kSelFromScores = 0, kSelMakeWords = 1, kSelGivenWords = 2 };
+struct Selection {
+  int32_t *meta = nullptr, *obj = nullptr, *seg_of = nullptr, *key = nullptr;
+  float *pts = nullptr;
+  int n_sel = 0;
+};
+static int select_classes(const sg_grouping_cfg *cfg, int source, const float *scores, const uint32_t *sel_words,
+                          const int32_t *blk_cnt_in, const float *pt_offsets, const float *coords_float,
+                          const int32_t *batch_idxs, int meta_words, int read_words, ScanArena &ar, int32_t *host,
+                          size_t *arena_needed, Selection *sel, hipStream_t stream, const char *kWhat) {
+  struct {
+    size_t &arena_needed;
+  } res_{*arena_needed}, *res = &res_;
+  const int n = cfg->n_points, n_seg = cfg->n_seg;
+  const int n_blocks = (n + kSelBlock - 1) / kSelBlock;
+  SG_REQUIRE(source == kSelGivenWords ? (sel_words != nullptr && blk_cnt_in != nullptr) : scores != nullptr,
+             "%s: the class selection has no source", kWhat);
+  SG_TAKE(meta, int32_t, meta_words);
+  const int32_t *blk_cnt = blk_cnt_in;
+  if (source != kSelGivenWords) {
+    SG_TAKE(cnt, int32_t, static_cast<size_t>(n_seg) * n_blocks);
+    blk_cnt = cnt;
+    if (source == kSelMakeWords) {
+      SG_TAKE(words, uint32_t, n);
+      sel_words = words;
+      select_words_kernel<<<n_blocks, kSelBlock, 0, stream>>>(scores, n, cfg->n_sem_classes, cfg->seg_class, n_seg,
+                                                             cfg->score_thr, n_blocks, words, cnt);
+    } else {
+      select_count_kernel<<<n_blocks, kSelBlock, 0, stream>>>(scores, n, cfg->n_sem_classes, cfg->seg_class, n_seg,
+                                                             cfg->score_thr, n_blocks, cnt);
+    }
+  }
+  SG_TAKE(blk_off, int32_t, static_cast<size_t>(n_seg) * n_blocks);
+  select_scan_kernel<<<1, 1024, 0, stream>>>(blk_cnt, n_seg, n_blocks, cfg->min_npoint, blk_off, meta);
+  SG_TRY(check_launch(kWhat));
+  SG_TRY(read_back(host, meta, read_words, stream, kWhat));
+  const int n_sel = host[0];
+  sel->meta = meta;
+  sel->n_sel = n_sel;
+  if (n_sel == 0) return SG_OK;
+  SG_TAKE(obj, int32_t, n_sel);
+  SG_TAKE(seg_of, int32_t, n_sel);
+  SG_TAKE(pts, float, 3 * static_cast<size_t>(n_sel));
+  SG_TAKE(key, int32_t, n_sel);
+  if (source == kSelFromScores)
+    select_emit_kernel<<<n_blocks, kSelBlock, 0, stream>>>(scores, n, cfg->n_sem_classes, cfg->seg_class, n_seg,
+                                                          cfg->score_thr, n_blocks, blk_off, coords_float,
+                                                          pt_offsets, batch_idxs, cfg->batch_size, obj, seg_of,
+                                                          pts, key);
+  else
+    select_emit_words_kernel<<<n_blocks, kSelBlock, 0, stream>>>(sel_words, n, n_seg, n_blocks, blk_off, coords_float,
+                                                                pt_offsets, batch_idxs, cfg->batch_size, obj,
+                                                                seg_of, pts, key);
+  sel->obj = obj;
+  sel->seg_of = seg_of;
+  sel->pts = pts;
+  sel->key = key;
+  return SG_OK;
+}
+
+namespace sg {
+
+int scan_grouping_run(const sg_grouping_cfg *cfg, const float *scores, const uint32_t *sel_words,
+                      const int32_t *blk_cnt, const float *pt_offsets, const float *coords_float,
+                      const int32_t *batch_idxs, const float *point_feats, void *arena, size_t arena_bytes,
+                      sg_grouping_result *res, sg_stream_t stream_) {
   static const char *kWhat = "sg_scan_grouping";
   SG_REQUIRE(cfg != nullptr && res != nullptr, "sg_scan_grouping: null descriptor");
   SG_REQUIRE(cfg->n_points >= 0 && cfg->n_sem_classes >= 1 && cfg->n_seg >= 0 && cfg->n_seg <= kMaxSeg &&
@@ -501,26 +624,14 @@
   const int n = cfg->n_points, n_seg = cfg->n_seg;
   if (n == 0 || n_seg == 0) return SG_OK;
 
-  const int n_blocks = (n + kSelBlock - 1) / kSelBlock;
-  SG_TAKE(meta, int32_t, 64);
-  SG_TAKE(blk_cnt, int32_t, static_cast<size_t>(n_seg) * n_blocks);
-  SG_TAKE(blk_off, int32_t, static_cast<size_t>(n_seg) * n_blocks);
-  select_count_kernel<<<n_blocks, kSelBlock, 0, stream>>>(scores, n, cfg->n_sem_classes, cfg->seg_class, n_seg,
-                                                         cfg->score_thr, n_blocks, blk_cnt);
-  select_scan_kernel<<<1, 1024, 0, stream>>>(blk_cnt, n_seg, n_blocks, cfg->min_npoint, blk_off, meta);
-  SG_TRY(check_launch(kWhat));
-  SG_TRY(read_back(host, meta, 1, stream, kWhat));
-  const int n_sel = host[0];
+  Selection sel;
+  SG_TRY(select_classes(cfg, sel_words != nullptr ? kSelGivenWords : kSelMakeWords, scores, sel_words, blk_cnt,
+                        pt_offsets, coords_float, batch_idxs, 64, 1, ar, host, &res->arena_needed, &sel, stream, kWhat));
+  int32_t *meta = sel.meta, *obj = sel.obj, *seg_of = sel.seg_of, *key = sel.key;
+  float *pts = sel.pts;
+  const int n_sel = sel.n_sel;
   res->n_selected = n_sel;
   if (n_sel == 0) return SG_OK;
-  SG_TAKE(obj, int32_t, n_sel);
-  SG_TAKE(seg_of, int32_t, n_sel);
-  SG_TAKE(pts, float, 3 * static_cast<size_t>(n_sel));
-  SG_TAKE(key, int32_t, n_sel);
-  select_emit_kernel<<<n_blocks, kSelBlock, 0, stream>>>(scores, n, cfg->n_sem_classes, cfg->seg_class, n_seg,
-                                                        cfg->score_thr, n_blocks, blk_off, coords_float,
-                                                        pt_offsets, batch_idxs, cfg->batch_size, obj, seg_of,
-                                                        pts, key);
 
   const size_t bq_bytes = sg_ballquery_workspace_bytes(n_sel);
   SG_TAKE(bq_ws, char, bq_bytes);
@@ -560,6 +671,46 @@
   }
 
   return voxelise_proposals(cfg, pairs, poff, n_prop, S, coords_float, point_feats, ar, meta, host, res, stream_, kWhat);
+}
+
+}
+
+extern "C" {
+
+int sg_scan_grouping(const sg_grouping_cfg *cfg, const float *scores, const float *pt_offsets,
+                     const float *coords_float, const int32_t *batch_idxs, const float *point_feats,
+                     void *arena, size_t arena_bytes, sg_grouping_result *res, sg_stream_t stream_) {
+  return scan_grouping_run(cfg, scores, nullptr, nullptr, pt_offsets, coords_float, batch_idxs, point_feats, arena,
+                           arena_bytes, res, stream_);
+}
+
+int sg_scan_select(const sg_grouping_cfg *cfg, int source, const float *scores, const uint32_t *sel_words,
+                   const int32_t *blk_cnt, const float *pt_offsets, const float *coords_float,
+                   const int32_t *batch_idxs, void *arena, size_t arena_bytes, size_t *out, sg_stream_t stream_) {
+  static const char *kWhat = "sg_scan_select";
+  SG_REQUIRE(cfg != nullptr && out != nullptr && source >= kSelFromScores && source <= kSelGivenWords,
+             "sg_scan_select: bad arguments");
+  SG_REQUIRE(cfg->n_points >= 0 && cfg->n_sem_classes >= 1 && cfg->n_seg >= 0 && cfg->n_seg <= kMaxSeg &&
+                 cfg->batch_size >= 1,
+             "sg_scan_select: bad configuration (n_seg must be <= %d)", kMaxSeg);
+  memset(out, 0, sizeof(size_t) * 8);
+  int32_t *host = pinned_words();
+  SG_REQUIRE(host != nullptr, "sg_scan_select: no pinned host words");
+  ScanArena ar(arena, arena_bytes);
+  if (cfg->n_points == 0 || cfg->n_seg == 0) return SG_OK;
+  Selection sel;
+  SG_TRY(select_classes(cfg, source, scores, sel_words, blk_cnt, pt_offsets, coords_float, batch_idxs, 64, 1, ar, host,
+                        &out[7], &sel, as_stream(stream_), kWhat));
+  out[0] = static_cast<size_t>(sel.n_sel);
+  out[1] = ar.at(sel.meta);
+  if (sel.n_sel > 0) {
+    out[2] = ar.at(sel.obj);
+    out[3] = ar.at(sel.seg_of);
+    out[4] = ar.at(sel.pts);
+    out[5] = ar.at(sel.key);
+  }
+  out[6] = ar.off;
+  return check_launch(kWhat);
 }
 
 int sg_scan_grouping_pp(const sg_grouping_pp_cfg *pcfg, const float *scores, const float *pt_offsets,
diff --git a/softgroup_amd/csrc/scan_forward.hip b/softgroup_amd/csrc/scan_forward.hip
--- a/softgroup_amd/csrc/scan_forward.hip
+++ b/softgroup_amd/csrc/scan_forward.hip
@@ -21,6 +21,17 @@
 extern thread_local void (*t_unet_conv_hook)(void *);
 extern thread_local void *t_unet_conv_ctx;
 extern thread_local void *t_scan_emit_ctx;
+int scan_grouping_run(const sg_grouping_cfg *cfg, const float *scores, const uint32_t *sel_words,
+                      const int32_t *blk_cnt, const float *pt_offsets, const float *coords_float,
+                      const int32_t *batch_idxs, const float *point_feats, void *arena, size_t arena_bytes,
+                      sg_grouping_result *res, sg_stream_t stream);
+
+static int g_pointwise_fused = -1;
+static bool pointwise_fused() {
+  if (g_pointwise_fused >= 0) return g_pointwise_fused != 0;
+  const char *e = getenv("SG_POINTWISE_FUSED");
+  return !(e && atoi(e) == 0);
+}
 
 __global__ void __launch_bounds__(256) voxelize_cat_kernel(const float *__restrict__ a, int ca,
                                                           const float *__restrict__ b, int cb,
@@ -62,29 +73,12 @@
   const int64_t r = blockIdx.x * 256LL + threadIdx.x;
   if (r >= rows) return;
   float e[32];
-  float mx = -INFINITY;
 #pragma unroll
-  for (int j = 0; j < COLS_MAX; ++j) {
-    e[j] = j < cols ? x[r * cols + j] : -INFINITY;
-    mx = fmaxf(mx, e[j]);
-  }
-#pragma unroll
-  for (int j = 0; j < 32; ++j) e[j] = j < COLS_MAX ? expf(e[j] - mx) : 0.f;
-  float s[32];
-#pragma unroll
-  for (int j = 0; j < 32; ++j) s[j] = e[j];
-#pragma unroll
-  for (int off = 16; off > 0; off >>= 1) {
-    float t[32];
-#pragma unroll
-    for (int j = 0; j < 32; ++j) t[j] = __fadd_rn(s[j], s[j ^ off]);
-#pragma unroll
-    for (int j = 0; j < 32; ++j) s[j] = t[j];
-  }
-  const float sum = s[0];
+  for (int j = 0; j < COLS_MAX; ++j) e[j] = j < cols ? x[r * cols + j] : -INFINITY;
+  softmax_row<COLS_MAX>(e);
 #pragma unroll
   for (int j = 0; j < COLS_MAX; ++j)
-    if (j < cols) out[r * cols + j] = __fdiv_rn(e[j], sum);
+    if (j < cols) out[r * cols + j] = e[j];
 }
 
 template <int C>
@@ -299,6 +293,12 @@
 
 extern "C" {
 
+int sg_scan_set_pointwise_fused(int mode) {
+  const int before = g_pointwise_fused;
+  g_pointwise_fused = mode < 0 ? -1 : (mode != 0);
+  return before;
+}
+
 int sg_softmax_rows(const float *x, int64_t rows, int cols, float *out, sg_stream_t stream) {
   SG_REQUIRE(rows >= 0 && cols >= 1 && cols <= 32 && x && out, "sg_softmax_rows: rows of 1..32 columns (got %d)", cols);
   if (rows == 0) return SG_OK;
@@ -335,7 +335,8 @@
   const size_t N = static_cast<size_t>(n_points > 0 ? n_points : 1), M = static_cast<size_t>(n_voxels > 0 ? n_voxels : 1);
   const size_t C = static_cast<size_t>(d->channels), ns = static_cast<size_t>(d->semantic_classes);
   size_t p = align_up(M * 16) + align_up(M * 8 * 4) + align_up(M * C * 4) + align_up(N * C * 4) + 2 * align_up(N * ns * 4) +
-             align_up(N * 12) + 2 * align_up(N * 8) + align_up(N * 96) + (1 << 20);
+             align_up(N * 12) + 2 * align_up(N * 8) + align_up(N * 96) + (1 << 20) +
+             align_up(N * 4) + align_up(32 * (N / 256 + 1) * 4);
   size_t bb = sg_unet_arena_bytes(d->backbone, n_voxels) / 4;
   if (bb < (64u << 20)) bb = 64u << 20;
   const size_t later = (160u << 20) + N * 256;
@@ -384,10 +385,10 @@
   SG_CARVE(vfeat, float, static_cast<size_t>(M) * cin);
   SG_CARVE(bb_out, float, static_cast<size_t>(M) * C);
   SG_CARVE(out_feats, float, static_cast<size_t>(N) * C);
-  SG_CARVE(sem, float, static_cast<size_t>(N) * ns);
   SG_CARVE(prob, float, static_cast<size_t>(N) * ns);
-  SG_CARVE(off, float, static_cast<size_t>(N) * 3);
-  SG_CARVE(preds, int64_t, N);
+  const bool fused = d->want_instances && pointwise_fused();
+  const bool fused_sel = fused && !(d->with_pyramid || d->with_octree) && d->grouping.n_seg > 0;
+  int slot[5] = {-1, -1, -1, -1, -1};
   PackList pl;
   pl.n = 0;
   size_t dense_total = 0;
@@ -410,6 +411,7 @@
     res->dense_offset[i] = dense_total;
     pl.dst[i] = dense_total;
     pl.bytes[i] = nb;
+    if (fused && it.kind >= 1 && it.kind <= 4 && slot[it.kind] < 0) slot[it.kind] = i;
     dense_total += align_up(nb);
   }
   pl.n = in->n_dense;
@@ -419,19 +421,56 @@
     set_error("%s: host block for the dense results too small (%zu bytes, need %zu)", kWhat, host_dense_bytes, dense_total);
     return SG_ERR_WORKSPACE;
   }
-  int64_t *gt = nullptr;
-  if (want_gt) {
+  SG_CARVE(dense_dev, char, dense_total);
+  auto in_block = [&](int kind) -> char * { return slot[kind] >= 0 ? dense_dev + pl.dst[slot[kind]] : nullptr; };
+  int64_t *preds = reinterpret_cast<int64_t *>(in_block(1));
+  float *off = reinterpret_cast<float *>(in_block(2));
+  int64_t *gt = reinterpret_cast<int64_t *>(in_block(3));
+  float *sem = reinterpret_cast<float *>(in_block(4));
+  if (preds == nullptr) {
+    SG_CARVE(preds_, int64_t, N);
+    preds = preds_;
+  }
+  if (off == nullptr) {
+    SG_CARVE(off_, float, static_cast<size_t>(N) * 3);
+    off = off_;
+  }
+  if (gt == nullptr && want_gt) {
     SG_CARVE(gt_, int64_t, N);
     gt = gt_;
   }
-  SG_CARVE(dense_dev, char, dense_total);
-  for (int i = 0; i < in->n_dense; ++i) {
-    switch (in->dense[i].kind) {
-      case 0: pl.src[i] = static_cast<const char *>(in->dense[i].ptr); break;
-      case 1: pl.src[i] = reinterpret_cast<const char *>(preds); break;
-      case 2: pl.src[i] = reinterpret_cast<const char *>(off); break;
-      case 3: pl.src[i] = reinterpret_cast<const char *>(gt); break;
-      default: pl.src[i] = reinterpret_cast<const char *>(sem); break;
+  if (sem == nullptr) {
+    SG_CARVE(sem_, float, static_cast<size_t>(N) * ns);
+    sem = sem_;
+  }
+  {
+    int m = 0;
+    for (int i = 0; i < in->n_dense; ++i) {
+      const int kind = in->dense[i].kind;
+      if (kind >= 1 && kind <= 4 && slot[kind] == i) continue;
+      const char *src = kind == 0   ? static_cast<const char *>(in->dense[i].ptr)
+                        : kind == 1 ? reinterpret_cast<const char *>(preds)
+                        : kind == 2 ? reinterpret_cast<const char *>(off)
+                        : kind == 3 ? reinterpret_cast<const char *>(gt)
+                                    : reinterpret_cast<const char *>(sem);
+      pl.src[m] = src;
+      pl.dst[m] = pl.dst[i];
+      pl.bytes[m] = pl.bytes[i];
+      ++m;
+    }
+    pl.n = m;
+  }
+  uint32_t *sel_words = nullptr;
+  int32_t *sel_cnt = nullptr;
+  if (fused_sel) {
+    const size_t cnt_words = static_cast<size_t>(d->grouping.n_seg) * ((N + 255) / 256);
+    SG_CARVE(words_, uint32_t, N);
+    SG_CARVE(cnt_, int32_t, cnt_words);
+    sel_words = words_;
+    sel_cnt = cnt_;
+    if (hipMemsetAsync(sel_cnt, 0, sizeof(int32_t) * cnt_words, stream) != hipSuccess) {
+      set_error("%s: clearing the selection's block counts failed", kWhat);
+      return SG_ERR_LAUNCH;
     }
   }
   res->voxel_feats_in = ar.at(vfeat);
@@ -478,8 +517,13 @@
     if (rc == SG_ERR_WORKSPACE) res->arena_needed = ar.off + sg_unet_arena_bytes(d->backbone, M) + (64u << 20);
     SG_TRY_(rc);
   }
-  SG_TRY_(sg_pointwise_heads(bb_out, in->v2p_map, in->v2p_is_int64, N, C, &d->semantic, &d->offset, out_feats, sem, off,
-                             preds, stream_));
+  if (fused)
+    SG_TRY_(pointwise_front(bb_out, in->v2p_map, in->v2p_is_int64, N, C, as_mlp(d->semantic), as_mlp(d->offset),
+                            d->grouping.seg_class, fused_sel ? d->grouping.n_seg : 0, d->grouping.score_thr, out_feats,
+                            sem, prob, off, preds, sel_words, sel_cnt, true, stream));
+  else
+    SG_TRY_(sg_pointwise_heads(bb_out, in->v2p_map, in->v2p_is_int64, N, C, &d->semantic, &d->offset, out_feats, sem,
+                               off, preds, stream_));
   if (want_gt)
     gt_instances_kernel<<<grid_for(N, 256, 1024), 256, 0, stream>>>(in->semantic_labels, in->instance_labels, N,
                                                                   static_cast<int64_t>(d->semantic_classes - d->instance_classes), gt);
@@ -518,7 +562,7 @@
     if (hipStreamSynchronize(stream) != hipSuccess) return SG_ERR_LAUNCH;
     return SG_OK;
   }
-  SG_TRY_(sg_softmax_rows(sem, N, ns, prob, stream_));
+  if (!fused) SG_TRY_(sg_softmax_rows(sem, N, ns, prob, stream_));
   if (use_token) {
     if (hipEventRecord(ss->backbone_done, stream) != hipSuccess || hipEventSynchronize(ss->backbone_done) != hipSuccess) {
       set_error("%s: waiting for the backbone failed", kWhat);
@@ -552,8 +596,8 @@
       rc = sg_scan_grouping_pp(&pc, prob, off, in->coords_float, in->batch_idxs, out_feats,
                                static_cast<char *>(arena) + ar.off, room, &res->grouping, stream_);
     } else {
-      rc = sg_scan_grouping(&gc, prob, off, in->coords_float, in->batch_idxs, out_feats,
-                            static_cast<char *>(arena) + ar.off, room, &res->grouping, stream_);
+      rc = scan_grouping_run(&gc, prob, sel_words, sel_cnt, off, in->coords_float, in->batch_idxs, out_feats,
+                             static_cast<char *>(arena) + ar.off, room, &res->grouping, stream_);
     }
     if (rc == SG_ERR_WORKSPACE) res->arena_needed = ar.off + res->grouping.arena_needed + (64u << 20);
     if (rc != SG_OK) return rc;
```
